# DigITs-AIML/MMNN_STS

Hardware: AMD Instinct MI355X
Metric: training volumes/sec/GPU (128^3 T1+T2+preop, batch 2) at 1/2/4/8 MI355X (higher is better)
Workload: dtype f32; 1 GPU; configs[2] --images --preop --survival --blend: MultiModalModel(DenseNet121-3D(in=2), MLP(32), blend) fwd + GradientBlender Cox loss + bwd + grad all-reduce + SGD-Nesterov/OneCycle step, dropout 0.2; micro_batch=2, global_batch=2, tabular=32, parallelism=dp1, allreduce=none

## Files before the change

### mmnn_sts_amd/csrc/conv3_bf16x3.hip

```cpp
#include <stdlib.h>

#include "fprop.hpp"

namespace mmnn {

typedef float f32x16_t __attribute__((ext_vector_type(16)));
typedef __bf16 bf16x8_t __attribute__((ext_vector_type(8)));

namespace c3b {
constexpr int KC = 16, NT = 7, MAXC = 256;
template <int TD, int TH, int TW>
struct Geo {
  static constexpr int HD = TD + 2, HH = TH + 2, HW = TW + 2, HV = HD * HH * HW, ROWS = TD * TH * TW / 32;
  static constexpr int ITEMS = (2 * HV + 255) / 256;
  static constexpr size_t OPER_BYTES = (size_t)2 * 6 * HV * 16;
  static constexpr size_t SMEM = OPER_BYTES + sizeof(float) * (2 * MAXC + 2 * 4 * 32 + 32);
  static_assert(TD * TH * TW % 32 == 0 && (TW == 32 || TW == 16), "rows of 32 voxels");
  static_assert(ITEMS <= NT, "one staging item per tap slot");
  static_assert(4 * ROWS * 16 * 64 * sizeof(float) <= OPER_BYTES, "the partial tiles are summed in the operand buffers");
  static_assert(SMEM <= 160 * 1024, "LDS");
};

__device__ __forceinline__ void split3(float x, __bf16& h, __bf16& m, __bf16& l) {
  h = (__bf16)x;
  const float r1 = x - (float)h;
  m = (__bf16)r1;
  l = (__bf16)(r1 - (float)m);
}
__device__ __forceinline__ uint32_t pack2(__bf16 lo, __bf16 hi) {
  return (uint32_t)__builtin_bit_cast(unsigned short, lo) | ((uint32_t)__builtin_bit_cast(unsigned short, hi) << 16);
}
__device__ __forceinline__ bf16x8_t as_bf16x8(uint4 v) { return __builtin_bit_cast(bf16x8_t, v); }
}

template <int TD, int TH, int TW>
__global__ void __launch_bounds__(256) conv3_fwd_bf16x3_kernel(const FpropArgs a) {
  using namespace c3b;
  using G = Geo<TD, TH, TW>;
  constexpr int HH = G::HH, HW = G::HW, HV = G::HV, ROWS = G::ROWS, ITEMS = G::ITEMS;
  constexpr size_t OPER_BYTES = G::OPER_BYTES;
  extern __shared__ uint4 xs128[];
  float* const coef = reinterpret_cast<float*>(reinterpret_cast<char*>(xs128) + OPER_BYTES);
  float* const sred = coef + 2 * MAXC;
  float* const dsc = sred + 2 * 4 * 32;
  const int tid = threadIdx.x, lane = tid & 63, wv = tid >> 6, g = tid & 1;
  const int D = a.D, H = a.H, W = a.W, V = D * H * W, Cin = a.Cin, nchunk = Cin / KC;
  const int twn = (W + TW - 1) / TW, thn = (H + TH - 1) / TH, tdn = (D + TD - 1) / TD;
  int b = blockIdx.x;
  const int w0 = (b % twn) * TW; b /= twn;
  const int h0 = (b % thn) * TH; b /= thn;
  const int d0 = (b % tdn) * TD;
  const int n = b / tdn;
  const float* __restrict__ xin = a.in0 + (long)n * a.in0_ns + (long)a.in0_coff * V;
  const float* __restrict__ wgt = a.w;
  for (int c = tid; c < Cin; c += 256) {
    float ca_, cb_, mu, rs;
    bn_fwd_coef(a.bn_in, c, ca_, cb_, mu, rs);
    coef[c] = ca_; coef[MAXC + c] = cb_;
  }
  if (tid < 32) dsc[tid] = drop_scale(a.drop_out, n, tid);
  f32x16_t acc[ROWS];
#pragma unroll
  for (int t = 0; t < ROWS; ++t)
#pragma unroll
    for (int q = 0; q < 16; ++q) acc[t][q] = 0.f;
  float xr[ITEMS][8], ca[8], cb[8];
  auto item_pos = [&](int it, int& hv, int& o) -> bool {
    const int item = tid + it * 256;
    hv = item >> 1;
    const int hd = hv / (HH * HW), hh = (hv / HW) % HH, hw = hv % HW;
    const int d = d0 + hd - 1, h = h0 + hh - 1, w = w0 + hw - 1;
    o = (d * H + h) * W + w;
    return item < 2 * HV && (unsigned)d < (unsigned)D && (unsigned)h < (unsigned)H && (unsigned)w < (unsigned)W;
  };
  auto issue = [&](int ch) {
    const int c0 = ch * KC + 8 * g;
#pragma unroll
    for (int e = 0; e < 8; ++e) { ca[e] = coef[c0 + e]; cb[e] = coef[MAXC + c0 + e]; }
#pragma unroll
    for (int it = 0; it < ITEMS; ++it) {
      int hv, o;
      const bool ok = item_pos(it, hv, o);
#pragma unroll
      for (int e = 0; e < 8; ++e) xr[it][e] = ok ? xin[(long)(c0 + e) * V + o] : 0.f;
    }
  };
  auto commit_item = [&](int it, int buf) {
    int hv, o;
    const bool ok = item_pos(it, hv, o);
    if (tid + it * 256 >= 2 * HV) return;
    __bf16 ph[8], pm[8], pl[8];
#pragma unroll
    for (int e = 0; e < 8; ++e) split3(ok ? fmaxf(fmaf(ca[e], xr[it][e], cb[e]), 0.f) : 0.f, ph[e], pm[e], pl[e]);
    uint4* dst = xs128 + buf * (6 * HV);
    dst[(0 * 2 + g) * HV + hv] = make_uint4(pack2(ph[0], ph[1]), pack2(ph[2], ph[3]), pack2(ph[4], ph[5]), pack2(ph[6], ph[7]));
    dst[(1 * 2 + g) * HV + hv] = make_uint4(pack2(pm[0], pm[1]), pack2(pm[2], pm[3]), pack2(pm[4], pm[5]), pack2(pm[6], pm[7]));
    dst[(2 * 2 + g) * HV + hv] = make_uint4(pack2(pl[0], pl[1]), pack2(pl[2], pl[3]), pack2(pl[4], pl[5]), pack2(pl[6], pl[7]));
  };
  float wr[NT][8];
  auto load_w = [&](int ti, int ch) {
    const int tap = wv + 4 * ti;
    if (tap < 27 && ch < nchunk) {
      const int c0 = ch * KC + 8 * (lane >> 5);
#pragma unroll
      for (int e = 0; e < 8; ++e) wr[ti][e] = wgt[((long)(c0 + e) * 27 + tap) * a.w_ld + (lane & 31)];
    }
  };
#pragma unroll
  for (int ti = 0; ti < NT; ++ti) load_w(ti, 0);
  __syncthreads();
  issue(0);
#pragma unroll
  for (int it = 0; it < ITEMS; ++it) commit_item(it, 0);
  __syncthreads();
  for (int ch = 0; ch < nchunk; ++ch) {
    const int cur = ch & 1;
    const bool more = ch + 1 < nchunk;
    if (more) issue(ch + 1);
#pragma unroll
    for (int ti = 0; ti < NT; ++ti) {
      const int tap = wv + 4 * ti;
      if (tap < 27) {
        const int td = tap / 9, th = (tap / 3) % 3, tw = tap % 3;
        __bf16 ph[8], pm[8], pl[8];
#pragma unroll
        for (int e = 0; e < 8; ++e) split3(wr[ti][e], ph[e], pm[e], pl[e]);
        bf16x8_t aw[3];
#pragma unroll
        for (int e = 0; e < 8; ++e) { aw[0][e] = ph[e]; aw[1][e] = pm[e]; aw[2][e] = pl[e]; }
        load_w(ti, ch + 1);
#pragma unroll
        for (int t = 0; t < ROWS; ++t) {
          const int v = t * 32 + (lane & 31);
          const int hv = ((v / (TW * TH) + td) * HH + ((v / TW) % TH + th)) * HW + (v % TW + tw);
          bf16x8_t bb[3];
#pragma unroll
          for (int p = 0; p < 3; ++p) bb[p] = as_bf16x8(xs128[cur * (6 * HV) + (p * 2 + (lane >> 5)) * HV + hv]);
          acc[t] = __builtin_amdgcn_mfma_f32_32x32x16_bf16(aw[1], bb[1], acc[t], 0, 0, 0);
          acc[t] = __builtin_amdgcn_mfma_f32_32x32x16_bf16(aw[0], bb[2], acc[t], 0, 0, 0);
          acc[t] = __builtin_amdgcn_mfma_f32_32x32x16_bf16(aw[2], bb[0], acc[t], 0, 0, 0);
          acc[t] = __builtin_amdgcn_mfma_f32_32x32x16_bf16(aw[0], bb[1], acc[t], 0, 0, 0);
          acc[t] = __builtin_amdgcn_mfma_f32_32x32x16_bf16(aw[1], bb[0], acc[t], 0, 0, 0);
          acc[t] = __builtin_amdgcn_mfma_f32_32x32x16_bf16(aw[0], bb[0], acc[t], 0, 0, 0);
        }
      }
      if (more && ti < ITEMS) commit_item(ti, cur ^ 1);
    }
    __syncthreads();
  }
  float* red = reinterpret_cast<float*>(xs128);
#pragma unroll
  for (int t = 0; t < ROWS; ++t)
#pragma unroll
    for (int q = 0; q < 16; ++q) red[((wv * ROWS + t) * 16 + q) * 64 + lane] = acc[t][q];
  __syncthreads();
  float* __restrict__ outn = a.out + (long)n * a.out_ns + (long)a.out_coff * V;
  const bool want_sums = a.st_out.sum != nullptr;
  float s0[16], s1[16];
#pragma unroll
  for (int q = 0; q < 16; ++q) { s0[q] = 0.f; s1[q] = 0.f; }
#pragma unroll
  for (int tt = 0; tt < (ROWS + 3) / 4; ++tt) {
    const int t = wv + 4 * tt;
    if (t >= ROWS) break;
    const int v = t * 32 + (lane & 31);
    const int d = d0 + v / (TW * TH), h = h0 + (v / TW) % TH, w = w0 + v % TW;
    const bool ok = d < D && h < H && w < W;
    const int o = (d * H + h) * W + w;
#pragma unroll
    for (int q = 0; q < 16; ++q) {
      float val = 0.f;
#pragma unroll
      for (int w2 = 0; w2 < 4; ++w2) val += red[((w2 * ROWS + t) * 16 + q) * 64 + lane];
      const int m = 8 * (q / 4) + 4 * (lane >> 5) + q % 4;
      val *= dsc[m];
      if (ok) {
        outn[(long)m * V + o] = val;
        s0[q] += val;
        s1[q] += val * val;
      }
    }
  }
  if (want_sums) {
#pragma unroll
    for (int q = 0; q < 16; ++q) {
      float t0 = s0[q], t1 = s1[q];
      t0 += swz_xor<16>(t0); t1 += swz_xor<16>(t1);
      t0 += swz_xor<8>(t0);  t1 += swz_xor<8>(t1);
      t0 += swz_xor<4>(t0);  t1 += swz_xor<4>(t1);
      t0 += swz_xor<2>(t0);  t1 += swz_xor<2>(t1);
      t0 += swz_xor<1>(t0);  t1 += swz_xor<1>(t1);
      if ((lane & 31) == 0) {
        const int m = 8 * (q / 4) + 4 * (lane >> 5) + q % 4;
        sred[wv * 32 + m] = t0;
        sred[4 * 32 + wv * 32 + m] = t1;
      }
    }
    __syncthreads();
    if (tid < 32) {
      const int rep = blockIdx.x & ((a.nrep > 0 ? a.nrep : NREP) - 1);
      double v0 = 0.0, v1 = 0.0;
#pragma unroll
      for (int w2 = 0; w2 < 4; ++w2) { v0 += (double)sred[w2 * 32 + tid]; v1 += (double)sred[4 * 32 + w2 * 32 + tid]; }
      atomicAdd(a.st_out.sum + (long)rep * a.st_out.stride + a.st_out.off + tid, v0);
      atomicAdd(a.st_out.sq + (long)rep * a.st_out.stride + a.st_out.off + tid, v1);
    }
  }
}

__global__ void __launch_bounds__(256) conv3_dgrad_bf16x3_kernel(const FpropArgs a) {
  using namespace c3b;
  using G = Geo<2, 4, 32>;
  constexpr int TH = 4, TW = 32, HH = G::HH, HW = G::HW, HV = G::HV, ROWS = G::ROWS, ITEMS = G::ITEMS, PF = 3;
  extern __shared__ uint4 xs128[];
  float* const coef = reinterpret_cast<float*>(reinterpret_cast<char*>(xs128) + G::OPER_BYTES);
  float* const ecoef = coef + 96;
  const int tid = threadIdx.x, lane = tid & 63, wv = tid >> 6, g = tid & 1;
  const int D = a.D, H = a.H, W = a.W, V = D * H * W;
  const int twn = (W + TW - 1) / TW, thn = (H + TH - 1) / TH, tdn = (D + 1) / 2;
  int b = blockIdx.x;
  const int w0 = (b % twn) * TW; b /= twn;
  const int h0 = (b % thn) * TH; b /= thn;
  const int d0 = (b % tdn) * 2;
  const int n = b / tdn;
  const float* __restrict__ in0n = a.in0 + (long)n * a.in0_ns + (long)a.in0_coff * V;
  const float* __restrict__ in1n = a.in1 + (long)n * a.in1_ns + (long)a.in1_coff * V;
  const float* __restrict__ wgt = a.w;
  if (tid < 32) {
    float p_, q_, r_;
    bn_bwd_coef(a.gr_in, tid, p_, q_, r_);
    const float sc = drop_scale(a.drop_in, n, tid);
    coef[tid] = p_ * sc; coef[32 + tid] = q_ * sc; coef[64 + tid] = r_ * sc;
  }
  if (tid >= 128) {
    const int m = tid - 128;
    float ea, eb, mu, rs;
    bn_fwd_coef(a.ebn, m, ea, eb, mu, rs);
    ecoef[m] = ea; ecoef[128 + m] = eb; ecoef[256 + m] = mu; ecoef[384 + m] = rs;
  }
  float x0[2][ITEMS][8], x1[2][ITEMS][8];
  auto item_pos = [&](int it, int& hv, int& o) -> bool {
    const int item = tid + it * 256;
    hv = item >> 1;
    const int hd = hv / (HH * HW), hh = (hv / HW) % HH, hw = hv % HW;
    const int d = d0 + hd - 1, h = h0 + hh - 1, w = w0 + hw - 1;
    o = (d * H + h) * W + w;
    return item < 2 * HV && (unsigned)d < (unsigned)D && (unsigned)h < (unsigned)H && (unsigned)w < (unsigned)W;
  };
  auto issue = [&](int ch) {
    const int c0 = ch * KC + 8 * g;
#pragma unroll
    for (int it = 0; it < ITEMS; ++it) {
      int hv, o;
      const bool ok = item_pos(it, hv, o);
#pragma unroll
      for (int e = 0; e < 8; ++e) {
        x0[ch][it][e] = ok ? in0n[(long)(c0 + e) * V + o] : 0.f;
        x1[ch][it][e] = ok ? in1n[(long)(c0 + e) * V + o] : 0.f;
      }
    }
  };
  auto commit_item = [&](int it, int buf) {
    int hv, o;
    const bool ok = item_pos(it, hv, o);
    if (tid + it * 256 >= 2 * HV) return;
    const int c0 = buf * KC + 8 * g;
    __bf16 ph[8], pm[8], pl[8];
#pragma unroll
    for (int e = 0; e < 8; ++e)
      split3(ok ? fmaf(coef[c0 + e], x0[buf][it][e], fmaf(coef[32 + c0 + e], x1[buf][it][e], coef[64 + c0 + e])) : 0.f, ph[e], pm[e], pl[e]);
    uint4* dst = xs128 + buf * (6 * HV);
    dst[(0 * 2 + g) * HV + hv] = make_uint4(pack2(ph[0], ph[1]), pack2(ph[2], ph[3]), pack2(ph[4], ph[5]), pack2(ph[6], ph[7]));
    dst[(1 * 2 + g) * HV + hv] = make_uint4(pack2(pm[0], pm[1]), pack2(pm[2], pm[3]), pack2(pm[4], pm[5]), pack2(pm[6], pm[7]));
    dst[(2 * 2 + g) * HV + hv] = make_uint4(pack2(pl[0], pl[1]), pack2(pl[2], pl[3]), pack2(pl[4], pl[5]), pack2(pl[6], pl[7]));
  };
  float wr[PF][8];
  auto load_w = [&](int slot, int tap, int ch) {
    if (ch < 2) {
      const int c0 = ch * KC + 8 * (lane >> 5);
#pragma unroll
      for (int e = 0; e < 8; ++e) wr[slot][e] = wgt[((long)(c0 + e) * 27 + tap) * a.w_ld + wv * 32 + (lane & 31)];
    }
  };
#pragma unroll
  for (int t = 0; t < PF; ++t) load_w(t, t, 0);
  issue(0);
  issue(1);
  __syncthreads();
#pragma unroll
  for (int it = 0; it < ITEMS; ++it) commit_item(it, 0);
#pragma unroll
  for (int it = 0; it < ITEMS; ++it) commit_item(it, 1);
  __syncthreads();
  f32x16_t acc[ROWS];
#pragma unroll
  for (int t = 0; t < ROWS; ++t)
#pragma unroll
    for (int q = 0; q < 16; ++q) acc[t][q] = 0.f;
  for (int ch = 0; ch < 2; ++ch) {
#pragma unroll 1
    for (int tq = 0; tq < 9; ++tq) {
    const int td = tq / 3, th = tq % 3;
#pragma unroll
    for (int tw = 0; tw < 3; ++tw) {
      const int tap = tq * 3 + tw;
      __bf16 ph[8], pm[8], pl[8];
#pragma unroll
      for (int e = 0; e < 8; ++e) split3(wr[tw][e], ph[e], pm[e], pl[e]);
      bf16x8_t aw[3];
#pragma unroll
      for (int e = 0; e < 8; ++e) { aw[0][e] = ph[e]; aw[1][e] = pm[e]; aw[2][e] = pl[e]; }
      if (tq < 8) load_w(tw, tap + PF, ch); else load_w(tw, tw, ch + 1);
#pragma unroll
      for (int t = 0; t < ROWS; ++t) {
        const int hv = ((t / TH + td) * HH + (t % TH + th)) * HW + ((lane & 31) + tw);
        bf16x8_t bb[3];
#pragma unroll
        for (int p = 0; p < 3; ++p) bb[p] = as_bf16x8(xs128[ch * (6 * HV) + (p * 2 + (lane >> 5)) * HV + hv]);
        acc[t] = __builtin_amdgcn_mfma_f32_32x32x16_bf16(aw[1], bb[1], acc[t], 0, 0, 0);
        acc[t] = __builtin_amdgcn_mfma_f32_32x32x16_bf16(aw[0], bb[2], acc[t], 0, 0, 0);
        acc[t] = __builtin_amdgcn_mfma_f32_32x32x16_bf16(aw[2], bb[0], acc[t], 0, 0, 0);
        acc[t] = __builtin_amdgcn_mfma_f32_32x32x16_bf16(aw[0], bb[1], acc[t], 0, 0, 0);
        acc[t] = __builtin_amdgcn_mfma_f32_32x32x16_bf16(aw[1], bb[0], acc[t], 0, 0, 0);
        acc[t] = __builtin_amdgcn_mfma_f32_32x32x16_bf16(aw[0], bb[0], acc[t], 0, 0, 0);
      }
    }
    }
  }
  const float* __restrict__ exn = a.ex + (long)n * a.ex_ns + (long)a.ex_coff * V;
  float* __restrict__ outn = a.out + (long)n * a.out_ns + (long)a.out_coff * V;
  float s0[16], s1[16];
#pragma unroll
  for (int q = 0; q < 16; ++q) { s0[q] = 0.f; s1[q] = 0.f; }
  auto row_pos = [&](int t, int& o) -> bool {
    const int d = d0 + t / TH, h = h0 + t % TH, w = w0 + (lane & 31);
    o = (d * H + h) * W + w;
    return d < D && h < H && w < W;
  };
  float xn[16];
  {
    int o;
    const bool ok = row_pos(0, o);
#pragma unroll
    for (int q = 0; q < 16; ++q) xn[q] = ok ? exn[(long)(wv * 32 + 8 * (q / 4) + 4 * (lane >> 5) + q % 4) * V + o] : 0.f;
  }
#pragma unroll
  for (int t = 0; t < ROWS; ++t) {
    int o;
    const bool ok = row_pos(t, o);
    float xe[16];
#pragma unroll
    for (int q = 0; q < 16; ++q) xe[q] = xn[q];
    if (t + 1 < ROWS) {
      int o2;
      const bool ok2 = row_pos(t + 1, o2);
#pragma unroll
      for (int q = 0; q < 16; ++q) xn[q] = ok2 ? exn[(long)(wv * 32 + 8 * (q / 4) + 4 * (lane >> 5) + q % 4) * V + o2] : 0.f;
    }
#pragma unroll
    for (int q = 0; q < 16; ++q) {
      const int m = wv * 32 + 8 * (q / 4) + 4 * (lane >> 5) + q % 4;
      if (ok) {
        const float pre = fmaf(ecoef[m], xe[q], ecoef[128 + m]);
        const float z = pre > 0.f ? acc[t][q] : 0.f;
        const float xh = (xe[q] - ecoef[256 + m]) * ecoef[384 + m];
        outn[(long)m * V + o] = z;
        s0[q] += z;
        s1[q] += z * xh;
      }
    }
  }
  const int rep = blockIdx.x & ((a.nrep > 0 ? a.nrep : NREP) - 1);
#pragma unroll
  for (int q = 0; q < 16; ++q) {
    float t0 = s0[q], t1 = s1[q];
    t0 += swz_xor<16>(t0); t1 += swz_xor<16>(t1);
    t0 += swz_xor<8>(t0);  t1 += swz_xor<8>(t1);
    t0 += swz_xor<4>(t0);  t1 += swz_xor<4>(t1);
    t0 += swz_xor<2>(t0);  t1 += swz_xor<2>(t1);
    t0 += swz_xor<1>(t0);  t1 += swz_xor<1>(t1);
    if ((lane & 31) == 0) {
      const int m = wv * 32 + 8 * (q / 4) + 4 * (lane >> 5) + q % 4;
      atomicAdd(a.dbeta + (long)rep * a.M + m, (double)t0);
      atomicAdd(a.dgamma + (long)rep * a.M + m, (double)t1);
    }
  }
}

bool conv3_dgrad_bf16x3_eligible(const FpropArgs& a) {
  static const int mode = [] { const char* e = getenv("MMNN_BF16X3_DGRAD"); return e ? atoi(e) : 1; }();
  static const int fmode = [] { const char* e = getenv("MMNN_BF16X3"); return e ? atoi(e) : 32; }();
  return mode != 0 && fmode != 0 && a.M == 128 && a.Cin == 32 && a.W > 16;
}

int launch_conv3_dgrad_bf16x3(const FpropArgs& a, hipStream_t stream) {
  using G = c3b::Geo<2, 4, 32>;
  constexpr size_t SMEM = G::OPER_BYTES + sizeof(float) * (96 + 512);
  static_assert(SMEM <= 160 * 1024, "LDS");
  MMNN_REQUIRE(conv3_dgrad_bf16x3_eligible(a), "conv3 dgrad bf16x3: shape not handled (M=%d, Cin=%d, W=%d)", a.M, a.Cin, a.W);
  MMNN_REQUIRE(a.in1 && a.ex && a.dgamma && a.dbeta, "conv3 dgrad bf16x3: operands missing");
  MMNN_REQUIRE((long)(a.M + 1) * a.D * a.H * a.W < (1l << 31), "conv3 dgrad bf16x3: volume too large for 32-bit element offsets");
  const long tiles = (long)a.N * cdiv(a.D, 2) * cdiv(a.H, 4) * cdiv(a.W, 32);
  MMNN_REQUIRE(tiles > 0 && tiles < (1l << 31), "conv3 dgrad bf16x3: grid out of range");
  static bool configured[MAX_DEVICES] = {false};
  bool& conf = configured[current_device_slot()];
  if (!conf) {
    MMNN_HIP(hipFuncSetAttribute(reinterpret_cast<const void*>(conv3_dgrad_bf16x3_kernel), hipFuncAttributeMaxDynamicSharedMemorySize, (int)SMEM));
    conf = true;
  }
  MMNN_LAUNCH(conv3_dgrad_bf16x3_kernel, dim3((unsigned)tiles), dim3(256), SMEM, stream, a);
  MMNN_HIP(hipGetLastError());
  return 0;
}

bool conv3_fwd_bf16x3_eligible(const FpropArgs& a) {
  static const int mode = [] { const char* e = getenv("MMNN_BF16X3"); return e ? atoi(e) : 32; }();
  return mode != 0 && a.M == 32 && a.Cin % c3b::KC == 0 && a.Cin >= c3b::KC && a.Cin <= c3b::MAXC && a.W > 16;
}

int launch_conv3_fwd_bf16x3(const FpropArgs& a, hipStream_t stream) {
  using G = c3b::Geo<2, 4, 32>;
  MMNN_REQUIRE(conv3_fwd_bf16x3_eligible(a), "conv3 bf16x3: shape not handled (M=%d, Cin=%d, W=%d)", a.M, a.Cin, a.W);
  MMNN_REQUIRE(a.drop_in.p <= 0.f, "conv3 bf16x3: no input dropout on this path");
  MMNN_REQUIRE((long)(a.Cin + 1) * a.D * a.H * a.W < (1l << 31), "conv3 bf16x3: volume too large for 32-bit element offsets");
  const long tiles = (long)a.N * cdiv(a.D, 2) * cdiv(a.H, 4) * cdiv(a.W, 32);
  MMNN_REQUIRE(tiles > 0 && tiles < (1l << 31), "conv3 bf16x3: grid out of range");
  static bool configured[MAX_DEVICES] = {false};
  bool& conf = configured[current_device_slot()];
  if (!conf) {
    MMNN_HIP(hipFuncSetAttribute(reinterpret_cast<const void*>(conv3_fwd_bf16x3_kernel<2, 4, 32>), hipFuncAttributeMaxDynamicSharedMemorySize, (int)G::SMEM));
    conf = true;
  }
  MMNN_LAUNCH((conv3_fwd_bf16x3_kernel<2, 4, 32>), dim3((unsigned)tiles), dim3(256), G::SMEM, stream, a);
  MMNN_HIP(hipGetLastError());
  return 0;
}

}
```

### mmnn_sts_amd/csrc/densenet.hip

```cpp
#include "densenet.hpp"

#include <stdlib.h>
#include <string.h>

#include <algorithm>

#include "fprop.hpp"
#include "stem.hpp"
#include "wgrad.hpp"

namespace mmnn {

static size_t align_up(size_t v, size_t a = 256) { return (v + a - 1) / a * a; }
constexpr size_t KZ_PART_BYTES = (size_t)512 * 4 * 1024 * sizeof(float);
constexpr unsigned KZ_CNT_ENTRIES = 4096;

namespace {
struct Carver {
  size_t cur = 0;
  size_t take(size_t bytes) {
    size_t o = cur;
    cur = align_up(cur + bytes);
    return o;
  }
};
}

int plan_build(Plan& p, const NetCfg& cfg, int N, int D, int H, int W) {
  MMNN_REQUIRE(cfg.nblocks >= 1 && cfg.nblocks <= MAX_BLOCKS, "plan: 1..%d dense blocks supported, got %d", MAX_BLOCKS, cfg.nblocks);
  MMNN_REQUIRE(cfg.in_channels >= 1 && cfg.in_channels <= 4, "plan: in_channels must be 1..4, got %d", cfg.in_channels);
  MMNN_REQUIRE(cfg.init_features >= 1 && cfg.init_features <= 64, "plan: init_features must be <= 64, got %d", cfg.init_features);
  MMNN_REQUIRE(cfg.growth >= 1 && cfg.growth <= 32, "plan: growth_rate must be <= 32, got %d", cfg.growth);
  MMNN_REQUIRE(cfg.bn_size >= 1 && cfg.dropout_p >= 0.f && cfg.dropout_p < 1.f, "plan: bad bn_size / dropout");
  MMNN_REQUIRE(N >= 1 && D >= 1 && H >= 1 && W >= 1, "plan: bad input extent");
  p.cfg = cfg; p.N = N; p.D = D; p.H = H; p.W = W;
  p.mid = cfg.bn_size * cfg.growth;
  p.D0 = (D - 1) / 2 + 1; p.H0 = (H - 1) / 2 + 1; p.W0 = (W - 1) / 2 + 1;
  int d = (p.D0 - 1) / 2 + 1, h = (p.H0 - 1) / 2 + 1, w = (p.W0 - 1) / 2 + 1;
  int c = cfg.init_features;
  for (int b = 0; b < cfg.nblocks; ++b) {
    MMNN_REQUIRE(cfg.block_layers[b] >= 1, "plan: empty dense block %d", b);
    MMNN_REQUIRE(d >= 1 && h >= 1 && w >= 1, "plan: input too small, block %d has no voxels", b + 1);
    p.Db[b] = d; p.Hb[b] = h; p.Wb[b] = w; p.Vb[b] = d * h * w;
    p.cin_b[b] = c;
    p.nrep_b[b] = (b == 0 || (long)N * d * h * w >= 32768) ? NREP : ((long)N * d * h * w >= 4096 ? 2 : 1);
    p.ctot_b[b] = c + cfg.block_layers[b] * cfg.growth;
    c = p.ctot_b[b];
    if (b != cfg.nblocks - 1) {
      MMNN_REQUIRE(c % 2 == 0, "plan: transition halves an odd channel count");
      c /= 2; d /= 2; h /= 2; w /= 2;
    }
  }
  long po = 0, ro = 0;
  int nbn = 0;
  auto bn = [&](int ch, long& w_, long& b_, long& m_, long& v_) { w_ = po; po += ch; b_ = po; po += ch; m_ = ro; ro += ch; v_ = ro; ro += ch; ++nbn; };
  p.p_conv0 = po; po += (long)cfg.init_features * cfg.in_channels * 343;
  bn(cfg.init_features, p.p_n0w, p.p_n0b, p.r_n0m, p.r_n0v);
  p.layers.assign(cfg.nblocks, {});
  p.trans.clear();
  for (int b = 0; b < cfg.nblocks; ++b) {
    int ci = p.cin_b[b];
    for (int l = 0; l < cfg.block_layers[b]; ++l) {
      LayerOff lo;
      lo.cin = ci;
      bn(ci, lo.n1w, lo.n1b, lo.r1m, lo.r1v);
      lo.c1 = po; po += (long)p.mid * ci;
      bn(p.mid, lo.n2w, lo.n2b, lo.r2m, lo.r2v);
      lo.c2 = po; po += (long)cfg.growth * p.mid * 27;
      p.layers[b].push_back(lo);
      ci += cfg.growth;
    }
    if (b != cfg.nblocks - 1) {
      TransOff t;
      t.cin = ci; t.cout = ci / 2;
      bn(ci, t.nw, t.nb, t.rm, t.rv);
      t.cw = po; po += (long)t.cout * ci;
      p.trans.push_back(t);
    } else {
      bn(ci, p.p_n5w, p.p_n5b, p.r_n5m, p.r_n5v);
    }
  }
  p.n_params = po; p.n_runstats = ro; p.n_bn = nbn;

  Carver cv;
  const int nb = cfg.nblocks;
  const size_t F = sizeof(float);
  const long V0 = (long)p.D0 * p.H0 * p.W0;
  p.o_conv0 = cv.take((size_t)N * cfg.init_features * V0 * F);
  p.o_idx = cv.take((size_t)N * cfg.init_features * p.Vb[0]);
  p.o_t1.assign(nb, {});
  size_t dap = 0;
  for (int b = 0; b < nb; ++b) {
    p.o_x[b] = cv.take((size_t)N * p.ctot_b[b] * p.Vb[b] * F);
    p.o_g[b] = cv.take((size_t)N * p.ctot_b[b] * p.Vb[b] * F);
    for (int l = 0; l < cfg.block_layers[b]; ++l) p.o_t1[b].push_back(cv.take((size_t)N * p.mid * p.Vb[b] * F));
    if (b != nb - 1) {
      p.o_ap[b] = cv.take((size_t)N * p.ctot_b[b] * p.Vb[b + 1] * F);
      dap = std::max(dap, (size_t)N * p.ctot_b[b] * p.Vb[b + 1] * F);
    } else {
      p.o_ap[b] = 0;
    }
  }
  p.o_dap = cv.take(dap ? dap : 256);
  p.o_dz0 = cv.take((size_t)N * cfg.init_features * V0 * F);
  const size_t PAIR = 2 * NREP * sizeof(double);
  p.o_fstat = cv.cur;
  p.o_st_conv0 = cv.take(PAIR * cfg.init_features);
  p.o_st_t1.assign(nb, {});
  for (int b = 0; b < nb; ++b) {
    p.o_st_x[b] = cv.take(PAIR * p.ctot_b[b]);
    for (int l = 0; l < cfg.block_layers[b]; ++l) p.o_st_t1[b].push_back(cv.take(PAIR * p.mid));
  }
  p.fstat_bytes = cv.cur - p.o_fstat;
  p.o_bstat = cv.cur;
  p.o_dg_n0 = cv.take(PAIR * cfg.init_features);
  p.o_dg_n1.assign(nb, {}); p.o_dg_n2.assign(nb, {}); p.o_dg_tr.clear();
  for (int b = 0; b < nb; ++b) {
    p.o_s_x[b] = cv.take(PAIR * p.ctot_b[b]);
    for (int l = 0; l < cfg.block_layers[b]; ++l) {
      p.o_dg_n1[b].push_back(cv.take(PAIR * p.layers[b][l].cin));
      p.o_dg_n2[b].push_back(cv.take(PAIR * p.mid));
    }
    if (b != nb - 1) p.o_dg_tr.push_back(cv.take(PAIR * p.ctot_b[b]));
  }
  p.o_dg_n5 = cv.take(PAIR * p.ctot_b[nb - 1]);
  p.bstat_bytes = cv.cur - p.o_bstat;
  p.o_pk_conv0 = cv.take((size_t)7 * stem_krows(cfg.in_channels) * 64 * F);
  p.o_pk_c1.assign(nb, {}); p.o_pk_c2f.assign(nb, {}); p.o_pk_c2b.assign(nb, {}); p.o_pk_tr.clear();
  for (int b = 0; b < nb; ++b) {
    for (int l = 0; l < cfg.block_layers[b]; ++l) {
      p.o_pk_c1[b].push_back(cv.take((size_t)p.mid * p.layers[b][l].cin * F));
      p.o_pk_c2f[b].push_back(cv.take((size_t)cfg.growth * p.mid * 27 * F));
      p.o_pk_c2b[b].push_back(cv.take((size_t)cfg.growth * p.mid * 27 * F));
    }
    if (b != nb - 1) p.o_pk_tr.push_back(cv.take((size_t)p.trans[b].cin * p.trans[b].cout * F));
  }
  p.ns_conv0 = stem_wgrad_pick_splits(N, p.D0, p.H0, p.W0, cfg.in_channels);
  p.o_sl_conv0 = cv.take((size_t)p.ns_conv0 * cfg.in_channels * cfg.init_features * 352 * F);
  p.o_sl_c1.assign(nb, {}); p.o_sl_c2.assign(nb, {}); p.ns_c1.assign(nb, {}); p.ns_c2.assign(nb, {});
  p.o_sl_tr.clear(); p.ns_tr.clear();
  for (int b = 0; b < nb; ++b) {
    for (int l = 0; l < cfg.block_layers[b]; ++l) {
      const int ci = p.layers[b][l].cin;
      int pairs = 0;
      {
        const int cw = wgrad1_channel_width(ci, p.Vb[b]);
        for (int k = 0; k < cfg.block_layers[b]; ++k)
          if (wgrad1_channel_width(p.layers[b][k].cin, p.Vb[b]) == cw) pairs += cdiv(p.layers[b][k].cin, cw);
      }
      const int s1 = wgrad_pick_splits(1, N, p.Db[b], p.Hb[b], p.Wb[b], p.mid, ci, pairs);
      const int s2 = wgrad_pick_splits(27, N, p.Db[b], p.Hb[b], p.Wb[b], cfg.growth, p.mid, cfg.block_layers[b]);
      p.ns_c1[b].push_back(s1); p.ns_c2[b].push_back(s2);
      p.o_sl_c1[b].push_back(cv.take((size_t)s1 * p.mid * ci * F));
      p.o_sl_c2[b].push_back(cv.take((size_t)s2 * 27 * cfg.growth * p.mid * F));
    }
    if (b != nb - 1) {
      const int s = wgrad_pick_splits(1, N, p.Db[b + 1], p.Hb[b + 1], p.Wb[b + 1], p.trans[b].cout, p.trans[b].cin);
      p.ns_tr.push_back(s);
      p.o_sl_tr.push_back(cv.take((size_t)s * p.trans[b].cout * p.trans[b].cin * F));
    }
  }
  for (int b = 0; b < nb; ++b) p.o_dz2[b] = cv.take((size_t)cfg.block_layers[b] * N * p.mid * p.Vb[b] * F);
  p.o_kz_part = cv.take(KZ_PART_BYTES);
  p.o_kz_cnt = cv.take(KZ_CNT_ENTRIES * sizeof(unsigned));
  int nlayers = 0;
  for (int b = 0; b < nb; ++b) nlayers += cfg.block_layers[b];
  p.n_run_jobs = nbn;
  p.n_pack_jobs = 1 + 3 * nlayers + (nb - 1);
  p.n_grad_jobs = 3 + 6 * nlayers + 3 * (nb - 1) + 2;
  p.o_jobs_run = cv.take(sizeof(RunStatJob) * p.n_run_jobs);
  p.o_jobs_pack = cv.take(sizeof(PackJob) * p.n_pack_jobs);
  p.o_jobs_grad = cv.take(sizeof(GradJob) * p.n_grad_jobs);
  p.n_layers = nlayers;
  p.o_wg_table = cv.take(sizeof(WgradArgs) * 2 * nlayers);
  p.ws_bytes = cv.cur;
  p.host_jobs_bytes = p.o_wg_table - p.o_jobs_run;
  if (p.host_jobs) { (void)hipHostFree(p.host_jobs); p.host_jobs = nullptr; }
  p.tab_params = nullptr; p.tab_run = nullptr; p.tab_ws = nullptr;
  return 0;
}

void plan_free(Plan& p) {
  if (p.host_jobs) (void)hipHostFree(p.host_jobs);
  p.host_jobs = nullptr;
  if (p.wg_pinned) (void)hipHostFree(p.wg_pinned);
  p.wg_pinned = nullptr;
  for (hipEvent_t e : p.timer_ev) (void)hipEventDestroy(e);
  p.timer_ev.clear();
  for (hipEvent_t e : p.sync_ev) (void)hipEventDestroy(e);
  p.sync_ev.clear();
  if (p.side) (void)hipStreamDestroy(p.side);
  if (p.side2) (void)hipStreamDestroy(p.side2);
  p.side = p.side2 = nullptr;
}

static StatPtr statptr(char* ws, size_t o, int C, int off, int nrep = NREP) {
  StatPtr s;
  s.sum = reinterpret_cast<double*>(ws + o);
  s.sq = s.sum + (long)NREP * C;
  s.stride = C;
  s.off = off;
  s.nrep = nrep;
  s.pad_ = 0;
  return s;
}
static float* fptr(char* ws, size_t o) { return reinterpret_cast<float*>(ws + o); }

static void set_kz(FpropArgs& a, const Plan& p, char* ws) {
  a.kz_part = p.no_kz ? nullptr : fptr(ws, p.o_kz_part); a.kz_cnt = reinterpret_cast<unsigned*>(ws + p.o_kz_cnt);
  a.kz_part_bytes = KZ_PART_BYTES; a.kz_cnt_entries = KZ_CNT_ENTRIES;
  a.trace = (p.trace_base && p.trace_seq < p.trace_slots) ? p.trace_base + (size_t)(p.trace_seq++) * 64 * 16 : nullptr;
}

static BnFwd bnfwd(const Plan& p, StatPtr st, const float* params, float* run, long w, long b, long rm, long rv, double count, int training) {
  BnFwd f;
  f.st = st;
  f.rmean = run + rm; f.rvar = run + rv;
  f.gamma = params + w; f.beta = params + b;
  f.inv_count = 1.0 / count;
  f.eps = p.cfg.eps;
  f.training = training;
  return f;
}

static bool build_tables(Plan& p, const float* params, float* run, char* ws) {
  if (p.tab_params == params && p.tab_run == run && p.tab_ws == ws) return false;
  char* hj = static_cast<char*>(p.host_jobs);
  RunStatJob* rj = reinterpret_cast<RunStatJob*>(hj);
  PackJob* pj = reinterpret_cast<PackJob*>(hj + (p.o_jobs_pack - p.o_jobs_run));
  GradJob* gj = reinterpret_cast<GradJob*>(hj + (p.o_jobs_grad - p.o_jobs_run));
  const NetCfg& c = p.cfg;
  const int nb = c.nblocks;
  int ir = 0, ip = 0, ig = 0;
  p.max_pack = 0; p.max_grad = 0;
  auto run_job = [&](size_t o, int C, int off, int n, long rm, long rv, double count) {
    StatPtr s = statptr(ws, o, C, off);
    RunStatJob j; j.sum = s.sum; j.sq = s.sq; j.stride = C; j.off = off; j.C = n; j.rmean = run ? run + rm : nullptr; j.rvar = run ? run + rv : nullptr; j.count = count;
    rj[ir++] = j;
  };
  auto pack_job = [&](long src, size_t dst, int kind, int M, int C, long count) {
    PackJob j; j.src = params + src; j.dst = fptr(ws, dst); j.kind = kind; j.M = M; j.C = C; j.count = count;
    pj[ip++] = j; p.max_pack = std::max(p.max_pack, count);
  };
  auto grad_slab = [&](int kind, size_t o, long stride, int ns, int M, int C, long dst, long count) {
    GradJob j; j.kind = kind; j.src = ws + o; j.stride = stride; j.nsplit = ns; j.off = 0; j.M = M; j.C = C; j.dst_off = dst; j.count = count;
    gj[ig++] = j; p.max_grad = std::max(p.max_grad, count);
  };
  auto grad_bn = [&](size_t o, int C, long dw, long db) {
    StatPtr s = statptr(ws, o, C, 0);
    GradJob j; j.kind = 3; j.stride = C; j.nsplit = 0; j.off = 0; j.M = 0; j.C = C; j.count = C;
    j.src = s.sq; j.dst_off = dw; gj[ig++] = j;
    j.src = s.sum; j.dst_off = db; gj[ig++] = j;
    p.max_grad = std::max(p.max_grad, (long)C);
  };
  const double cnt0 = (double)p.N * p.D0 * p.H0 * p.W0;
  run_job(p.o_st_conv0, c.init_features, 0, c.init_features, p.r_n0m, p.r_n0v, cnt0);
  pack_job(p.p_conv0, p.o_pk_conv0, (c.in_channels % 2 == 0) ? 3 : 4, c.init_features, c.in_channels, (long)7 * stem_krows(c.in_channels) * 64);
  grad_slab(2, p.o_sl_conv0, (long)c.in_channels * c.init_features * 352, p.ns_conv0, c.init_features, c.in_channels, p.p_conv0,
            (long)c.init_features * c.in_channels * 343);
  grad_bn(p.o_dg_n0, c.init_features, p.p_n0w, p.p_n0b);
  for (int b = 0; b < nb; ++b) {
    const double cnt = (double)p.N * p.Vb[b];
    p.gj_begin[b] = ig;
    const long max_before = p.max_grad;
    p.max_grad = 0;
    for (int l = 0; l < c.block_layers[b]; ++l) {
      const LayerOff& lo = p.layers[b][l];
      run_job(p.o_st_x[b], p.ctot_b[b], 0, lo.cin, lo.r1m, lo.r1v, cnt);
      run_job(p.o_st_t1[b][l], p.mid, 0, p.mid, lo.r2m, lo.r2v, cnt);
      pack_job(lo.c1, p.o_pk_c1[b][l], 0, p.mid, lo.cin, (long)p.mid * lo.cin);
      pack_job(lo.c2, p.o_pk_c2f[b][l], 1, c.growth, p.mid, (long)c.growth * p.mid * 27);
      pack_job(lo.c2, p.o_pk_c2b[b][l], 2, c.growth, p.mid, (long)c.growth * p.mid * 27);
      grad_bn(p.o_dg_n1[b][l], lo.cin, lo.n1w, lo.n1b);
      grad_slab(0, p.o_sl_c1[b][l], (long)p.mid * lo.cin, p.ns_c1[b][l], p.mid, lo.cin, lo.c1, (long)p.mid * lo.cin);
      grad_bn(p.o_dg_n2[b][l], p.mid, lo.n2w, lo.n2b);
      grad_slab(1, p.o_sl_c2[b][l], (long)27 * c.growth * p.mid, p.ns_c2[b][l], c.growth, p.mid, lo.c2, (long)c.growth * p.mid * 27);
    }
    if (b != nb - 1) {
      const TransOff& t = p.trans[b];
      run_job(p.o_st_x[b], p.ctot_b[b], 0, t.cin, t.rm, t.rv, cnt);
      pack_job(t.cw, p.o_pk_tr[b], 0, t.cout, t.cin, (long)t.cout * t.cin);
      grad_bn(p.o_dg_tr[b], t.cin, t.nw, t.nb);
      grad_slab(0, p.o_sl_tr[b], (long)t.cout * t.cin, p.ns_tr[b], t.cout, t.cin, t.cw, (long)t.cout * t.cin);
    } else {
      run_job(p.o_st_x[b], p.ctot_b[b], 0, p.ctot_b[b], p.r_n5m, p.r_n5v, cnt);
      grad_bn(p.o_dg_n5, p.ctot_b[b], p.p_n5w, p.p_n5b);
    }
    p.gj_max[b] = p.max_grad;
    p.max_grad = std::max(p.max_grad, max_before);
  }
  p.gj_begin[nb] = ig;
  p.n_run_jobs = ir; p.n_pack_jobs = ip; p.n_grad_jobs = ig;
  p.tab_params = params; p.tab_run = run; p.tab_ws = ws;
  return true;
}

namespace {
struct ScopedTimer {
  Plan& p; hipStream_t s; bool on;
  ScopedTimer(Plan& p_, int kind, int block, hipStream_t s_) : p(p_), s(s_), on(false) {
    if (!((p.timer_mask >> kind) & 1u) || (p.timer_block >= 0 && p.timer_block != block)) return;
    if (p.timer_used + 2 > p.timer_ev.size()) {
      if (p.timer_ev.size() >= 16384) return;
      hipEvent_t a, b;
      if (hipEventCreate(&a) != hipSuccess || hipEventCreate(&b) != hipSuccess) return;
      p.timer_ev.push_back(a); p.timer_ev.push_back(b);
      p.timer_tag.push_back(0);
    }
    p.timer_tag[p.timer_used / 2] = kind * MAX_BLOCKS + (block >= 0 && block < MAX_BLOCKS ? block : 0);
    on = hipEventRecord(p.timer_ev[p.timer_used], s) == hipSuccess;
  }
  ~ScopedTimer() {
    if (!on) return;
    (void)hipEventRecord(p.timer_ev[p.timer_used + 1], s);
    p.timer_used += 2;
  }
};
}

int plan_set_timer(Plan& p, int kind, int block) {
  MMNN_REQUIRE(kind >= -1 && kind < T_COUNT, "set_timer: unknown kernel class %d", kind);
  p.timer_mask = kind < 0 ? ~1u : (kind == T_NONE ? 0u : 1u << kind);
  p.timer_block = block; p.timer_used = 0;
  for (int k = 0; k < T_COUNT * MAX_BLOCKS; ++k) { p.timer_ms[k] = 0.0; p.timer_count[k] = 0; }
  return 0;
}

int plan_read_timer(Plan& p, int kind, int block, double* total_ms, long* count) {
  MMNN_REQUIRE(kind >= T_NONE && kind < T_COUNT && block < MAX_BLOCKS, "read_timer: unknown kernel class %d / block %d", kind, block);
  for (size_t i = 0; i + 1 < p.timer_used; i += 2) {
    MMNN_HIP(hipEventSynchronize(p.timer_ev[i + 1]));
    float ms = 0.f;
    MMNN_HIP(hipEventElapsedTime(&ms, p.timer_ev[i], p.timer_ev[i + 1]));
    const int k = p.timer_tag[i / 2];
    p.timer_ms[k] += ms; p.timer_count[k] += 1;
  }
  p.timer_used = 0;
  double ms = 0.0; long n = 0;
  for (int k = 1; k < T_COUNT; ++k)
    for (int b = 0; b < MAX_BLOCKS; ++b)
      if ((kind == T_NONE || kind == k) && (block < 0 || block == b)) { ms += p.timer_ms[k * MAX_BLOCKS + b]; n += p.timer_count[k * MAX_BLOCKS + b]; }
  if (total_ms) *total_ms = ms;
  if (count) *count = n;
  return 0;
}

int plan_set_option(Plan& p, const char* name, long value) {
  const std::string s(name ? name : "");
  if (s == "single_stream") { p.single_stream = value != 0; return 0; }
  if (s == "side_streams") { p.side_streams = value < 0 ? 0 : (value > 2 ? 2 : (int)value); p.side_tried = false; return 0; }
  if (s == "trace_buffer") { p.trace_base = reinterpret_cast<unsigned long long*>(value); p.trace_seq = 0; return 0; }
  if (s == "trace_slots") { p.trace_slots = (int)value; return 0; }
  if (s == "params_version") { p.params_version = value; return 0; }
  if (s == "no_kz") { p.no_kz = value != 0; return 0; }
  set_error("set_option: unknown option '%s'", s.c_str());
  return 1;
}

static DropCfg dropcfg(const Plan& p, uint64_t seed, int layer, int training) {
  DropCfg d;
  d.seed = seed; d.layer = layer;
  d.p = training ? p.cfg.dropout_p : 0.f;
  return d;
}

int plan_forward(Plan& p, const float* params, float* run, const float* x, char* ws, float* out, int training, uint64_t seed,
                 hipStream_t stream) {
  MMNN_REQUIRE(params && run && x && ws && out, "forward: null buffer");
  MMNN_REQUIRE(((uintptr_t)ws & 255) == 0 && ((uintptr_t)params & 15) == 0 && ((uintptr_t)x & 15) == 0, "forward: buffers must be 256/16-byte aligned");
  const NetCfg& c = p.cfg;
  const int nb = c.nblocks, N = p.N;
  if (!p.host_jobs) {
    MMNN_HIP(hipHostMalloc(&p.host_jobs, p.host_jobs_bytes, hipHostMallocDefault));
    memset(p.host_jobs, 0, p.host_jobs_bytes);
  }
  if (p.tab_params != params || p.tab_run != run || p.tab_ws != ws) {
    if (p.tab_ws != nullptr) MMNN_HIP(hipStreamSynchronize(stream));
    build_tables(p, params, run, ws);
    MMNN_HIP(hipMemcpyAsync(ws + p.o_jobs_run, p.host_jobs, p.host_jobs_bytes, hipMemcpyHostToDevice, stream));
  }
  p.trace_seq = 0;
  if (training) MMNN_HIP(hipMemsetAsync(ws + p.o_fstat, 0, p.fstat_bytes, stream));
  MMNN_HIP(hipMemsetAsync(ws + p.o_kz_cnt, 0, KZ_CNT_ENTRIES * sizeof(unsigned), stream));
  int rc = 0;
  if (p.params_version == 0 || p.params_version != p.packed_version || p.packed_params != params || p.packed_ws != ws) {
    rc = launch_pack(reinterpret_cast<const PackJob*>(ws + p.o_jobs_pack), p.n_pack_jobs, p.max_pack, stream);
    if (rc) return rc;
    p.packed_version = p.params_version; p.packed_params = params; p.packed_ws = ws;
    ++p.pack_launches;
  }

  const double cnt0 = (double)N * p.D0 * p.H0 * p.W0;
  {
    StemConvArgs a;
    a.N = N; a.Cin = c.in_channels; a.D = p.D; a.H = p.H; a.W = p.W; a.Do = p.D0; a.Ho = p.H0; a.Wo = p.W0; a.M = c.init_features;
    a.x = x; a.wp = fptr(ws, p.o_pk_conv0); a.out = fptr(ws, p.o_conv0);
    a.st_out = statptr(ws, p.o_st_conv0, c.init_features, 0);
    if (!training) a.st_out.sum = nullptr;
    { ScopedTimer t(p, T_STEM_CONV, -1, stream); rc = launch_stem_conv(a, stream); }
    if (rc) return rc;
    StemPoolArgs q;
    q.N = N; q.C = c.init_features; q.Di = p.D0; q.Hi = p.H0; q.Wi = p.W0; q.Do = p.Db[0]; q.Ho = p.Hb[0]; q.Wo = p.Wb[0];
    q.x = fptr(ws, p.o_conv0);
    q.bn = bnfwd(p, statptr(ws, p.o_st_conv0, c.init_features, 0), params, run, p.p_n0w, p.p_n0b, p.r_n0m, p.r_n0v, cnt0, training);
    q.out = fptr(ws, p.o_x[0]); q.out_ns = (long)p.ctot_b[0] * p.Vb[0];
    q.idx = reinterpret_cast<unsigned char*>(ws + p.o_idx);
    q.st_out = statptr(ws, p.o_st_x[0], p.ctot_b[0], 0, p.nrep_b[0]);
    if (!training) q.st_out.sum = nullptr;
    if ((rc = launch_stem_pool(q, stream))) return rc;
  }
  int layer_id = 0;
  for (int b = 0; b < nb; ++b) {
    const double cnt = (double)N * p.Vb[b];
    const long xns = (long)p.ctot_b[b] * p.Vb[b];
    for (int l = 0; l < c.block_layers[b]; ++l, ++layer_id) {
      const LayerOff& lo = p.layers[b][l];
      FpropArgs a;
      memset(&a, 0, sizeof(a));
      set_kz(a, p, ws);
      a.N = N; a.D = p.Db[b]; a.H = p.Hb[b]; a.W = p.Wb[b];
      a.Cin = lo.cin; a.M = p.mid; a.nrep = p.nrep_b[b];
      a.in0 = fptr(ws, p.o_x[b]); a.in0_ns = xns; a.in0_coff = 0;
      a.bn_in = bnfwd(p, statptr(ws, p.o_st_x[b], p.ctot_b[b], 0, p.nrep_b[b]), params, run, lo.n1w, lo.n1b, lo.r1m, lo.r1v, cnt, training);
      a.w = fptr(ws, p.o_pk_c1[b][l]); a.w_ld = p.mid;
      a.out = fptr(ws, p.o_t1[b][l]); a.out_ns = (long)p.mid * p.Vb[b]; a.out_coff = 0;
      a.st_out = statptr(ws, p.o_st_t1[b][l], p.mid, 0, p.nrep_b[b]);
      if (!training) a.st_out.sum = nullptr;
      a.pf_ptr = fptr(ws, p.o_pk_c2f[b][l]); a.pf_bytes = (unsigned)(sizeof(float) * c.growth * p.mid * 27);
      { ScopedTimer t(p, T_CONV1_FWD, b, stream); rc = launch_fprop(a, 1, PRO_BNRELU, EPI_STORE_STATS, stream); }
      if (rc) return rc;
      FpropArgs e;
      memset(&e, 0, sizeof(e));
      set_kz(e, p, ws);
      e.N = N; e.D = p.Db[b]; e.H = p.Hb[b]; e.W = p.Wb[b];
      e.Cin = p.mid; e.M = c.growth; e.nrep = p.nrep_b[b];
      e.in0 = fptr(ws, p.o_t1[b][l]); e.in0_ns = (long)p.mid * p.Vb[b]; e.in0_coff = 0;
      e.bn_in = bnfwd(p, statptr(ws, p.o_st_t1[b][l], p.mid, 0, p.nrep_b[b]), params, run, lo.n2w, lo.n2b, lo.r2m, lo.r2v, cnt, training);
      e.w = fptr(ws, p.o_pk_c2f[b][l]); e.w_ld = c.growth;
      e.out = fptr(ws, p.o_x[b]); e.out_ns = xns; e.out_coff = lo.cin;
      e.drop_out = dropcfg(p, seed, layer_id, training);
      e.st_out = statptr(ws, p.o_st_x[b], p.ctot_b[b], lo.cin, p.nrep_b[b]);
      if (!training) e.st_out.sum = nullptr;
      if (l + 1 < c.block_layers[b]) {
        e.pf_ptr = fptr(ws, p.o_pk_c1[b][l + 1]); e.pf_bytes = (unsigned)(sizeof(float) * p.mid * p.layers[b][l + 1].cin);
      } else if (b != nb - 1) {
        e.pf_ptr = fptr(ws, p.o_pk_tr[b]); e.pf_bytes = (unsigned)(sizeof(float) * p.trans[b].cin * p.trans[b].cout);
      }
      { ScopedTimer t(p, T_CONV2_FWD, b, stream); rc = launch_fprop(e, 27, PRO_BNRELU, EPI_STORE_STATS, stream); }
      if (rc) return rc;
    }
    if (b != nb - 1) {
      const TransOff& t = p.trans[b];
      PoolFwdArgs q;
      q.N = N; q.C = t.cin; q.D = p.Db[b]; q.H = p.Hb[b]; q.W = p.Wb[b];
      q.x = fptr(ws, p.o_x[b]); q.x_ns = xns;
      q.bn = bnfwd(p, statptr(ws, p.o_st_x[b], p.ctot_b[b], 0, p.nrep_b[b]), params, run, t.nw, t.nb, t.rm, t.rv, cnt, training);
      q.out = fptr(ws, p.o_ap[b]);
      if ((rc = launch_bnrelu_avgpool(q, stream))) return rc;
      FpropArgs a;
      memset(&a, 0, sizeof(a));
      set_kz(a, p, ws);
      a.N = N; a.D = p.Db[b + 1]; a.H = p.Hb[b + 1]; a.W = p.Wb[b + 1];
      a.Cin = t.cin; a.M = t.cout; a.nrep = p.nrep_b[b + 1];
      a.in0 = fptr(ws, p.o_ap[b]); a.in0_ns = (long)t.cin * p.Vb[b + 1]; a.in0_coff = 0;
      a.w = fptr(ws, p.o_pk_tr[b]); a.w_ld = t.cout;
      a.out = fptr(ws, p.o_x[b + 1]); a.out_ns = (long)p.ctot_b[b + 1] * p.Vb[b + 1]; a.out_coff = 0;
      a.st_out = statptr(ws, p.o_st_x[b + 1], p.ctot_b[b + 1], 0, p.nrep_b[b + 1]);
      if (!training) a.st_out.sum = nullptr;
      a.pf_ptr = fptr(ws, p.o_pk_c1[b + 1][0]); a.pf_bytes = (unsigned)(sizeof(float) * p.mid * p.layers[b + 1][0].cin);
      if ((rc = launch_fprop(a, 1, PRO_NONE, EPI_STORE_STATS, stream))) return rc;
    } else {
      BnApplyArgs q;
      q.N = N; q.C = p.ctot_b[b]; q.V = p.Vb[b];
      q.x = fptr(ws, p.o_x[b]); q.x_ns = xns;
      q.bn = bnfwd(p, statptr(ws, p.o_st_x[b], p.ctot_b[b], 0, p.nrep_b[b]), params, run, p.p_n5w, p.p_n5b, p.r_n5m, p.r_n5v, cnt, training);
      q.out = out;
      if ((rc = launch_bn_apply(q, stream))) return rc;
    }
  }
  if (training) {
    if ((rc = launch_running_stats(reinterpret_cast<const RunStatJob*>(ws + p.o_jobs_run), p.n_run_jobs, c.momentum,
                                   p.nbt_count == p.n_run_jobs ? p.nbt : nullptr, stream))) return rc;
  }
  return 0;
}

static void layer_wgrad_args(const Plan& p, const float* params, float* run, char* ws, int b, int l, int layer_id, uint64_t seed,
                             WgradArgs& w2, WgradArgs& w1) {
  const NetCfg& c = p.cfg;
  const int N = p.N;
  const double cnt = (double)N * p.Vb[b];
  const long xns = (long)p.ctot_b[b] * p.Vb[b], tns = (long)p.mid * p.Vb[b];
  const LayerOff& lo = p.layers[b][l];
  const BnFwd bn1 = bnfwd(p, statptr(ws, p.o_st_x[b], p.ctot_b[b], 0, p.nrep_b[b]), params, run, lo.n1w, lo.n1b, lo.r1m, lo.r1v, cnt, 1);
  const BnFwd bn2 = bnfwd(p, statptr(ws, p.o_st_t1[b][l], p.mid, 0, p.nrep_b[b]), params, run, lo.n2w, lo.n2b, lo.r2m, lo.r2v, cnt, 1);
  const StatPtr dg2 = statptr(ws, p.o_dg_n2[b][l], p.mid, 0, p.nrep_b[b]);
  float* dz2 = fptr(ws, p.o_dz2[b]) + (long)l * N * tns;
  memset(&w2, 0, sizeof(w2));
  w2.N = N; w2.D = p.Db[b]; w2.H = p.Hb[b]; w2.W = p.Wb[b];
  w2.M = c.growth; w2.Cin = p.mid;
  w2.g0 = fptr(ws, p.o_g[b]); w2.g0_ns = xns; w2.g0_coff = lo.cin;
  w2.g1 = fptr(ws, p.o_x[b]); w2.g1_ns = xns; w2.g1_coff = lo.cin;
  w2.gr.st = statptr(ws, p.o_st_x[b], p.ctot_b[b], lo.cin, p.nrep_b[b]);
  w2.gr.s = statptr(ws, p.o_s_x[b], p.ctot_b[b], lo.cin, p.nrep_b[b]);
  w2.gr.gamma = nullptr; w2.gr.inv_count = 1.0 / cnt; w2.gr.eps = c.eps;
  w2.drop.seed = seed; w2.drop.layer = layer_id; w2.drop.p = c.dropout_p;
  w2.x = fptr(ws, p.o_t1[b][l]); w2.x_ns = tns; w2.x_coff = 0;
  w2.bn = bn2;
  w2.slab = fptr(ws, p.o_sl_c2[b][l]); w2.slab_stride = (long)27 * c.growth * p.mid; w2.nsplit = p.ns_c2[b][l];
  memset(&w1, 0, sizeof(w1));
  w1.N = N; w1.D = p.Db[b]; w1.H = p.Hb[b]; w1.W = p.Wb[b];
  w1.M = p.mid; w1.Cin = lo.cin;
  w1.g0 = dz2; w1.g0_ns = tns; w1.g0_coff = 0;
  w1.g1 = fptr(ws, p.o_t1[b][l]); w1.g1_ns = tns; w1.g1_coff = 0;
  w1.gr.st = statptr(ws, p.o_st_t1[b][l], p.mid, 0, p.nrep_b[b]);
  w1.gr.s = dg2;
  w1.gr.gamma = params + lo.n2w; w1.gr.inv_count = 1.0 / cnt; w1.gr.eps = c.eps;
  w1.x = fptr(ws, p.o_x[b]); w1.x_ns = xns; w1.x_coff = 0;
  w1.bn = bn1;
  w1.slab = fptr(ws, p.o_sl_c1[b][l]); w1.slab_stride = (long)p.mid * lo.cin; w1.nsplit = p.ns_c1[b][l];
}

int plan_backward(Plan& p, const float* params, const float* x, char* ws, const float* grad_out, float* grad_params, int accumulate,
                  uint64_t seed, hipStream_t stream) {
  return plan_backward_range(p, params, x, ws, grad_out, grad_params, accumulate, seed, p.cfg.nblocks - 1, 0, stream);
}

int plan_block_param_range(const Plan& p, int block, long* begin, long* end) {
  const int nb = p.cfg.nblocks;
  MMNN_REQUIRE(block >= -1 && block < nb && begin && end, "block_param_range: block %d out of range [-1, %d)", block, nb);
  if (block < 0) { *begin = 0; *end = p.layers[0][0].n1w; return 0; }
  *begin = p.layers[block][0].n1w;
  *end = (block + 1 < nb) ? p.layers[block + 1][0].n1w : p.n_params;
  return 0;
}

int plan_backward_range(Plan& p, const float* params, const float* x, char* ws, const float* grad_out, float* grad_params, int accumulate,
                        uint64_t seed, int hi, int lo, hipStream_t stream) {
  MMNN_REQUIRE(params && x && ws && grad_out && grad_params, "backward: null buffer");
  MMNN_REQUIRE(p.tab_ws == ws && p.tab_params == params, "backward: must follow a training forward on the same buffers");
  const NetCfg& c = p.cfg;
  const int nb = c.nblocks, N = p.N;
  MMNN_REQUIRE(hi >= lo && lo >= 0 && hi < nb, "backward: bad block range [%d, %d] of %d blocks", lo, hi, nb);
  MMNN_REQUIRE(hi == nb - 1 || p.bwd_next == hi, "backward: block range [%d, %d] out of order (expected to continue at block %d)", lo, hi, p.bwd_next);
  float* run = p.tab_run;
  int rc;
  const bool first_call = hi == nb - 1;
  if (first_call) {
    MMNN_HIP(hipMemsetAsync(ws + p.o_bstat, 0, p.bstat_bytes, stream));
    MMNN_HIP(hipMemsetAsync(ws + p.o_kz_cnt, 0, KZ_CNT_ENTRIES * sizeof(unsigned), stream));
  }
  p.bwd_next = lo - 1;
  const int want_side = p.single_stream ? 0 : p.side_streams;
  const bool single = want_side <= 0;
  if (!single && (!p.side || (want_side >= 2 && !p.side2)) && !p.side_tried) {
    p.side_tried = true;
    if (!p.side && hipStreamCreateWithFlags(&p.side, hipStreamNonBlocking) != hipSuccess) p.side = nullptr;
    if (want_side >= 2 && p.side && !p.side2 && hipStreamCreateWithFlags(&p.side2, hipStreamNonBlocking) != hipSuccess) p.side2 = nullptr;
  }
  hipStream_t side = (p.side && !single) ? p.side : stream;
  hipStream_t side2 = (p.side2 && !single && want_side >= 2) ? p.side2 : side;
  const bool two = side != stream;
  p.sync_used = 0;
  auto next_event = [&]() -> hipEvent_t {
    if (p.sync_used == p.sync_ev.size()) {
      hipEvent_t e = nullptr;
      if (hipEventCreateWithFlags(&e, hipEventDisableTiming) != hipSuccess) return nullptr;
      p.sync_ev.push_back(e);
    }
    return p.sync_ev[p.sync_used++];
  };
  auto order = [&](hipStream_t from, hipStream_t to) -> int {
    if (!two) return 0;
    hipEvent_t e = next_event();
    MMNN_REQUIRE(e != nullptr, "backward: cannot create a synchronisation event");
    MMNN_HIP(hipEventRecord(e, from));
    MMNN_HIP(hipStreamWaitEvent(to, e, 0));
    return 0;
  };
  if (first_call || !p.wg_uploaded) {
    const size_t bytes = sizeof(WgradArgs) * 2 * p.n_layers;
    if (!p.wg_pinned) {
      MMNN_HIP(hipHostMalloc(&p.wg_pinned, bytes, hipHostMallocDefault));
      p.wg_shadow.assign(bytes, 0);
      p.wg_uploaded = false;
    }
    std::vector<WgradArgs> tab(2 * p.n_layers);
    int id = 0;
    for (int b = 0; b < nb; ++b)
      for (int l = 0; l < c.block_layers[b]; ++l, ++id) layer_wgrad_args(p, params, run, ws, b, l, id, 0, tab[id], tab[p.n_layers + id]);
    if (!p.wg_uploaded || memcmp(tab.data(), p.wg_shadow.data(), bytes) != 0) {
      if (p.wg_uploaded) MMNN_HIP(hipStreamSynchronize(stream));
      memcpy(p.wg_pinned, tab.data(), bytes);
      memcpy(p.wg_shadow.data(), tab.data(), bytes);
      MMNN_HIP(hipMemcpyAsync(ws + p.o_wg_table, p.wg_pinned, bytes, hipMemcpyHostToDevice, stream));
      p.wg_uploaded = true;
    }
  }
  const WgradArgs* dev_w2 = reinterpret_cast<const WgradArgs*>(ws + p.o_wg_table);
  const WgradArgs* dev_w1 = dev_w2 + p.n_layers;
  struct PendingW { WgradArgs w2, w1; int b, id; };
  std::vector<PendingW> pend;
  static const bool no_batch = [] { const char* e = getenv("MMNN_NO_WGRAD_BATCH"); return e && e[0] == '1'; }();
  auto flush = [&]() -> int {
    if (pend.empty()) return 0;
    int rc2;
    if (two) {
      hipEvent_t e = next_event();
      MMNN_REQUIRE(e != nullptr, "backward: cannot create a synchronisation event");
      MMNN_HIP(hipEventRecord(e, stream));
      MMNN_HIP(hipStreamWaitEvent(side, e, 0));
      if (side2 != side) MMNN_HIP(hipStreamWaitEvent(side2, e, 0));
    }
    const int np = (int)pend.size();
    std::vector<WgradArgs> host(np);
    if (np > 1 && !no_batch) {
      for (int i = 0; i < np; ++i) host[np - 1 - i] = pend[i].w2;
      { ScopedTimer t(p, T_CONV2_WGRAD, pend[0].b, side); rc2 = launch_wgrad_batched(host.data(), dev_w2 + pend[np - 1].id, np, seed, 27, PRO_BNRELU, side); }
      if (rc2) return rc2;
      for (int i = 0; i < np;) {
        int j = i + 1;
        const long vb = (long)pend[i].w1.D * pend[i].w1.H * pend[i].w1.W;
        while (j < np && wgrad1_channel_width(pend[j].w1.Cin, vb) == wgrad1_channel_width(pend[i].w1.Cin, vb)) ++j;
        if (j - i > 1) {
          for (int k = i; k < j; ++k) host[j - 1 - k] = pend[k].w1;
          ScopedTimer t(p, T_CONV1_WGRAD, pend[i].b, side2);
          rc2 = launch_wgrad_batched(host.data(), dev_w1 + pend[j - 1].id, j - i, seed, 1, PRO_BNRELU, side2);
        } else {
          ScopedTimer t(p, T_CONV1_WGRAD, pend[i].b, side2);
          rc2 = launch_wgrad(pend[i].w1, 1, PRO_BNRELU, side2);
        }
        if (rc2) return rc2;
        i = j;
      }
    } else {
      for (const PendingW& q : pend) {
        { ScopedTimer t(p, T_CONV2_WGRAD, q.b, side); rc2 = launch_wgrad(q.w2, 27, PRO_BNRELU, side); }
        if (rc2) return rc2;
      }
      for (const PendingW& q : pend) {
        { ScopedTimer t(p, T_CONV1_WGRAD, q.b, side2); rc2 = launch_wgrad(q.w1, 1, PRO_BNRELU, side2); }
        if (rc2) return rc2;
      }
    }
    pend.clear();
    return 0;
  };
  auto sptr = [&](int b, int off) { return statptr(ws, p.o_s_x[b], p.ctot_b[b], off, p.nrep_b[b]); };
  auto concat_grad = [&](int b, int off) {
    BnBwd g;
    g.st = statptr(ws, p.o_st_x[b], p.ctot_b[b], off, p.nrep_b[b]);
    g.s = sptr(b, off);
    g.gamma = nullptr;
    g.inv_count = 1.0 / ((double)N * p.Vb[b]);
    g.eps = c.eps;
    return g;
  };
  if (first_call) {
    const int b = nb - 1;
    ConsumerBwdArgs a;
    a.N = N; a.C = p.ctot_b[b]; a.D = p.Db[b]; a.H = p.Hb[b]; a.W = p.Wb[b]; a.mode = 0; a.nrep = p.nrep_b[b];
    a.dy = grad_out;
    a.x = fptr(ws, p.o_x[b]); a.x_ns = (long)p.ctot_b[b] * p.Vb[b];
    a.bn = bnfwd(p, statptr(ws, p.o_st_x[b], p.ctot_b[b], 0, p.nrep_b[b]), params, run, p.p_n5w, p.p_n5b, p.r_n5m, p.r_n5v, (double)N * p.Vb[b], 1);
    a.g = fptr(ws, p.o_g[b]); a.g_ns = a.x_ns;
    StatPtr dg = statptr(ws, p.o_dg_n5, p.ctot_b[b], 0, p.nrep_b[b]);
    a.dbeta = dg.sum; a.dgamma = dg.sq;
    a.s_acc = sptr(b, 0);
    if ((rc = launch_consumer_bwd(a, stream))) return rc;
  }
  int layer_id = 0;
  for (int b = 0; b <= hi; ++b) layer_id += c.block_layers[b];
  for (int b = hi; b >= lo; --b) {
    const double cnt = (double)N * p.Vb[b];
    const long xns = (long)p.ctot_b[b] * p.Vb[b];
    const long tns = (long)p.mid * p.Vb[b];
    for (int l = c.block_layers[b] - 1; l >= 0; --l) {
      --layer_id;
      const LayerOff& lo = p.layers[b][l];
      const BnFwd bn1 = bnfwd(p, statptr(ws, p.o_st_x[b], p.ctot_b[b], 0, p.nrep_b[b]), params, run, lo.n1w, lo.n1b, lo.r1m, lo.r1v, cnt, 1);
      const BnFwd bn2 = bnfwd(p, statptr(ws, p.o_st_t1[b][l], p.mid, 0, p.nrep_b[b]), params, run, lo.n2w, lo.n2b, lo.r2m, lo.r2v, cnt, 1);
      const StatPtr dg2 = statptr(ws, p.o_dg_n2[b][l], p.mid, 0, p.nrep_b[b]);
      const StatPtr dg1 = statptr(ws, p.o_dg_n1[b][l], lo.cin, 0, p.nrep_b[b]);
      const DropCfg drop = dropcfg(p, seed, layer_id, 1);
      FpropArgs a;
      memset(&a, 0, sizeof(a));
      set_kz(a, p, ws);
      a.N = N; a.D = p.Db[b]; a.H = p.Hb[b]; a.W = p.Wb[b];
      a.Cin = c.growth; a.M = p.mid; a.nrep = p.nrep_b[b];
      a.in0 = fptr(ws, p.o_g[b]); a.in0_ns = xns; a.in0_coff = lo.cin;
      a.in1 = fptr(ws, p.o_x[b]); a.in1_ns = xns; a.in1_coff = lo.cin;
      a.gr_in = concat_grad(b, lo.cin);
      a.drop_in = drop;
      a.w = fptr(ws, p.o_pk_c2b[b][l]); a.w_ld = p.mid;
      float* dz2 = fptr(ws, p.o_dz2[b]) + (long)l * N * tns;
      a.out = dz2; a.out_ns = tns; a.out_coff = 0;
      a.ex = fptr(ws, p.o_t1[b][l]); a.ex_ns = tns; a.ex_coff = 0;
      a.ebn = bn2;
      a.dbeta = dg2.sum; a.dgamma = dg2.sq;
      a.pf_ptr = params + lo.c1; a.pf_bytes = (unsigned)(sizeof(float) * p.mid * lo.cin);
      { ScopedTimer t(p, T_CONV2_DGRAD, b, stream); rc = launch_fprop(a, 27, PRO_GRAD, EPI_MASK_STORE, stream); }
      if (rc) return rc;
      WgradArgs w2, w1;
      layer_wgrad_args(p, params, run, ws, b, l, layer_id, seed, w2, w1);
      w2.trace = (p.trace_base && p.trace_seq < p.trace_slots) ? p.trace_base + (size_t)(p.trace_seq++) * 64 * 16 : nullptr;
      w1.trace = (p.trace_base && p.trace_seq < p.trace_slots) ? p.trace_base + (size_t)(p.trace_seq++) * 64 * 16 : nullptr;
      BnBwd g1;
      g1.st = statptr(ws, p.o_st_t1[b][l], p.mid, 0, p.nrep_b[b]);
      g1.s = dg2;
      g1.gamma = params + lo.n2w;
      g1.inv_count = 1.0 / cnt;
      g1.eps = c.eps;
      FpropArgs d;
      memset(&d, 0, sizeof(d));
      set_kz(d, p, ws);
      d.N = N; d.D = p.Db[b]; d.H = p.Hb[b]; d.W = p.Wb[b];
      d.Cin = p.mid; d.M = lo.cin; d.nrep = p.nrep_b[b];
      d.in0 = dz2; d.in0_ns = tns; d.in0_coff = 0;
      d.in1 = fptr(ws, p.o_t1[b][l]); d.in1_ns = tns; d.in1_coff = 0;
      d.gr_in = g1;
      d.w = params + lo.c1; d.w_ld = lo.cin;
      d.out = fptr(ws, p.o_g[b]); d.out_ns = xns; d.out_coff = 0;
      d.ex = fptr(ws, p.o_x[b]); d.ex_ns = xns; d.ex_coff = 0;
      d.ebn = bn1;
      d.dbeta = dg1.sum; d.dgamma = dg1.sq;
      d.s_acc = sptr(b, 0);
      if (l > 0) { d.pf_ptr = fptr(ws, p.o_pk_c2b[b][l - 1]); d.pf_bytes = (unsigned)(sizeof(float) * c.growth * p.mid * 27); }
      { ScopedTimer t(p, T_CONV1_DGRAD, b, stream); rc = launch_fprop(d, 1, PRO_GRAD, EPI_MASK_ACCUM, stream); }
      if (rc) return rc;
      PendingW pw;
      pw.w2 = w2; pw.w1 = w1; pw.b = b; pw.id = layer_id;
      pend.push_back(pw);
      if (l == 0 && (rc = flush())) return rc;
    }
    if (two) {
      if ((rc = order(stream, side))) return rc;
      if (side2 != side && (rc = order(side2, side))) return rc;
      if ((rc = launch_finalize(reinterpret_cast<const GradJob*>(ws + p.o_jobs_grad) + p.gj_begin[b], p.gj_begin[b + 1] - p.gj_begin[b],
                                p.gj_max[b], grad_params, accumulate, side))) return rc;
    }
    if (b > 0) {
      const int pb = b - 1;
      const TransOff& t = p.trans[pb];
      const long pxns = (long)p.ctot_b[pb] * p.Vb[pb];
      WgradArgs w;
      memset(&w, 0, sizeof(w));
      w.N = N; w.D = p.Db[b]; w.H = p.Hb[b]; w.W = p.Wb[b];
      w.M = t.cout; w.Cin = t.cin;
      w.g0 = fptr(ws, p.o_g[b]); w.g0_ns = xns; w.g0_coff = 0;
      w.g1 = fptr(ws, p.o_x[b]); w.g1_ns = xns; w.g1_coff = 0;
      w.gr = concat_grad(b, 0);
      w.x = fptr(ws, p.o_ap[pb]); w.x_ns = (long)t.cin * p.Vb[b]; w.x_coff = 0;
      w.slab = fptr(ws, p.o_sl_tr[pb]); w.slab_stride = (long)t.cout * t.cin; w.nsplit = p.ns_tr[pb];
      if ((rc = launch_wgrad(w, 1, PRO_NONE, stream))) return rc;
      FpropArgs d;
      memset(&d, 0, sizeof(d));
      set_kz(d, p, ws);
      d.N = N; d.D = p.Db[b]; d.H = p.Hb[b]; d.W = p.Wb[b];
      d.Cin = t.cout; d.M = t.cin;
      d.in0 = w.g0; d.in0_ns = xns; d.in0_coff = 0;
      d.in1 = w.g1; d.in1_ns = xns; d.in1_coff = 0;
      d.gr_in = w.gr;
      d.w = params + t.cw; d.w_ld = t.cin;
      d.out = fptr(ws, p.o_dap); d.out_ns = (long)t.cin * p.Vb[b]; d.out_coff = 0;
      if ((rc = launch_fprop(d, 1, PRO_GRAD, EPI_STORE, stream))) return rc;
      ConsumerBwdArgs q;
      q.N = N; q.C = t.cin; q.D = p.Db[pb]; q.H = p.Hb[pb]; q.W = p.Wb[pb]; q.mode = 1; q.nrep = p.nrep_b[pb];
      q.dy = fptr(ws, p.o_dap);
      q.x = fptr(ws, p.o_x[pb]); q.x_ns = pxns;
      q.bn = bnfwd(p, statptr(ws, p.o_st_x[pb], p.ctot_b[pb], 0, p.nrep_b[pb]), params, run, t.nw, t.nb, t.rm, t.rv, (double)N * p.Vb[pb], 1);
      q.g = fptr(ws, p.o_g[pb]); q.g_ns = pxns;
      StatPtr dg = statptr(ws, p.o_dg_tr[pb], t.cin, 0, p.nrep_b[pb]);
      q.dbeta = dg.sum; q.dgamma = dg.sq;
      q.s_acc = sptr(pb, 0);
      if ((rc = launch_consumer_bwd(q, stream))) return rc;
    } else {
      const double cnt0 = (double)N * p.D0 * p.H0 * p.W0;
      StemPoolBwdArgs q;
      q.N = N; q.C = c.init_features; q.Di = p.D0; q.Hi = p.H0; q.Wi = p.W0; q.Do = p.Db[0]; q.Ho = p.Hb[0]; q.Wo = p.Wb[0];
      q.x = fptr(ws, p.o_conv0);
      q.bn = bnfwd(p, statptr(ws, p.o_st_conv0, c.init_features, 0), params, run, p.p_n0w, p.p_n0b, p.r_n0m, p.r_n0v, cnt0, 1);
      q.g = fptr(ws, p.o_g[0]); q.g_ns = xns;
      q.xp = fptr(ws, p.o_x[0]); q.xp_ns = xns;
      q.gr = concat_grad(0, 0);
      q.idx = reinterpret_cast<const unsigned char*>(ws + p.o_idx);
      q.dz = fptr(ws, p.o_dz0);
      StatPtr dg = statptr(ws, p.o_dg_n0, c.init_features, 0);
      q.dbeta = dg.sum; q.dgamma = dg.sq;
      if ((rc = launch_stem_pool_bwd(q, stream))) return rc;
      StemWgradArgs w;
      w.N = N; w.Cin = c.in_channels; w.D = p.D; w.H = p.H; w.W = p.W; w.Do = p.D0; w.Ho = p.H0; w.Wo = p.W0; w.M = c.init_features;
      w.x = x; w.dz = fptr(ws, p.o_dz0); w.y = fptr(ws, p.o_conv0);
      w.gr.st = statptr(ws, p.o_st_conv0, c.init_features, 0);
      w.gr.s = dg;
      w.gr.gamma = params + p.p_n0w;
      w.gr.inv_count = 1.0 / cnt0;
      w.gr.eps = c.eps;
      w.slab = fptr(ws, p.o_sl_conv0); w.slab_stride = (long)c.in_channels * c.init_features * 352; w.nsplit = p.ns_conv0;
      { ScopedTimer t(p, T_STEM_WGRAD, -1, stream); rc = launch_stem_wgrad(w, stream); }
      if (rc) return rc;
    }
  }
  if ((rc = order(side, stream))) return rc;
  if (side2 != side && (rc = order(side2, stream))) return rc;
  const long stem_count = (long)c.init_features * c.in_channels * 343;
  const GradJob* jobs = reinterpret_cast<const GradJob*>(ws + p.o_jobs_grad);
  if (two) {
    if (lo > 0) return 0;
    return launch_finalize(jobs, 3, stem_count, grad_params, accumulate, stream);
  }
  const int j0 = lo == 0 ? 0 : p.gj_begin[lo], j1 = p.gj_begin[hi + 1];
  long jmax = lo == 0 ? stem_count : 0;
  for (int b = lo; b <= hi; ++b) jmax = std::max(jmax, p.gj_max[b]);
  return launch_finalize(jobs + j0, j1 - j0, jmax, grad_params, accumulate, stream);
}

int plan_relu_mask(Plan& p, const float* params, char* ws, int kind, int b, int l, unsigned char* out, hipStream_t stream) {
  MMNN_REQUIRE(p.tab_ws == ws && p.tab_params == params, "relu_mask: must follow a training forward on the same buffers");
  const NetCfg& c = p.cfg;
  float* run = p.tab_run;
  MaskArgs a;
  a.out = out; a.N = p.N;
  if (kind == 0) {
    a.C = c.init_features; a.V = p.D0 * p.H0 * p.W0;
    a.x = fptr(ws, p.o_conv0); a.x_ns = (long)a.C * a.V;
    a.bn = bnfwd(p, statptr(ws, p.o_st_conv0, c.init_features, 0), params, run, p.p_n0w, p.p_n0b, p.r_n0m, p.r_n0v, (double)p.N * a.V, 1);
    return launch_relu_mask(a, stream);
  }
  MMNN_REQUIRE(b >= 0 && b < c.nblocks, "relu_mask: bad block %d", b);
  const double cnt = (double)p.N * p.Vb[b];
  a.V = p.Vb[b];
  if (kind == 3) {
    MMNN_REQUIRE(b < c.nblocks - 1, "relu_mask: block %d has no transition", b);
    const TransOff& t = p.trans[b];
    a.C = t.cin; a.x = fptr(ws, p.o_x[b]); a.x_ns = (long)p.ctot_b[b] * p.Vb[b];
    a.bn = bnfwd(p, statptr(ws, p.o_st_x[b], p.ctot_b[b], 0, p.nrep_b[b]), params, run, t.nw, t.nb, t.rm, t.rv, cnt, 1);
    return launch_relu_mask(a, stream);
  }
  MMNN_REQUIRE(l >= 0 && l < c.block_layers[b] && (kind == 1 || kind == 2), "relu_mask: bad site (%d,%d,%d)", kind, b, l);
  const LayerOff& lo = p.layers[b][l];
  if (kind == 1) {
    a.C = lo.cin; a.x = fptr(ws, p.o_x[b]); a.x_ns = (long)p.ctot_b[b] * p.Vb[b];
    a.bn = bnfwd(p, statptr(ws, p.o_st_x[b], p.ctot_b[b], 0, p.nrep_b[b]), params, run, lo.n1w, lo.n1b, lo.r1m, lo.r1v, cnt, 1);
  } else {
    a.C = p.mid; a.x = fptr(ws, p.o_t1[b][l]); a.x_ns = (long)p.mid * p.Vb[b];
    a.bn = bnfwd(p, statptr(ws, p.o_st_t1[b][l], p.mid, 0, p.nrep_b[b]), params, run, lo.n2w, lo.n2b, lo.r2m, lo.r2v, cnt, 1);
  }
  return launch_relu_mask(a, stream);
}

long plan_ws_offset(const Plan& p, const char* name, int i, int j) {
  const std::string s(name);
  const int nb = p.cfg.nblocks;
  auto okb = [&](int b) { return b >= 0 && b < nb; };
  auto okl = [&](int b, int l) { return okb(b) && l >= 0 && l < p.cfg.block_layers[b]; };
  if (s == "conv0") return (long)p.o_conv0;
  if (s == "idx") return (long)p.o_idx;
  if (s == "dz0") return (long)p.o_dz0;
  if (s == "dz2" && okl(i, j)) return (long)(p.o_dz2[i] + (size_t)j * p.N * p.mid * p.Vb[i] * sizeof(float));
  if (s == "dap") return (long)p.o_dap;
  if (s == "x" && okb(i)) return (long)p.o_x[i];
  if (s == "g" && okb(i)) return (long)p.o_g[i];
  if (s == "ap" && okb(i) && i < nb - 1) return (long)p.o_ap[i];
  if (s == "t1" && okl(i, j)) return (long)p.o_t1[i][j];
  if (s == "st_conv0") return (long)p.o_st_conv0;
  if (s == "st_x" && okb(i)) return (long)p.o_st_x[i];
  if (s == "st_t1" && okl(i, j)) return (long)p.o_st_t1[i][j];
  if (s == "s_x" && okb(i)) return (long)p.o_s_x[i];
  if (s == "pk_c1" && okl(i, j)) return (long)p.o_pk_c1[i][j];
  if (s == "pk_c2f" && okl(i, j)) return (long)p.o_pk_c2f[i][j];
  if (s == "pk_c2b" && okl(i, j)) return (long)p.o_pk_c2b[i][j];
  if (s == "pk_conv0") return (long)p.o_pk_conv0;
  if (s == "#pack_launches") return p.pack_launches;
  return -1;
}

}
```

### mmnn_sts_amd/csrc/densenet.hpp

```cpp
#pragma once
#include <string>
#include <vector>

#include "common.hpp"
#include "elementwise.hpp"

namespace mmnn {

constexpr int MAX_BLOCKS = 8;

struct NetCfg {
  int in_channels, init_features, growth, bn_size, nblocks;
  int block_layers[MAX_BLOCKS];
  float eps, momentum, dropout_p;
};

struct LayerOff {
  long n1w, n1b, c1, n2w, n2b, c2;
  long r1m, r1v, r2m, r2v;
  int cin;
};
struct TransOff { long nw, nb, cw; long rm, rv; int cin, cout; };

struct Plan {
  NetCfg cfg;
  int N, D, H, W;
  int D0, H0, W0;
  int Db[MAX_BLOCKS], Hb[MAX_BLOCKS], Wb[MAX_BLOCKS], Vb[MAX_BLOCKS];
  int cin_b[MAX_BLOCKS], ctot_b[MAX_BLOCKS];
  int nrep_b[MAX_BLOCKS];
  int mid;
  long p_conv0, p_n0w, p_n0b, r_n0m, r_n0v, p_n5w, p_n5b, r_n5m, r_n5v;
  std::vector<std::vector<LayerOff>> layers;
  std::vector<TransOff> trans;
  long n_params, n_runstats;
  int n_bn;
  size_t ws_bytes;
  size_t o_conv0, o_idx, o_x[MAX_BLOCKS], o_g[MAX_BLOCKS], o_ap[MAX_BLOCKS], o_dz2[MAX_BLOCKS], o_dap, o_dz0;
  std::vector<std::vector<size_t>> o_t1;
  size_t o_fstat, fstat_bytes, o_bstat, bstat_bytes;
  size_t o_st_conv0, o_st_x[MAX_BLOCKS];
  std::vector<std::vector<size_t>> o_st_t1;
  size_t o_s_x[MAX_BLOCKS];
  size_t o_dg_n0, o_dg_n5;
  std::vector<std::vector<size_t>> o_dg_n1, o_dg_n2;
  std::vector<size_t> o_dg_tr;
  size_t o_pk_conv0;
  std::vector<std::vector<size_t>> o_pk_c1, o_pk_c2f, o_pk_c2b;
  std::vector<size_t> o_pk_tr;
  size_t o_sl_conv0; int ns_conv0;
  std::vector<std::vector<size_t>> o_sl_c1, o_sl_c2;
  std::vector<std::vector<int>> ns_c1, ns_c2;
  std::vector<size_t> o_sl_tr; std::vector<int> ns_tr;
  size_t o_kz_part, o_kz_cnt;
  size_t o_jobs_run, o_jobs_pack, o_jobs_grad;
  int n_layers = 0;
  size_t o_wg_table = 0;
  void* wg_pinned = nullptr; std::vector<char> wg_shadow; bool wg_uploaded = false;
  void* host_jobs = nullptr; size_t host_jobs_bytes = 0;
  const float* tab_params = nullptr; float* tab_run = nullptr; char* tab_ws = nullptr;
  int n_run_jobs = 0, n_pack_jobs = 0, n_grad_jobs = 0; long max_pack = 0, max_grad = 0;
  int gj_begin[MAX_BLOCKS + 1] = {0};
  long gj_max[MAX_BLOCKS] = {0};
  hipStream_t side = nullptr, side2 = nullptr; bool side_tried = false;
  std::vector<hipEvent_t> sync_ev; size_t sync_used = 0;
  unsigned timer_mask = 0; int timer_block = -1;
  std::vector<hipEvent_t> timer_ev;
  std::vector<int> timer_tag;
  size_t timer_used = 0;
  double timer_ms[16 * MAX_BLOCKS] = {0}; long timer_count[16 * MAX_BLOCKS] = {0};
  bool single_stream = false;
  int side_streams = 0;
  long params_version = 0, packed_version = 0; const float* packed_params = nullptr; const char* packed_ws = nullptr;
  long pack_launches = 0;
  long long* nbt = nullptr; int nbt_count = 0;
  bool no_kz = false;
  int bwd_next = -1;
  unsigned long long* trace_base = nullptr; mutable int trace_seq = 0; int trace_slots = 0;
};

enum TimerKind { T_NONE = 0, T_CONV2_FWD = 1, T_CONV2_DGRAD = 2, T_CONV2_WGRAD = 3, T_CONV1_FWD = 4, T_CONV1_DGRAD = 5,
                 T_CONV1_WGRAD = 6, T_STEM_CONV = 7, T_STEM_WGRAD = 8, T_BLOCK_FWD = 9, T_COUNT = 10 };
int plan_set_timer(Plan& p, int kind, int block);
int plan_read_timer(Plan& p, int kind, int block, double* total_ms, long* count);
int plan_set_option(Plan& p, const char* name, long value);

int plan_build(Plan& p, const NetCfg& cfg, int N, int D, int H, int W);
void plan_free(Plan& p);
int plan_forward(Plan& p, const float* params, float* runstats, const float* x, char* ws, float* out, int training,
                 uint64_t seed, hipStream_t stream);
int plan_backward(Plan& p, const float* params, const float* x, char* ws, const float* grad_out, float* grad_params,
                  int accumulate, uint64_t seed, hipStream_t stream);
int plan_backward_range(Plan& p, const float* params, const float* x, char* ws, const float* grad_out, float* grad_params,
                        int accumulate, uint64_t seed, int hi, int lo, hipStream_t stream);
int plan_block_param_range(const Plan& p, int block, long* begin, long* end);
long plan_ws_offset(const Plan& p, const char* name, int i, int j);
int plan_relu_mask(Plan& p, const float* params, char* ws, int kind, int b, int l, unsigned char* out, hipStream_t stream);

}
```

### mmnn_sts_amd/csrc/elementwise.hip

```cpp
#include "elementwise.hpp"

#include <algorithm>

namespace mmnn {

__device__ __forceinline__ void block_sum2(float& s0, float& s1, float (*red)[4]) {
  s0 = wave_sum(s0);
  s1 = wave_sum(s1);
  const int wave = threadIdx.x >> 6;
  if ((threadIdx.x & 63) == 0) { red[0][wave] = s0; red[1][wave] = s1; }
  __syncthreads();
  s0 = red[0][0] + red[0][1] + red[0][2] + red[0][3];
  s1 = red[1][0] + red[1][1] + red[1][2] + red[1][3];
}

__global__ void __launch_bounds__(256) bnrelu_avgpool_kernel(const PoolFwdArgs a) {
  const int c = blockIdx.y, n = blockIdx.z;
  const int Do = a.D / 2, Ho = a.H / 2, Wo = a.W / 2;
  const int Vo = Do * Ho * Wo, V = a.D * a.H * a.W;
  float ca, cb, mu, rs;
  bn_fwd_coef(a.bn, c, ca, cb, mu, rs);
  const float* xc = a.x + (long)n * a.x_ns + (long)c * V;
  for (int p = blockIdx.x * 256 + threadIdx.x; p < Vo; p += gridDim.x * 256) {
    const int wo = p % Wo, ho = (p / Wo) % Ho, d_o = p / (Wo * Ho);
    float s = 0.f;
#pragma unroll
    for (int kd = 0; kd < 2; ++kd)
#pragma unroll
      for (int kh = 0; kh < 2; ++kh) {
        const float* row = xc + ((long)(2 * d_o + kd) * a.H + 2 * ho + kh) * a.W + 2 * wo;
        s += fmaxf(fmaf(ca, row[0], cb), 0.f) + fmaxf(fmaf(ca, row[1], cb), 0.f);
      }
    a.out[((long)n * a.C + c) * Vo + p] = s * 0.125f;
  }
}

int launch_bnrelu_avgpool(const PoolFwdArgs& a, hipStream_t stream) {
  MMNN_REQUIRE(a.N > 0 && a.C > 0 && a.D >= 2 && a.H >= 2 && a.W >= 2, "avgpool: extent too small (%d,%d,%d)", a.D, a.H, a.W);
  MMNN_REQUIRE(a.N <= 65535 && a.C <= 65535, "avgpool: grid out of range");
  const int Vo = (a.D / 2) * (a.H / 2) * (a.W / 2);
  MMNN_LAUNCH(bnrelu_avgpool_kernel, dim3(cdiv(Vo, 256), a.C, a.N), dim3(256), 0, stream, a);
  MMNN_HIP(hipGetLastError());
  return 0;
}

__global__ void __launch_bounds__(256) bn_apply_kernel(const BnApplyArgs a) {
  const int c = blockIdx.y, n = blockIdx.z;
  float ca, cb, mu, rs;
  bn_fwd_coef(a.bn, c, ca, cb, mu, rs);
  const float* xc = a.x + (long)n * a.x_ns + (long)c * a.V;
  float* oc = a.out + ((long)n * a.C + c) * a.V;
  for (int v = blockIdx.x * 256 + threadIdx.x; v < a.V; v += gridDim.x * 256) oc[v] = fmaf(ca, xc[v], cb);
}

int launch_bn_apply(const BnApplyArgs& a, hipStream_t stream) {
  MMNN_REQUIRE(a.N > 0 && a.C > 0 && a.V > 0 && a.N <= 65535 && a.C <= 65535, "bn_apply: bad extent");
  int gx = cdiv(a.V, 256);
  if (gx > 64) gx = 64;
  MMNN_LAUNCH(bn_apply_kernel, dim3(gx, a.C, a.N), dim3(256), 0, stream, a);
  MMNN_HIP(hipGetLastError());
  return 0;
}

__global__ void __launch_bounds__(256) relu_mask_kernel(const MaskArgs a) {
  const int c = blockIdx.y, n = blockIdx.z;
  float ca, cb, mu, rs;
  bn_fwd_coef(a.bn, c, ca, cb, mu, rs);
  const float* xc = a.x + (long)n * a.x_ns + (long)c * a.V;
  unsigned char* oc = a.out + ((long)n * a.C + c) * a.V;
  for (int v = blockIdx.x * 256 + threadIdx.x; v < a.V; v += gridDim.x * 256) oc[v] = fmaf(ca, xc[v], cb) > 0.f ? 1 : 0;
}

int launch_relu_mask(const MaskArgs& a, hipStream_t stream) {
  MMNN_REQUIRE(a.N > 0 && a.C > 0 && a.V > 0 && a.N <= 65535 && a.C <= 65535 && a.out, "relu_mask: bad arguments");
  int gx = cdiv(a.V, 256);
  if (gx > 64) gx = 64;
  MMNN_LAUNCH(relu_mask_kernel, dim3(gx, a.C, a.N), dim3(256), 0, stream, a);
  MMNN_HIP(hipGetLastError());
  return 0;
}

__global__ void __launch_bounds__(256) consumer_bwd_kernel(const ConsumerBwdArgs a) {
  __shared__ float red[2][4];
  const int c = blockIdx.y, n = blockIdx.z;
  const int V = a.D * a.H * a.W;
  const int Do = a.D / 2, Ho = a.H / 2, Wo = a.W / 2;
  float ca, cb, mu, rs;
  bn_fwd_coef(a.bn, c, ca, cb, mu, rs);
  const float gam = a.bn.gamma[c];
  const float* xc = a.x + (long)n * a.x_ns + (long)c * V;
  float* gc = a.g + (long)n * a.g_ns + (long)c * V;
  const float* dyc = a.dy + ((long)n * a.C + c) * (a.mode == 0 ? V : Do * Ho * Wo);
  float s0 = 0.f, s1 = 0.f;
  if (a.mode == 1 && (a.W & 3) == 0 && ((((uintptr_t)xc | (uintptr_t)gc) & 15) == 0) && (Wo & 1) == 0 &&
      (long)V * (a.W >> 2) < (4l << 32) && (long)a.D * a.H * a.H < (1l << 32)) {
    const int wq_n = a.W >> 2, rows = a.D * a.H, items = rows * wq_n;
    const unsigned mg_q = wq_n > 1 ? (unsigned)((0x100000000ull + wq_n - 1) / wq_n) : 0u;
    const unsigned mg_h = a.H > 1 ? (unsigned)((0x100000000ull + a.H - 1) / a.H) : 0u;
    for (int it = blockIdx.x * 256 + threadIdx.x; it < items; it += gridDim.x * 256) {
      const int row = mg_q ? (int)__umulhi((unsigned)it, mg_q) : it;
      const int w = (it - row * wq_n) << 2;
      const int d = mg_h ? (int)__umulhi((unsigned)row, mg_h) : row;
      const int h = row - d * a.H;
      const int v = row * a.W + w;
      const f32x4 x = *reinterpret_cast<const f32x4*>(xc + v);
      const int pw = w >> 1, ph = h >> 1, pd = d >> 1;
      float dy0 = 0.f, dy1 = 0.f;
      if (pw < Wo && ph < Ho && pd < Do) {
        const float* q = dyc + ((long)pd * Ho + ph) * Wo + pw;
        dy0 = 0.125f * q[0]; dy1 = 0.125f * q[1];
      }
      f32x4 g;
#pragma unroll
      for (int e = 0; e < 4; ++e) {
        const float z = fmaf(ca, x[e], cb) > 0.f ? (e < 2 ? dy0 : dy1) : 0.f;
        g[e] = gam * z;
        s0 += z;
        s1 += z * (x[e] - mu) * rs;
      }
      *reinterpret_cast<f32x4*>(gc + v) = g;
    }
  } else
  for (int v = blockIdx.x * 256 + threadIdx.x; v < V; v += gridDim.x * 256) {
    const float x = xc[v];
    float z;
    if (a.mode == 0) {
      z = dyc[v];
    } else {
      const int w = v % a.W, h = (v / a.W) % a.H, d = v / (a.W * a.H);
      const int pw = w >> 1, ph = h >> 1, pd = d >> 1;
      z = 0.f;
      if (pw < Wo && ph < Ho && pd < Do && fmaf(ca, x, cb) > 0.f) z = 0.125f * dyc[((long)pd * Ho + ph) * Wo + pw];
    }
    gc[v] = gam * z;
    s0 += z;
    s1 += z * (x - mu) * rs;
  }
  block_sum2(s0, s1, red);
  if (threadIdx.x == 0) {
    const int rep = blockIdx.x & ((a.nrep > 0 ? a.nrep : NREP) - 1);
    atomicAdd(a.dbeta + (long)rep * a.C + c, (double)s0);
    atomicAdd(a.dgamma + (long)rep * a.C + c, (double)s1);
    atomicAdd(a.s_acc.sum + (long)rep * a.s_acc.stride + a.s_acc.off + c, (double)gam * s0);
    atomicAdd(a.s_acc.sq + (long)rep * a.s_acc.stride + a.s_acc.off + c, (double)gam * s1);
  }
}

int launch_consumer_bwd(const ConsumerBwdArgs& a, hipStream_t stream) {
  MMNN_REQUIRE(a.N > 0 && a.C > 0 && a.N <= 65535 && a.C <= 65535, "consumer_bwd: bad extent");
  MMNN_REQUIRE(a.mode == 0 || a.mode == 1, "consumer_bwd: bad mode");
  const int V = a.D * a.H * a.W;
  int gx = cdiv(V, 8192);
  if (gx > 64) gx = 64;
  MMNN_LAUNCH(consumer_bwd_kernel, dim3(gx, a.C, a.N), dim3(256), 0, stream, a);
  MMNN_HIP(hipGetLastError());
  return 0;
}

__global__ void __launch_bounds__(256) running_stats_kernel(const RunStatJob* jobs, float momentum, long long* nbt) {
  const RunStatJob j = jobs[blockIdx.x];
  if (nbt && threadIdx.x == 0) nbt[blockIdx.x] += 1;
  for (int c = threadIdx.x; c < j.C; c += 256) {
    const double mean = stat_total(j.sum, j.stride, j.off + c) / j.count;
    double var = stat_total(j.sq, j.stride, j.off + c) / j.count - mean * mean;
    if (var < 0.0) var = 0.0;
    const double unb = j.count > 1.0 ? var * j.count / (j.count - 1.0) : var;
    j.rmean[c] = (float)((1.0 - momentum) * (double)j.rmean[c] + momentum * mean);
    j.rvar[c] = (float)((1.0 - momentum) * (double)j.rvar[c] + momentum * unb);
  }
}

int launch_running_stats(const RunStatJob* jobs_dev, int njobs, float momentum, long long* nbt, hipStream_t stream) {
  if (njobs <= 0) return 0;
  MMNN_LAUNCH(running_stats_kernel, dim3(njobs), dim3(256), 0, stream, jobs_dev, momentum, nbt);
  MMNN_HIP(hipGetLastError());
  return 0;
}

__global__ void __launch_bounds__(256) pack_kernel(const PackJob* jobs) {
  const PackJob j = jobs[blockIdx.y];
  if (j.kind <= 2) {
    __shared__ float tile[32][33];
    const int B = j.kind == 2 ? j.M : 1, I = j.kind == 2 ? j.C : j.M, J = j.kind == 0 ? j.C : (j.kind == 1 ? j.C * 27 : 27);
    const bool flip = j.kind == 2;
    const int ti_n = (I + 31) / 32, tj_n = (J + 31) / 32;
    const long ntiles = (long)B * ti_n * tj_n;
    const int tx = threadIdx.x & 31, ty = threadIdx.x >> 5;
    for (long t = blockIdx.x; t < ntiles; t += gridDim.x) {
      const int tj = (int)(t % tj_n), ti = (int)((t / tj_n) % ti_n), b = (int)(t / ((long)tj_n * ti_n));
      const float* src = j.src + (long)b * I * J;
      float* dst = j.dst + (long)b * I * J;
      __syncthreads();
#pragma unroll
      for (int r = 0; r < 4; ++r) {
        const int i = ti * 32 + ty + 8 * r, jj = tj * 32 + tx;
        tile[ty + 8 * r][tx] = (i < I && jj < J) ? src[(long)i * J + jj] : 0.f;
      }
      __syncthreads();
#pragma unroll
      for (int r = 0; r < 4; ++r) {
        const int jj = tj * 32 + ty + 8 * r, i = ti * 32 + tx;
        if (i < I && jj < J) dst[(long)(flip ? J - 1 - jj : jj) * I + i] = tile[tx][ty + 8 * r];
      }
    }
    return;
  }
  for (long i = (long)blockIdx.x * 256 + threadIdx.x; i < j.count; i += (long)gridDim.x * 256) {
    float v = 0.f;
    if (j.kind == 0) {
      const int m = (int)(i % j.M), c = (int)(i / j.M);
      v = j.src[(long)m * j.C + c];
    } else if (j.kind == 1) {
      const int m = (int)(i % j.M);
      const long k = i / j.M;
      v = j.src[(long)m * j.C * 27 + k];
    } else if (j.kind == 2) {
      const int c = (int)(i % j.C);
      const long k = i / j.C;
      const int t = (int)(k % 27), m = (int)(k / 27);
      v = j.src[((long)m * j.C + c) * 27 + 26 - t];
    } else if (j.kind == 3) {
      const int m = (int)(i % 64);
      long k = i / 64;
      const int r = (int)(k % (j.C * 49)), kd = (int)(k / (j.C * 49));
      const int c = r / 49, hw = r % 49;
      if (m < j.M) v = j.src[(((long)m * j.C + c) * 7 + kd) * 49 + hw];
    } else {
      const int m = (int)(i % 64);
      long k = i / 64;
      const int r = (int)(k % (j.C * 56)), kd = (int)(k / (j.C * 56));
      const int c = r / 56, kh = (r % 56) / 8, kw = r % 8;
      if (m < j.M && kw < 7) v = j.src[((((long)m * j.C + c) * 7 + kd) * 7 + kh) * 7 + kw];
    }
    j.dst[i] = v;
  }
}

int launch_pack(const PackJob* jobs_dev, int njobs, long max_count, hipStream_t stream) {
  if (njobs <= 0) return 0;
  MMNN_REQUIRE(njobs <= 65535, "pack: too many jobs");
  int gx = cdiv(max_count, 256 * 4);
  if (gx < 1) gx = 1;
  if (gx > 256) gx = 256;
  MMNN_LAUNCH(pack_kernel, dim3(gx, njobs), dim3(256), 0, stream, jobs_dev);
  MMNN_HIP(hipGetLastError());
  return 0;
}

__global__ void __launch_bounds__(256) finalize_kernel(const GradJob* jobs, float* grad, int accumulate) {
  const GradJob j = jobs[blockIdx.y];
  float* dst = grad + j.dst_off;
  for (long i = (long)blockIdx.x * 256 + threadIdx.x; i < j.count; i += (long)gridDim.x * 256) {
    float v;
    long di = i;
    if (j.kind == 3) {
      const double* s = static_cast<const double*>(j.src);
      double t = 0.0;
      for (int r = 0; r < NREP; ++r) t += s[(long)r * j.stride + j.off + i];
      v = (float)t;
    } else {
      const float* s = static_cast<const float*>(j.src);
      long si;
      if (j.kind == 0) {
        si = i;
      } else if (j.kind == 1) {
        const long mc_n = (long)j.M * j.C;
        const int tap = (int)(i / mc_n);
        const long mc = i - (long)tap * mc_n;
        si = i;
        di = mc * 27 + tap;
      } else {
        const int tap = (int)(i % 343);
        const long mc = i / 343;
        const int c = (int)(mc % j.C), m = (int)(mc / j.C);
        si = ((long)c * j.M + m) * 352 + tap;
      }
      float t = 0.f;
      int sp = 0;
      for (; sp + 8 <= j.nsplit; sp += 8) {
        float u[8];
#pragma unroll
        for (int k = 0; k < 8; ++k) u[k] = s[(long)(sp + k) * j.stride + si];
#pragma unroll
        for (int k = 0; k < 8; ++k) t += u[k];
      }
      for (; sp < j.nsplit; ++sp) t += s[(long)sp * j.stride + si];
      v = t;
    }
    dst[di] = accumulate ? dst[di] + v : v;
  }
}

int launch_finalize(const GradJob* jobs_dev, int njobs, long max_count, float* grad, int accumulate, hipStream_t stream) {
  if (njobs <= 0) return 0;
  MMNN_REQUIRE(njobs <= 65535 && grad, "finalize: bad arguments");
  int gx = cdiv(max_count, 256 * 2);
  if (gx < 1) gx = 1;
  if (gx > 128) gx = 128;
  MMNN_LAUNCH(finalize_kernel, dim3(gx, njobs), dim3(256), 0, stream, jobs_dev, grad, accumulate);
  MMNN_HIP(hipGetLastError());
  return 0;
}

__global__ void __launch_bounds__(256) sgd_kernel(float* p, const float* g, float* buf, long n, float lr, float mom, float wd, int nesterov, int first) {
  for (long i = ((long)blockIdx.x * 256 + threadIdx.x) * 4; i < n; i += (long)gridDim.x * 1024) {
    if (i + 3 < n && ((((uintptr_t)p | (uintptr_t)g | (uintptr_t)buf) & 15) == 0)) {
      f32x4 pv = *reinterpret_cast<f32x4*>(p + i), gv = *reinterpret_cast<const f32x4*>(g + i);
      f32x4 bv = first ? f32x4{0.f, 0.f, 0.f, 0.f} : *reinterpret_cast<f32x4*>(buf + i);
#pragma unroll
      for (int e = 0; e < 4; ++e) {
        float d = fmaf(wd, pv[e], gv[e]);
        const float b = first ? d : fmaf(mom, bv[e], d);
        bv[e] = b;
        d = nesterov ? fmaf(mom, b, d) : b;
        pv[e] = fmaf(-lr, d, pv[e]);
      }
      *reinterpret_cast<f32x4*>(p + i) = pv;
      *reinterpret_cast<f32x4*>(buf + i) = bv;
    } else {
      for (long j = i; j < n && j < i + 4; ++j) {
        float d = fmaf(wd, p[j], g[j]);
        const float b = first ? d : fmaf(mom, buf[j], d);
        buf[j] = b;
        d = nesterov ? fmaf(mom, b, d) : b;
        p[j] = fmaf(-lr, d, p[j]);
      }
    }
  }
}

int launch_sgd(float* p, const float* g, float* buf, long n, float lr, float momentum, float weight_decay, int nesterov, int first_step,
               hipStream_t stream) {
  MMNN_REQUIRE(p && g && buf && n > 0, "sgd: bad arguments");
  int gx = cdiv(n, 1024);
  if (gx > 2048) gx = 2048;
  MMNN_LAUNCH(sgd_kernel, dim3(gx), dim3(256), 0, stream, p, g, buf, n, lr, momentum, weight_decay, nesterov, first_step);
  MMNN_HIP(hipGetLastError());
  return 0;
}

struct MultiTable {
  int n;
  float* p[MMNN_MULTI_MAX]; const float* g[MMNN_MULTI_MAX]; long count[MMNN_MULTI_MAX]; long off[MMNN_MULTI_MAX]; int first[MMNN_MULTI_MAX];
};

__global__ void __launch_bounds__(256) sgd_multi_kernel(const MultiTable t, float* buf, float lr, float mom, float wd, int nesterov) {
  const int k = blockIdx.y;
  float* p = t.p[k]; const float* g = t.g[k]; float* b = buf + t.off[k];
  const bool first = t.first[k] != 0;
  for (long i = (long)blockIdx.x * 256 + threadIdx.x; i < t.count[k]; i += (long)gridDim.x * 256) {
    float d = fmaf(wd, p[i], g[i]);
    const float m = first ? d : fmaf(mom, b[i], d);
    b[i] = m;
    d = nesterov ? fmaf(mom, m, d) : m;
    p[i] = fmaf(-lr, d, p[i]);
  }
}

int launch_sgd_multi(const mmnn_tensor_ref* refs, int n, float* buf, float lr, float momentum, float weight_decay, int nesterov, hipStream_t stream) {
  MMNN_REQUIRE(refs && buf && n >= 1 && n <= MMNN_MULTI_MAX, "sgd_multi: 1..%d tensors per call, got %d", MMNN_MULTI_MAX, n);
  MultiTable t;
  t.n = n;
  long most = 0;
  for (int i = 0; i < n; ++i) {
    MMNN_REQUIRE(refs[i].param && refs[i].grad && refs[i].count > 0 && refs[i].flat_offset >= 0, "sgd_multi: bad tensor %d", i);
    t.p[i] = refs[i].param; t.g[i] = refs[i].grad; t.count[i] = refs[i].count; t.off[i] = refs[i].flat_offset; t.first[i] = refs[i].first_step;
    most = std::max(most, (long)refs[i].count);
  }
  int gx = cdiv(most, 256);
  if (gx > 64) gx = 64;
  MMNN_LAUNCH(sgd_multi_kernel, dim3(gx, n), dim3(256), 0, stream, t, buf, lr, momentum, weight_decay, nesterov);
  MMNN_HIP(hipGetLastError());
  return 0;
}

__global__ void __launch_bounds__(256) multi_copy_kernel(const MultiTable t, float* flat, int scatter) {
  const int k = blockIdx.y;
  float* g = const_cast<float*>(t.g[k]); float* f = flat + t.off[k];
  for (long i = (long)blockIdx.x * 256 + threadIdx.x; i < t.count[k]; i += (long)gridDim.x * 256) {
    if (scatter) g[i] = f[i]; else f[i] = g[i];
  }
}

int launch_multi_copy(const mmnn_tensor_ref* refs, int n, float* flat, int scatter, hipStream_t stream) {
  MMNN_REQUIRE(refs && flat && n >= 1 && n <= MMNN_MULTI_MAX, "multi_copy: 1..%d tensors per call, got %d", MMNN_MULTI_MAX, n);
  MultiTable t;
  t.n = n;
  long most = 0;
  for (int i = 0; i < n; ++i) {
    MMNN_REQUIRE(refs[i].grad && refs[i].count > 0 && refs[i].flat_offset >= 0, "multi_copy: bad tensor %d", i);
    t.p[i] = nullptr; t.g[i] = refs[i].grad; t.count[i] = refs[i].count; t.off[i] = refs[i].flat_offset; t.first[i] = 0;
    most = std::max(most, (long)refs[i].count);
  }
  int gx = cdiv(most, 256);
  if (gx > 64) gx = 64;
  MMNN_LAUNCH(multi_copy_kernel, dim3(gx, n), dim3(256), 0, stream, t, flat, scatter);
  MMNN_HIP(hipGetLastError());
  return 0;
}

__global__ void __launch_bounds__(256) poison_lds_kernel(int words) {
  extern __shared__ unsigned poison[];
  volatile unsigned* q = poison;
  for (int i = threadIdx.x; i < words; i += 256) q[i] = 0xFFFFFFFFu;
}

void debug_poison_lds(hipStream_t stream) {
  static const int on = [] { const char* e = getenv("MMNN_POISON_LDS"); return (e && e[0] == '1') ? 1 : 0; }();
  if (!on) return;
  constexpr int BYTES = 160 * 1024;
  static const bool ready =
      hipFuncSetAttribute(reinterpret_cast<const void*>(poison_lds_kernel), hipFuncAttributeMaxDynamicSharedMemorySize, BYTES) == hipSuccess;
  if (!ready) return;
  hipLaunchKernelGGL(poison_lds_kernel, dim3(1024), dim3(256), BYTES, stream, BYTES / 4);
}

}
```

### mmnn_sts_amd/csrc/fprop.hpp

```cpp
#pragma once
#include "common.hpp"

namespace mmnn {

#if !defined(MMNN_KZ_FENCED)
#if defined(__gfx950__) || !defined(__HIP_DEVICE_COMPILE__)
#define MMNN_KZ_FENCED 0
#else
#define MMNN_KZ_FENCED 1
#endif
#endif

enum Pro { PRO_NONE = 0, PRO_BNRELU = 1, PRO_GRAD = 2 };
enum Epi { EPI_STORE = 0, EPI_STORE_STATS = 1, EPI_MASK_STORE = 2, EPI_MASK_ACCUM = 3 };

struct FpropArgs {
  int N, D, H, W;
  int Cin, M;
  const float* in0; long in0_ns; int in0_coff;
  const float* in1; long in1_ns; int in1_coff;
  BnFwd bn_in;
  BnBwd gr_in;
  DropCfg drop_in;
  const float* w; int w_ld;
  float* out; long out_ns; int out_coff;
  DropCfg drop_out;
  StatPtr st_out;
  const float* ex; long ex_ns; int ex_coff;
  BnFwd ebn;
  double* dgamma; double* dbeta;
  StatPtr s_acc;
  int nrep;
  float* kz_part; unsigned* kz_cnt;
  size_t kz_part_bytes; unsigned kz_cnt_entries;
  const float* pf_ptr; unsigned pf_bytes;
  unsigned mg_w, mg_h, mg_d;
  unsigned long long* trace;
};

int launch_fprop(const FpropArgs& a, int taps, int pro, int epi, hipStream_t stream);
int current_device_slot();
constexpr int MAX_DEVICES = 32;

#if defined(__HIPCC__)

template <int TAPS, int PRO, int EPI, int WM, int WN, int KS, int MT, int NT, int KC, int TD, int TH, int TW, bool SPEC = false>
struct FpropCfg {
  static constexpr int NWAVES = WM * WN * KS;
  static constexpr int NCOMPUTE = NWAVES * 64;
  static constexpr int NTHREADS = NCOMPUTE * (SPEC ? 2 : 1);
  static constexpr int M_B = WM * MT * 32;
  static constexpr int V_B = WN * NT * 32;
  static constexpr int RS = (TAPS == 27) ? TW + 8 : TW;
  static constexpr int HS = (TAPS == 27) ? TH + 2 : 1;
  static constexpr int DS = (TAPS == 27) ? TD + 2 : 1;
  static constexpr int XS = DS * HS * RS;
  static constexpr int NCOEF = (PRO == PRO_BNRELU) ? 2 : (PRO == PRO_GRAD ? 3 : 0);
  static constexpr int ECOEF = 6 + 2 * WN;
  static_assert(TD * TH * TW == V_B, "tile volume must equal the block's voxel count");
  static_assert(KC % 2 == 0 && (KC / 2) % KS == 0, "channel-pair count of a chunk must be a multiple of the K-split");
  static constexpr int STAGE = KC * XS + KC * TAPS * M_B;
  static constexpr bool DIST = (MT * NT == 1) && KS > 1 && !SPEC;
  static constexpr int REDN = (DIST ? KS : KS - 1) * WM * WN * MT * NT * 1024;
  static constexpr int BUF0 = ((SPEC ? 2 : 1) * STAGE) > REDN ? ((SPEC ? 2 : 1) * STAGE) : REDN;
  static constexpr bool WIDE = (EPI == EPI_MASK_STORE || EPI == EPI_MASK_ACCUM || (EPI == EPI_STORE_STATS && !(TAPS == 27 && WM * WN > 1))) && !SPEC;
  static constexpr int TSTRIDE = 36;
  static constexpr int TRANS = WIDE ? WM * WN * 32 * TSTRIDE : 0;
  static constexpr int BUF = BUF0 > TRANS ? BUF0 : TRANS;
  static size_t smem_bytes(int Cin) {
    int cpad = ((Cin + KC - 1) / KC) * KC;
    size_t ncoef = ((size_t)NCOEF * cpad + 3) & ~(size_t)3;
    return sizeof(float) * (ncoef + (size_t)BUF + (size_t)ECOEF * M_B + 4);
  }
};

template <int PRO>
__device__ __forceinline__ float pro_apply(const float* coef, int cpad, int c, float x0, float x1) {
  if (PRO == PRO_BNRELU) return fmaxf(fmaf(coef[c], x0, coef[cpad + c]), 0.f);
  if (PRO == PRO_GRAD) return fmaf(coef[c], x0, fmaf(coef[cpad + c], x1, coef[2 * cpad + c]));
  return x0;
}

template <int R>
__device__ __forceinline__ float half_reduce_n(const float (&v)[R], int lane) {
  static_assert(R == 2 || R == 4 || R == 8, "half_reduce_n: 2, 4 or 8 registers");
  float w[R];
#pragma unroll
  for (int r = 0; r < R; ++r) w[r] = v[r];
  if (R >= 8) {
    const bool b = lane & 16;
#pragma unroll
    for (int r = 0; r < 4; ++r) { const float send = b ? w[r] : w[r + 4], keep = b ? w[r + 4] : w[r]; w[r] = keep + swz_xor<16>(send); }
  }
  if (R >= 4) {
    constexpr int X = (R == 8) ? 8 : 16;
    const bool b = lane & X;
#pragma unroll
    for (int r = 0; r < 2; ++r) { const float send = b ? w[r] : w[r + 2], keep = b ? w[r + 2] : w[r]; w[r] = keep + swz_xor<X>(send); }
  }
  {
    constexpr int X = (R == 8) ? 4 : (R == 4 ? 8 : 16);
    const bool b = lane & X;
    const float send = b ? w[0] : w[1], keep = b ? w[1] : w[0];
    w[0] = keep + swz_xor<X>(send);
  }
  float t = w[0];
  if (R <= 2) t += swz_xor<8>(t);
  if (R <= 4) t += swz_xor<4>(t);
  t += swz_xor<2>(t);
  t += swz_xor<1>(t);
  return t;
}

template <int TAPS, int PRO, int EPI, int WM, int WN, int KS, int MT, int NT, int KC, int TD, int TH, int TW, bool SPEC = false>
__global__ void __launch_bounds__(WM* WN* KS * 64 * (SPEC ? 2 : 1)) fprop_kernel(const FpropArgs a) {
  using C = FpropCfg<TAPS, PRO, EPI, WM, WN, KS, MT, NT, KC, TD, TH, TW, SPEC>;
  constexpr int NL = C::NCOMPUTE;
  constexpr int NTHREADS = C::NTHREADS, M_B = C::M_B, V_B = C::V_B, RS = C::RS, HS = C::HS, DS = C::DS, XS = C::XS;
  extern __shared__ __attribute__((aligned(16))) float smem[];
  const int tid = threadIdx.x, lane = tid & 63;
#if defined(MMNN_PHASE_TRACE)
  const bool tracing = a.trace != nullptr && tid == 0 && blockIdx.x < 64 && blockIdx.y == 0;
#else
  constexpr bool tracing = false;
#endif
  auto stamp = [&](int k) {
    if (tracing) a.trace[(blockIdx.x * (gridDim.z > 1 ? 2 : 1) + (blockIdx.z ? 1 : 0)) % 64 * 16 + k] = __builtin_amdgcn_s_memtime();
  };
  stamp(0);
  kernarg_warm<sizeof(FpropArgs)>();
  stamp(13);
  float pf_sink = 0.f, pf_sink2 = 0.f;
  const bool loader = SPEC && tid >= NL;
  const int ltid = loader ? tid - NL : tid;
  const int wave = ltid >> 6;
  const int half = lane >> 5, l31 = lane & 31;
  const int kg = wave / (WM * WN);
  const int wm = (wave % (WM * WN)) / WN, wn = wave % WN;
  const int V = a.D * a.H * a.W;
  const int cpad = ((a.Cin + KC - 1) / KC) * KC;

  float* coef = smem;
  float* Xs = coef + ((C::NCOEF * cpad + 3) & ~3);
  float* Ws = Xs + KC * XS;
  float* ecoef = Xs + C::BUF;

  int n, d0 = 0, h0 = 0, w0 = 0, v0_ = 0;
  {
    int b = blockIdx.x;
    if (TAPS == 27 && (gridDim.x & 7) == 0) b = (b & 7) * (int)(gridDim.x >> 3) + (b >> 3);
    auto divmod = [](int& x, int d, unsigned magic) {
      const int q = magic ? (int)__umulhi((unsigned)x, magic) : x;
      const int r = x - q * d;
      x = q;
      return r;
    };
    if (TAPS == 27) {
      const int nw = (a.W + TW - 1) / TW, nh = (a.H + TH - 1) / TH, nd = (a.D + TD - 1) / TD;
      w0 = divmod(b, nw, a.mg_w) * TW;
      h0 = divmod(b, nh, a.mg_h) * TH;
      d0 = divmod(b, nd, a.mg_d) * TD;
      n = b;
    } else {
      const int nt = (V + V_B - 1) / V_B;
      v0_ = divmod(b, nt, a.mg_w) * V_B;
      n = b;
    }
  }
  const int m0 = blockIdx.y * M_B;
  const int rep = blockIdx.x & ((a.nrep > 0 ? a.nrep : NREP) - 1);
  const int kz = gridDim.z, nch_all = (a.Cin + KC - 1) / KC;
  const int kz_sh = __builtin_ctz((unsigned)kz);
  const int c_begin = ((nch_all * (int)blockIdx.z) >> kz_sh) * KC;
  const int c_end = min(a.Cin, ((nch_all * ((int)blockIdx.z + 1)) >> kz_sh) * KC);

  constexpr bool EARLY_K = (MT * NT == 1) || (TAPS == 27 && TW <= 16);
  constexpr bool MASK_E = (EPI == EPI_MASK_STORE || EPI == EPI_MASK_ACCUM);
  static_assert(!EARLY_K || M_B <= NTHREADS, "one epilogue row per thread");
  const int c_hi = min(cpad, c_begin + ((c_end - c_begin + KC - 1) / KC) * KC);
  bool fastp = EARLY_K && (c_hi - c_begin) <= NTHREADS;
  if (PRO == PRO_BNRELU) fastp = fastp && a.bn_in.training && a.bn_in.st.nrep <= 2;
  if (PRO == PRO_GRAD) fastp = fastp && a.gr_in.st.nrep <= 2 && a.gr_in.s.nrep <= 2;
  if (MASK_E) fastp = fastp && a.ebn.training && a.ebn.st.nrep <= 2;
  BnFwdRaw raw_in, raw_e;
  BnBwdRaw raw_gr;
  if (EARLY_K && fastp) {
    const int pc = max(0, min(c_begin + tid, a.Cin - 1)), pm = max(0, min(m0 + tid, a.M - 1));
    if (PRO != PRO_NONE && c_begin + (tid & ~63) < c_hi) {
      if (PRO == PRO_BNRELU) bn_fwd_issue(a.bn_in, pc, raw_in);
      if (PRO == PRO_GRAD) bn_bwd_issue(a.gr_in, pc, raw_gr);
    }
    if (MASK_E && (tid & ~63) < M_B) bn_fwd_issue(a.ebn, pm, raw_e);
  }
  stamp(14);
  auto prologue_fast = [&]() {
    const int c = c_begin + tid;
    if (c < c_hi) {
      if (PRO == PRO_BNRELU) {
        float ca = 0.f, cb = 0.f, mu, rs;
        bn_fwd_finish(a.bn_in, raw_in, ca, cb, mu, rs);
        const bool ok = c < a.Cin;
        coef[c] = ok ? ca : 0.f; coef[cpad + c] = ok ? cb : 0.f;
      } else if (PRO == PRO_GRAD) {
        float p = 0.f, q = 0.f, r = 0.f;
        bn_bwd_finish(a.gr_in, raw_gr, p, q, r);
        const bool ok = c < a.Cin;
        const float sc = drop_scale(a.drop_in, n, c);
        coef[c] = ok ? p * sc : 0.f; coef[cpad + c] = ok ? q * sc : 0.f; coef[2 * cpad + c] = ok ? r * sc : 0.f;
      }
    }
    if (tid < M_B) {
      const int m = tid;
      float ea = 0.f, eb = 0.f, mu = 0.f, rs = 0.f, g = 0.f, ds = 1.f;
      if (m0 + m < a.M) {
        if (MASK_E) {
          bn_fwd_finish(a.ebn, raw_e, ea, eb, mu, rs);
          g = raw_e.g;
        }
        if (EPI == EPI_STORE_STATS) ds = drop_scale(a.drop_out, n, m0 + m);
      }
      ecoef[m] = ea; ecoef[M_B + m] = eb; ecoef[2 * M_B + m] = mu; ecoef[3 * M_B + m] = rs;
      ecoef[4 * M_B + m] = g; ecoef[5 * M_B + m] = ds;
    }
    __syncthreads();
  };

  auto prologue = [&]() {
    if (PRO == PRO_BNRELU) {
      for (int c = c_begin + tid; c < min(cpad, c_begin + ((c_end - c_begin + KC - 1) / KC) * KC); c += NTHREADS) {
        float ca = 0.f, cb = 0.f, mu, rs;
        if (c < a.Cin) bn_fwd_coef(a.bn_in, c, ca, cb, mu, rs);
        coef[c] = ca; coef[cpad + c] = cb;
      }
    } else if (PRO == PRO_GRAD) {
      for (int c = c_begin + tid; c < min(cpad, c_begin + ((c_end - c_begin + KC - 1) / KC) * KC); c += NTHREADS) {
        float p = 0.f, q = 0.f, r = 0.f;
        if (c < a.Cin) {
          bn_bwd_coef(a.gr_in, c, p, q, r);
          const float s = drop_scale(a.drop_in, n, c);
          p *= s; q *= s; r *= s;
        }
        coef[c] = p; coef[cpad + c] = q; coef[2 * cpad + c] = r;
      }
    }
    for (int m = tid; m < M_B; m += NTHREADS) {
      float ea = 0.f, eb = 0.f, mu = 0.f, rs = 0.f, g = 0.f, ds = 1.f;
      if (m0 + m < a.M) {
        if (EPI == EPI_MASK_STORE || EPI == EPI_MASK_ACCUM) {
          bn_fwd_coef(a.ebn, m0 + m, ea, eb, mu, rs);
          g = a.ebn.gamma[m0 + m];
        }
        if (EPI == EPI_STORE_STATS) ds = drop_scale(a.drop_out, n, m0 + m);
      }
      ecoef[m] = ea; ecoef[M_B + m] = eb; ecoef[2 * M_B + m] = mu; ecoef[3 * M_B + m] = rs;
      ecoef[4 * M_B + m] = g; ecoef[5 * M_B + m] = ds;
    }
    __syncthreads();
  };

  f32x16 acc[MT][NT];
#pragma unroll
  for (int i = 0; i < MT; ++i)
#pragma unroll
    for (int j = 0; j < NT; ++j)
#pragma unroll
      for (int r = 0; r < 16; ++r) acc[i][j][r] = 0.f;

  int pos[NT];
#pragma unroll
  for (int j = 0; j < NT; ++j) {
    const int t = (wn * NT + j) * 32 + l31;
    if (TAPS == 27) {
      const int wx = t % TW, hy = (t / TW) % TH, dz = t / (TW * TH);
      pos[j] = (dz * HS + hy) * RS + wx + 3;
    } else {
      pos[j] = t;
    }
  }

  const float* in0n = a.in0 + (long)n * a.in0_ns + (long)a.in0_coff * V;
  const float* in1n = (PRO == PRO_GRAD) ? a.in1 + (long)n * a.in1_ns + (long)a.in1_coff * V : nullptr;
  const bool al_x = (((uintptr_t)in0n | (uintptr_t)in1n) & 15) == 0;
  const bool vecx = al_x && ((TAPS == 27) ? ((a.W & 3) == 0) : ((V & 3) == 0));
  const bool vecw = ((a.w_ld & 3) == 0) && ((a.M & 3) == 0) && (((uintptr_t)a.w & 15) == 0);

  auto mfma_chunk = [&](int boff = 0) {
    const float* xb = Xs + boff + (2 * kg + half) * XS;
    const float* wb = Ws + boff + (2 * kg + half) * TAPS * M_B + wm * MT * 32 + l31;
    constexpr int PAIR = 2 * KS;
    constexpr int NSTEP = (KC / 2 / KS) * TAPS;
    auto rd = [&](int st, float (&av)[MT], float (&bv)[NT]) {
      const int jj = st / TAPS, tap = st % TAPS;
      const int toff = (TAPS == 27) ? (((tap / 9) * HS + (tap / 3) % 3) * RS + tap % 3) : 0;
#pragma unroll
      for (int i = 0; i < MT; ++i) av[i] = wb[(jj * PAIR * TAPS + tap) * M_B + i * 32];
#pragma unroll
      for (int j = 0; j < NT; ++j) bv[j] = xb[jj * PAIR * XS + pos[j] + toff];
    };
    auto mm = [&](const float (&av)[MT], const float (&bv)[NT]) {
#pragma unroll
      for (int i = 0; i < MT; ++i)
#pragma unroll
        for (int j = 0; j < NT; ++j) acc[i][j] = __builtin_amdgcn_mfma_f32_32x32x2f32(av[i], bv[j], acc[i][j], 0, 0, 0);
    };
    float a0[MT], b0[NT], a1[MT], b1[NT];
    rd(0, a0, b0);
#pragma unroll
    for (int st = 0; st < NSTEP; st += 2) {
      if (st + 1 < NSTEP) rd(st + 1, a1, b1);
      __builtin_amdgcn_sched_group_barrier(0x100, MT + NT, 0);
      mm(a0, b0);
      __builtin_amdgcn_sched_group_barrier(0x008, MT * NT, 0);
      if (st + 2 < NSTEP) rd(st + 2, a0, b0);
      __builtin_amdgcn_sched_group_barrier(0x100, MT + NT, 0);
      if (st + 1 < NSTEP) mm(a1, b1);
      __builtin_amdgcn_sched_group_barrier(0x008, MT * NT, 0);
    }
  };

  float* outn = a.out + (long)n * a.out_ns + (long)a.out_coff * V;
  const float* exn = (EPI == EPI_MASK_STORE || EPI == EPI_MASK_ACCUM) ? a.ex + (long)n * a.ex_ns + (long)a.ex_coff * V : nullptr;
  constexpr bool ALL_ROWS = (EPI == EPI_MASK_STORE);
  float xall[ALL_ROWS ? MT : 1][ALL_ROWS ? 16 : 1][NT];
  bool xall_loaded = false;
  auto load_xall = [&]() {
    if (ALL_ROWS) {
      int vox[NT];
      bool vok[NT];
#pragma unroll
      for (int j = 0; j < NT; ++j) {
        const int t = (wn * NT + j) * 32 + l31;
        if (TAPS == 27) {
          const int wx = t % TW, hy = (t / TW) % TH, dz = t / (TW * TH);
          const int d = d0 + dz, h = h0 + hy, w = w0 + wx;
          vok[j] = d < a.D && h < a.H && w < a.W;
          vox[j] = (d * a.H + h) * a.W + w;
        } else {
          vox[j] = v0_ + t;
          vok[j] = vox[j] < V;
        }
      }
#pragma unroll
      for (int i = 0; i < MT; ++i)
#pragma unroll
        for (int q = 0; q < 16; ++q) {
          const int ml = wm * MT * 32 + i * 32 + acc_row(q, half);
          const bool mok = (m0 + ml) < a.M;
#pragma unroll
          for (int j = 0; j < NT; ++j) {
            const unsigned o = (mok && vok[j]) ? (unsigned)(m0 + ml) * (unsigned)V + (unsigned)vox[j] : 0u;
            xall[ALL_ROWS ? i : 0][ALL_ROWS ? q : 0][j] = exn[o];
          }
        }
    }
    xall_loaded = true;
  };
  constexpr bool XPRE = false && ALL_ROWS && TAPS == 27 && TW > 16 && MT * NT > 1 && !SPEC;
  const bool xall_early = XPRE && gridDim.z == 1 && kg == 0 && !loader;

  if (vecx && vecw && (long)KC * V < (1l << 30)) {
    constexpr int ROWS = (TAPS == 27) ? KC * DS * HS : KC;
    constexpr int VPR = (TAPS == 27) ? TW / 4 : V_B / 4;
    constexpr int XV_ITEMS = ROWS * VPR;
    constexpr int XH_ITEMS = (TAPS == 27) ? ROWS * 2 : 0;
    constexpr int W_ITEMS = KC * TAPS * (M_B / 4);
    constexpr int XV_IT = (XV_ITEMS + NL - 1) / NL, XH_IT = (XH_ITEMS + NL - 1) / NL;
    constexpr int W_IT = (W_ITEMS + NL - 1) / NL;
    static_assert(XV_IT <= 32 && XH_IT <= 32 && W_IT <= 32, "validity bits of the staged items are kept in 32-bit masks");
    constexpr bool GR = (PRO == PRO_GRAD);
    constexpr int PF = (MT * NT == 1) ? 2 : 1;
    struct Stage {
      f32x4 xv0[XV_IT], xv1[GR ? XV_IT : 1], wr[W_IT];
      float xh0[XH_IT > 0 ? XH_IT : 1], xh1[(GR && XH_IT > 0) ? XH_IT : 1];
      unsigned okv, okh, okw;
    };
    Stage stA, stB;

    int xv_off[XV_IT], xv_dst[XV_IT], xv_cl[XV_IT];
    int xh_off[XH_IT > 0 ? XH_IT : 1], xh_dst[XH_IT > 0 ? XH_IT : 1], xh_cl[XH_IT > 0 ? XH_IT : 1];
    int w_off[W_IT], w_cl[W_IT];
#pragma unroll
    for (int i = 0; i < W_IT; ++i) {
      const int it = ltid + i * NL;
      const int q = it % (M_B / 4), kr = it / (M_B / 4);
      const bool ok = (it < W_ITEMS) && (m0 + 4 * q < a.M);
      w_off[i] = ok ? kr * a.w_ld + m0 + 4 * q : -1;
      w_cl[i] = kr / TAPS;
    }
    const bool w_nomask = (a.Cin % KC == 0) && (m0 + M_B <= a.M);
    auto load_w = [&](int c0, Stage& st) {
      const int crem = a.Cin - c0;
      const float* bw = a.w + (long)c0 * TAPS * a.w_ld;
      unsigned okw = 0;
#pragma unroll
      for (int i = 0; i < W_IT; ++i) {
        const bool ok = w_off[i] >= 0 && w_cl[i] < crem;
        okw |= (ok ? 1u : 0u) << i;
        st.wr[i] = *reinterpret_cast<const f32x4*>(ok ? bw + w_off[i] : a.w);
      }
      st.okw = okw;
    };
    constexpr bool EARLY = (MT * NT == 1) || (TAPS == 27 && TW <= 16);
    const bool first_chunk_mine = (c_begin < c_end) && (!SPEC || loader);
    if (EARLY && first_chunk_mine) load_w(c_begin, stA);
    stamp(15);
    {
      auto row_info = [&](int r, int& cl, int& lrow, int& gro, bool& rowok) {
        if (TAPS == 27) {
          const int hy = r % HS, dz = (r / HS) % DS;
          cl = r / (HS * DS);
          const int d = d0 + dz - 1, h = h0 + hy - 1;
          rowok = (unsigned)d < (unsigned)a.D && (unsigned)h < (unsigned)a.H;
          gro = cl * V + (d * a.H + h) * a.W;
          lrow = cl * XS + (dz * HS + hy) * RS;
        } else {
          cl = r;
          rowok = true;
          gro = cl * V;
          lrow = cl * XS;
        }
      };
#pragma unroll
      for (int i = 0; i < XV_IT; ++i) {
        const int it = ltid + i * NL;
        int cl, lrow, gro; bool rowok;
        row_info(it / VPR, cl, lrow, gro, rowok);
        const int col = ((TAPS == 27) ? w0 : v0_) + 4 * (it % VPR);
        const bool ok = (it < XV_ITEMS) && rowok && col < ((TAPS == 27) ? a.W : V);
        xv_off[i] = ok ? gro + col : -1;
        xv_dst[i] = lrow + ((TAPS == 27) ? 4 : 0) + 4 * (it % VPR);
        xv_cl[i] = cl;
      }
#pragma unroll
      for (int i = 0; i < XH_IT; ++i) {
        const int it = ltid + i * NL;
        int cl, lrow, gro; bool rowok;
        row_info(it >> 1, cl, lrow, gro, rowok);
        const int w = (it & 1) ? w0 + TW : w0 - 1;
        const bool ok = (it < XH_ITEMS) && rowok && (unsigned)w < (unsigned)a.W;
        xh_off[i] = ok ? gro + w : -1;
        xh_dst[i] = lrow + ((it & 1) ? TW + 4 : 3);
        xh_cl[i] = cl;
      }
    }

    auto load_x = [&](int c0, Stage& st) {
      unsigned okv = 0, okh = 0;
      const float* b0 = in0n + (long)c0 * V;
      const float* b1 = GR ? in1n + (long)c0 * V : nullptr;
      const int crem = a.Cin - c0;
#pragma unroll
      for (int i = 0; i < XV_IT; ++i) {
        const bool ok = xv_off[i] >= 0 && xv_cl[i] < crem;
        const int off = ok ? xv_off[i] : 0;
        okv |= (ok ? 1u : 0u) << i;
        st.xv0[i] = *reinterpret_cast<const f32x4*>(ok ? b0 + off : in0n);
        if (GR) st.xv1[i] = *reinterpret_cast<const f32x4*>(ok ? b1 + off : in1n);
      }
#pragma unroll
      for (int i = 0; i < XH_IT; ++i) {
        const bool ok = xh_off[i] >= 0 && xh_cl[i] < crem;
        const int off = ok ? xh_off[i] : 0;
        okh |= (ok ? 1u : 0u) << i;
        st.xh0[i] = *(ok ? b0 + off : in0n);
        if (GR) st.xh1[i] = *(ok ? b1 + off : in1n);
      }
      st.okv = okv; st.okh = okh;
    };

    auto load_chunk = [&](int c0, Stage& st) { load_x(c0, st); load_w(c0, st); };
    auto load_first = [&](Stage& st) { if (EARLY) load_x(c_begin, st); else load_chunk(c_begin, st); };

    auto store_chunk = [&](int c0, const Stage& st, int boff = 0) {
      const unsigned okv = st.okv, okh = st.okh;
#pragma unroll
      for (int i = 0; i < XV_IT; ++i) {
        if (ltid + i * NL < XV_ITEMS) {
          f32x4 o;
#pragma unroll
          for (int e = 0; e < 4; ++e) o[e] = pro_apply<PRO>(coef, cpad, c0 + xv_cl[i], st.xv0[i][e], GR ? st.xv1[i][e] : 0.f);
          if (!((okv >> i) & 1u)) o = f32x4{0.f, 0.f, 0.f, 0.f};
          *reinterpret_cast<f32x4*>(Xs + boff + xv_dst[i]) = o;
        }
      }
#pragma unroll
      for (int i = 0; i < XH_IT; ++i) {
        if (ltid + i * NL < XH_ITEMS) {
          const float o = pro_apply<PRO>(coef, cpad, c0 + xh_cl[i], st.xh0[i], GR ? st.xh1[i] : 0.f);
          Xs[boff + xh_dst[i]] = ((okh >> i) & 1u) ? o : 0.f;
        }
      }
      if (w_nomask) {
#pragma unroll
        for (int i = 0; i < W_IT; ++i) {
          const int it = ltid + i * NL;
          if (it < W_ITEMS) *reinterpret_cast<f32x4*>(Ws + boff + 4 * it) = st.wr[i];
        }
      } else {
#pragma unroll
        for (int i = 0; i < W_IT; ++i) {
          const int it = ltid + i * NL;
          if (it < W_ITEMS) *reinterpret_cast<f32x4*>(Ws + boff + 4 * it) = ((st.okw >> i) & 1u) ? st.wr[i] : f32x4{0.f, 0.f, 0.f, 0.f};
        }
      }
    };

    if (!EARLY) prologue();
    auto prefetch_next_weights = [&]() {
      const unsigned lines = a.pf_bytes >> 7;
      if (a.pf_ptr == nullptr || lines == 0) return;
      const unsigned lin = blockIdx.x + gridDim.x * (blockIdx.y + gridDim.y * blockIdx.z);
      const unsigned per_xcd = (gridDim.x * gridDim.y * gridDim.z + 7u) >> 3;
      const unsigned ln0 = (lin >> 3) * NTHREADS + tid, ln1 = ln0 + per_xcd * NTHREADS;
      pf_sink = a.pf_ptr[(size_t)min(ln0, lines - 1) * 32];
      pf_sink2 = a.pf_ptr[(size_t)min(ln1, lines - 1) * 32];
    };
    if (SPEC) {
      if (loader && c_begin < c_end) load_first(stA);
      stamp(1);
      if (EARLY) { if (fastp) prologue_fast(); else prologue(); }
      prefetch_next_weights();
      stamp(2);
      if (loader && c_begin < c_end) store_chunk(c_begin, stA, 0);
      __syncthreads();
      stamp(9);
      int k = 0;
      for (int c0 = c_begin; c0 < c_end; c0 += KC, ++k) {
        if (loader) {
          if (c0 + KC < c_end) { load_chunk(c0 + KC, stA); store_chunk(c0 + KC, stA, ((k + 1) & 1) * C::STAGE); }
        } else {
          mfma_chunk((k & 1) * C::STAGE);
        }
        __syncthreads();
      }
    } else if (PF == 1) {
      if (c_begin < c_end) load_first(stA);
      stamp(1);
      if (EARLY) { if (fastp) prologue_fast(); else prologue(); }
      prefetch_next_weights();
      stamp(2);
      for (int c0 = c_begin; c0 < c_end; c0 += KC) {
        store_chunk(c0, stA);
        __syncthreads();
        if (c0 == c_begin) stamp(9);
        if (c0 + KC < c_end) load_chunk(c0 + KC, stA);
        else if (XPRE && xall_early) load_xall();
        mfma_chunk();
        __syncthreads();
      }
    } else {
      if (c_begin < c_end) load_first(stA);
      if (c_begin + KC < c_end) load_chunk(c_begin + KC, stB);
      stamp(1);
      if (EARLY) { if (fastp) prologue_fast(); else prologue(); }
      prefetch_next_weights();
      stamp(2);
      for (int c0 = c_begin; c0 < c_end; c0 += 2 * KC) {
        store_chunk(c0, stA);
        __syncthreads();
        if (c0 == c_begin) stamp(9);
        if (c0 + 2 * KC < c_end) load_chunk(c0 + 2 * KC, stA);
        mfma_chunk();
        __syncthreads();
        if (c0 + KC < c_end) {
          store_chunk(c0 + KC, stB);
          __syncthreads();
          if (c0 + 3 * KC < c_end) load_chunk(c0 + 3 * KC, stB);
          mfma_chunk();
          __syncthreads();
        }
      }
    }
  } else {
  prologue();
  for (int c0 = c_begin; c0 < c_end; c0 += KC) {
    if (TAPS == 27) {
      if (vecx) {
        constexpr int IPR = TW / 4 + 2;
        constexpr int ITEMS = KC * DS * HS * IPR;
        for (int it = tid; it < ITEMS; it += NTHREADS) {
          const int q = it % IPR;
          int row = it / IPR;
          const int hy = row % HS; row /= HS;
          const int dz = row % DS;
          const int cl = row / DS;
          const int c = c0 + cl;
          const int d = d0 + dz - 1, h = h0 + hy - 1;
          const bool rowok = (c < a.Cin) && (unsigned)d < (unsigned)a.D && (unsigned)h < (unsigned)a.H;
          float* dst = Xs + cl * XS + (dz * HS + hy) * RS;
          const long gro = (long)c * V + ((long)d * a.H + h) * a.W;
          if (q < TW / 4) {
            const int w = w0 + 4 * q;
            f32x4 o = {0.f, 0.f, 0.f, 0.f};
            if (rowok && w < a.W) {
              f32x4 x0 = *reinterpret_cast<const f32x4*>(in0n + gro + w);
              f32x4 x1 = x0;
              if (PRO == PRO_GRAD) x1 = *reinterpret_cast<const f32x4*>(in1n + gro + w);
#pragma unroll
              for (int e = 0; e < 4; ++e) o[e] = pro_apply<PRO>(coef, cpad, c, x0[e], x1[e]);
            }
            *reinterpret_cast<f32x4*>(dst + 4 + 4 * q) = o;
          } else {
            const int w = (q == TW / 4) ? w0 - 1 : w0 + TW;
            float o = 0.f;
            if (rowok && (unsigned)w < (unsigned)a.W) {
              const float x0 = in0n[gro + w];
              const float x1 = (PRO == PRO_GRAD) ? in1n[gro + w] : x0;
              o = pro_apply<PRO>(coef, cpad, c, x0, x1);
            }
            dst[(q == TW / 4) ? 3 : TW + 4] = o;
          }
        }
      } else {
        constexpr int IPR = TW + 2;
        constexpr int ITEMS = KC * DS * HS * IPR;
        for (int it = tid; it < ITEMS; it += NTHREADS) {
          const int q = it % IPR;
          int row = it / IPR;
          const int hy = row % HS; row /= HS;
          const int dz = row % DS;
          const int cl = row / DS;
          const int c = c0 + cl;
          const int d = d0 + dz - 1, h = h0 + hy - 1, w = w0 + q - 1;
          float o = 0.f;
          if ((c < a.Cin) && (unsigned)d < (unsigned)a.D && (unsigned)h < (unsigned)a.H && (unsigned)w < (unsigned)a.W) {
            const long g = (long)c * V + ((long)d * a.H + h) * a.W + w;
            const float x0 = in0n[g];
            const float x1 = (PRO == PRO_GRAD) ? in1n[g] : x0;
            o = pro_apply<PRO>(coef, cpad, c, x0, x1);
          }
          Xs[cl * XS + (dz * HS + hy) * RS + 3 + q] = o;
        }
      }
    } else {
      if (vecx) {
        constexpr int ITEMS = KC * V_B / 4;
        for (int it = tid; it < ITEMS; it += NTHREADS) {
          const int q = it % (V_B / 4);
          const int cl = it / (V_B / 4);
          const int c = c0 + cl;
          const int v = v0_ + 4 * q;
          f32x4 o = {0.f, 0.f, 0.f, 0.f};
          if (c < a.Cin && v < V) {
            const long g = (long)c * V + v;
            f32x4 x0 = *reinterpret_cast<const f32x4*>(in0n + g);
            f32x4 x1 = x0;
            if (PRO == PRO_GRAD) x1 = *reinterpret_cast<const f32x4*>(in1n + g);
#pragma unroll
            for (int e = 0; e < 4; ++e) o[e] = pro_apply<PRO>(coef, cpad, c, x0[e], x1[e]);
          }
          *reinterpret_cast<f32x4*>(Xs + cl * XS + 4 * q) = o;
        }
      } else {
        constexpr int ITEMS = KC * V_B;
        for (int it = tid; it < ITEMS; it += NTHREADS) {
          const int q = it % V_B;
          const int cl = it / V_B;
          const int c = c0 + cl;
          const int v = v0_ + q;
          float o = 0.f;
          if (c < a.Cin && v < V) {
            const long g = (long)c * V + v;
            const float x0 = in0n[g];
            const float x1 = (PRO == PRO_GRAD) ? in1n[g] : x0;
            o = pro_apply<PRO>(coef, cpad, c, x0, x1);
          }
          Xs[cl * XS + q] = o;
        }
      }
    }
    {
      const int krows = KC * TAPS;
      const long kbase = (long)c0 * TAPS;
      const long klim = (long)a.Cin * TAPS;
      if (vecw) {
        const int items = krows * (M_B / 4);
        for (int it = tid; it < items; it += NTHREADS) {
          const int q = it % (M_B / 4);
          const int kr = it / (M_B / 4);
          const int m = m0 + 4 * q;
          f32x4 o = {0.f, 0.f, 0.f, 0.f};
          if (kbase + kr < klim && m < a.M) o = *reinterpret_cast<const f32x4*>(a.w + (kbase + kr) * a.w_ld + m);
          *reinterpret_cast<f32x4*>(Ws + kr * M_B + 4 * q) = o;
        }
      } else {
        const int items = krows * M_B;
        for (int it = tid; it < items; it += NTHREADS) {
          const int q = it % M_B;
          const int kr = it / M_B;
          float o = 0.f;
          if (kbase + kr < klim && m0 + q < a.M) o = a.w[(kbase + kr) * a.w_ld + m0 + q];
          Ws[kr * M_B + q] = o;
        }
      }
    }
    __syncthreads();
    if (!loader) mfma_chunk();
    __syncthreads();
  }
  }

  stamp(3);
  float* red0 = ecoef + 6 * M_B;
  float* red1 = red0 + WN * M_B;
  const bool want_sums = (EPI == EPI_STORE_STATS) ? (a.st_out.sum != nullptr) : (EPI != EPI_STORE);
  if constexpr (C::DIST) {
    constexpr int RP = 16 / KS, NSLOT = WM * WN;
    constexpr bool MASK = (EPI == EPI_MASK_STORE || EPI == EPI_MASK_ACCUM);
    float* rbuf = Xs;
    const int slot = wm * WN + wn;
#pragma unroll
    for (int r = 0; r < 16; ++r) rbuf[((kg * NSLOT + slot) * 16 + r) * 64 + lane] = acc[0][0][r];
    __syncthreads();
    float my[RP];
#pragma unroll
    for (int q = 0; q < RP; ++q) {
      float t = rbuf[((0 * NSLOT + slot) * 16 + kg * RP + q) * 64 + lane];
#pragma unroll
      for (int g = 1; g < KS; ++g) t += rbuf[((g * NSLOT + slot) * 16 + kg * RP + q) * 64 + lane];
      my[q] = t;
    }
    stamp(4);
    if (kz > 1) {
      const long tile_id = blockIdx.x + (long)gridDim.x * blockIdx.y;
      float* part = a.kz_part + (tile_id * kz) * NSLOT * 1024;
#pragma unroll
      for (int q = 0; q < RP; ++q) {
        float* dst = part + (((long)blockIdx.z * NSLOT + slot) * 16 + kg * RP + q) * 64 + lane;
#if MMNN_KZ_FENCED
        *dst = my[q];
#else
        __hip_atomic_store(dst, my[q], __ATOMIC_RELAXED, __HIP_MEMORY_SCOPE_AGENT);
#endif
      }
      asm volatile("s_waitcnt vmcnt(0)" ::: "memory");
      __syncthreads();
      unsigned* ticket = reinterpret_cast<unsigned*>(ecoef + C::ECOEF * M_B);
      if (tid == 0) {
#if MMNN_KZ_FENCED
        __builtin_amdgcn_fence(__ATOMIC_RELEASE, "agent");
        asm volatile("s_waitcnt vmcnt(0)" ::: "memory");
#endif
        *ticket = __hip_atomic_fetch_add(a.kz_cnt + tile_id, 1u, __ATOMIC_RELAXED, __HIP_MEMORY_SCOPE_AGENT);
      }
      __syncthreads();
      stamp(5);
      const unsigned arrived = *ticket;
      if (arrived != (unsigned)(kz - 1)) return;
      if (tid == 0) __hip_atomic_store(a.kz_cnt + tile_id, 0u, __ATOMIC_RELAXED, __HIP_MEMORY_SCOPE_AGENT);
#if MMNN_KZ_FENCED
      __builtin_amdgcn_fence(__ATOMIC_ACQUIRE, "agent");
#endif
      constexpr int ZB = (RP <= 4) ? 8 : 4;
#pragma unroll
      for (int q = 0; q < RP; ++q) my[q] = 0.f;
      for (int z0 = 0; z0 < kz; z0 += ZB) {
        float pz[ZB][RP];
#pragma unroll
        for (int z = 0; z < ZB; ++z) {
          const int zc = min(z0 + z, kz - 1);
#pragma unroll
          for (int q = 0; q < RP; ++q) {
            const float* sp = part + (((long)zc * NSLOT + slot) * 16 + kg * RP + q) * 64 + lane;
#if MMNN_KZ_FENCED
            pz[z][q] = *sp;
#else
            pz[z][q] = __hip_atomic_load(sp, __ATOMIC_RELAXED, __HIP_MEMORY_SCOPE_AGENT);
#endif
          }
        }
#pragma unroll
        for (int z = 0; z < ZB; ++z)
#pragma unroll
          for (int q = 0; q < RP; ++q) my[q] += (z0 + z < kz) ? pz[z][q] : 0.f;
      }
    }
    stamp(6);
    int vox; bool vok;
    {
      const int t = wn * 32 + l31;
      if (TAPS == 27) {
        const int wx = t % TW, hy = (t / TW) % TH, dz = t / (TW * TH);
        const int d = d0 + dz, h = h0 + hy, w = w0 + wx;
        vok = d < a.D && h < a.H && w < a.W;
        vox = (d * a.H + h) * a.W + w;
      } else {
        vox = v0_ + t;
        vok = vox < V;
      }
    }
    int ml[RP]; bool ok[RP]; unsigned off[RP];
    float xe[MASK ? RP : 1], go[(EPI == EPI_MASK_ACCUM) ? RP : 1];
#pragma unroll
    for (int q = 0; q < RP; ++q) {
      ml[q] = wm * 32 + acc_row(kg * RP + q, half);
      ok[q] = vok && (m0 + ml[q]) < a.M;
      off[q] = ok[q] ? (unsigned)(m0 + ml[q]) * (unsigned)V + (unsigned)vox : 0u;
      if (MASK) xe[MASK ? q : 0] = exn[off[q]];
      if (EPI == EPI_MASK_ACCUM) go[(EPI == EPI_MASK_ACCUM) ? q : 0] = outn[off[q]];
    }
    float s0[RP], s1[RP];
#pragma unroll
    for (int q = 0; q < RP; ++q) {
      float val = my[q], t0 = 0.f, t1 = 0.f;
      if (EPI == EPI_STORE) {
        if (ok[q]) outn[off[q]] = val;
      } else if (EPI == EPI_STORE_STATS) {
        val *= ecoef[5 * M_B + ml[q]];
        if (ok[q]) { outn[off[q]] = val; t0 = val; t1 = val * val; }
      } else {
        if (ok[q]) {
          const float x = xe[MASK ? q : 0];
          const float pre = fmaf(ecoef[ml[q]], x, ecoef[M_B + ml[q]]);
          const float z = pre > 0.f ? val : 0.f;
          const float xh = (x - ecoef[2 * M_B + ml[q]]) * ecoef[3 * M_B + ml[q]];
          t0 = z; t1 = z * xh;
          if (EPI == EPI_MASK_STORE) outn[off[q]] = z;
          else outn[off[q]] = go[(EPI == EPI_MASK_ACCUM) ? q : 0] + ecoef[4 * M_B + ml[q]] * z;
        }
      }
      s0[q] = t0; s1[q] = t1;
    }
    if (want_sums) {
      const float r0 = half_reduce_n<RP>(s0, lane), r1 = half_reduce_n<RP>(s1, lane);
      constexpr int SH = (RP == 8) ? 2 : (RP == 4 ? 3 : 4);
      if ((l31 & ((1 << SH) - 1)) == 0) {
        const int mrow = wm * 32 + acc_row(kg * RP + (l31 >> SH), half);
        red0[wn * M_B + mrow] = r0;
        red1[wn * M_B + mrow] = r1;
      }
    }
  } else {
  if (KS > 1) {
    float* rbuf = Xs;
    const int slot = (wm * WN + wn) * MT * NT;
    if (kg > 0 && !loader) {
#pragma unroll
      for (int i = 0; i < MT; ++i)
#pragma unroll
        for (int j = 0; j < NT; ++j)
#pragma unroll
          for (int r = 0; r < 16; ++r) rbuf[(((kg - 1) * WM * WN * MT * NT + slot + i * NT + j) * 16 + r) * 64 + lane] = acc[i][j][r];
    }
    __syncthreads();
    if (kg == 0 && !loader) {
#pragma unroll
      for (int g = 1; g < KS; ++g)
#pragma unroll
        for (int i = 0; i < MT; ++i)
#pragma unroll
          for (int j = 0; j < NT; ++j)
#pragma unroll
            for (int r = 0; r < 16; ++r) acc[i][j][r] += rbuf[(((g - 1) * WM * WN * MT * NT + slot + i * NT + j) * 16 + r) * 64 + lane];
    }
  }

  stamp(4);
  if (kz > 1) {
    constexpr int NSLOT = WM * WN * MT * NT;
    const long tile_id = blockIdx.x + (long)gridDim.x * blockIdx.y;
    float* part = a.kz_part + (tile_id * kz) * NSLOT * 1024;
    const int slot = (wm * WN + wn) * MT * NT;
    if (kg == 0 && !loader) {
#pragma unroll
      for (int i = 0; i < MT; ++i)
#pragma unroll
        for (int j = 0; j < NT; ++j)
#pragma unroll
          for (int r = 0; r < 16; ++r) {
            float* dst = part + (((long)blockIdx.z * NSLOT + slot + i * NT + j) * 16 + r) * 64 + lane;
#if MMNN_KZ_FENCED
            *dst = acc[i][j][r];
#else
            __hip_atomic_store(dst, acc[i][j][r], __ATOMIC_RELAXED, __HIP_MEMORY_SCOPE_AGENT);
#endif
          }
    }
    asm volatile("s_waitcnt vmcnt(0)" ::: "memory");
    __syncthreads();
    unsigned* ticket = reinterpret_cast<unsigned*>(ecoef + C::ECOEF * M_B);
    if (tid == 0) {
#if MMNN_KZ_FENCED
      __builtin_amdgcn_fence(__ATOMIC_RELEASE, "agent");
      asm volatile("s_waitcnt vmcnt(0)" ::: "memory");
#endif
      *ticket = __hip_atomic_fetch_add(a.kz_cnt + tile_id, 1u, __ATOMIC_RELAXED, __HIP_MEMORY_SCOPE_AGENT);
    }
    __syncthreads();
    stamp(5);
    const unsigned arrived = *ticket;
    if (arrived != (unsigned)(kz - 1)) return;
    if (tid == 0) __hip_atomic_store(a.kz_cnt + tile_id, 0u, __ATOMIC_RELAXED, __HIP_MEMORY_SCOPE_AGENT);
#if MMNN_KZ_FENCED
    __builtin_amdgcn_fence(__ATOMIC_ACQUIRE, "agent");
#endif
    if constexpr (KS > 1) {
      constexpr int RP = 16 / KS;
      constexpr int ZB = (RP <= 4) ? 8 : 4;
      float* xbuf = Xs;
      if (!loader) {
#pragma unroll
        for (int i = 0; i < MT; ++i)
#pragma unroll
          for (int j = 0; j < NT; ++j) {
            float sacc[RP];
#pragma unroll
            for (int q = 0; q < RP; ++q) sacc[q] = 0.f;
            for (int z0 = 0; z0 < kz; z0 += ZB) {
              float pz[ZB][RP];
#pragma unroll
              for (int z = 0; z < ZB; ++z) {
                const int zc = min(z0 + z, kz - 1);
#pragma unroll
                for (int q = 0; q < RP; ++q) {
                  const float* sp = part + (((long)zc * NSLOT + slot + i * NT + j) * 16 + kg * RP + q) * 64 + lane;
#if MMNN_KZ_FENCED
                  pz[z][q] = *sp;
#else
                  pz[z][q] = __hip_atomic_load(sp, __ATOMIC_RELAXED, __HIP_MEMORY_SCOPE_AGENT);
#endif
                }
              }
#pragma unroll
              for (int z = 0; z < ZB; ++z)
#pragma unroll
                for (int q = 0; q < RP; ++q) sacc[q] += (z0 + z < kz) ? pz[z][q] : 0.f;
            }
#pragma unroll
            for (int q = 0; q < RP; ++q) xbuf[((slot + i * NT + j) * 16 + kg * RP + q) * 64 + lane] = sacc[q];
          }
      }
      __syncthreads();
      if (kg == 0 && !loader) {
#pragma unroll
        for (int i = 0; i < MT; ++i)
#pragma unroll
          for (int j = 0; j < NT; ++j)
#pragma unroll
            for (int r = 0; r < 16; ++r) acc[i][j][r] = xbuf[((slot + i * NT + j) * 16 + r) * 64 + lane];
      }
    } else {
    if (kg == 0 && !loader) {
#pragma unroll
      for (int i = 0; i < MT; ++i)
#pragma unroll
        for (int j = 0; j < NT; ++j) {
#pragma unroll
          for (int r = 0; r < 16; ++r) acc[i][j][r] = 0.f;
          for (int z = 0; z < kz; z += 2) {
            float p0[16], p1[16];
#pragma unroll
            for (int r = 0; r < 16; ++r) {
              const float* s0 = part + (((long)z * NSLOT + slot + i * NT + j) * 16 + r) * 64 + lane;
              const float* s1 = part + (((long)(z + 1) * NSLOT + slot + i * NT + j) * 16 + r) * 64 + lane;
#if MMNN_KZ_FENCED
              p0[r] = *s0; p1[r] = *s1;
#else
              p0[r] = __hip_atomic_load(s0, __ATOMIC_RELAXED, __HIP_MEMORY_SCOPE_AGENT);
              p1[r] = __hip_atomic_load(s1, __ATOMIC_RELAXED, __HIP_MEMORY_SCOPE_AGENT);
#endif
            }
#pragma unroll
            for (int r = 0; r < 16; ++r) acc[i][j][r] = (acc[i][j][r] + p0[r]) + p1[r];
          }
        }
    }
    }
  }

  stamp(6);
  if (C::WIDE && KS > 1) __syncthreads();

  int vox[NT];
  bool vok[NT];
#pragma unroll
  for (int j = 0; j < NT; ++j) {
    const int t = (wn * NT + j) * 32 + l31;
    if (TAPS == 27) {
      const int wx = t % TW, hy = (t / TW) % TH, dz = t / (TW * TH);
      const int d = d0 + dz, h = h0 + hy, w = w0 + wx;
      vok[j] = d < a.D && h < a.H && w < a.W;
      vox[j] = (d * a.H + h) * a.W + w;
    } else {
      vox[j] = v0_ + t;
      vok[j] = vox[j] < V;
    }
  }

  if (kg == 0 && !loader) {
  constexpr bool MASK = (EPI == EPI_MASK_STORE || EPI == EPI_MASK_ACCUM);
  const bool wide_ok = C::WIDE && (V & 3) == 0 && ((TAPS == 27) ? ((a.W & 3) == 0) : true) && ((((uintptr_t)outn | (uintptr_t)exn) & 15) == 0);
  if (C::WIDE && wide_ok) {
    float* tb = Xs + (wm * WN + wn) * (32 * C::TSTRIDE);
    const int q4 = 4 * (lane & 7), rl = lane >> 3;
#pragma unroll
    for (int i = 0; i < MT; ++i) {
      f32x4 vt[NT][4], xq[MASK ? NT : 1][4], gq[(EPI == EPI_MASK_ACCUM) ? NT : 1][4];
      unsigned off[NT][4];
      bool okq[NT][4];
#pragma unroll
      for (int j = 0; j < NT; ++j) {
        const int t = (wn * NT + j) * 32 + q4;
        int vq; bool vk;
        if (TAPS == 27) {
          const int wx = t % TW, hy = (t / TW) % TH, dz = t / (TW * TH);
          const int d = d0 + dz, h = h0 + hy, w = w0 + wx;
          vk = d < a.D && h < a.H && w < a.W;
          vq = (d * a.H + h) * a.W + w;
        } else {
          vq = v0_ + t;
          vk = vq < V;
        }
        __builtin_amdgcn_fence(__ATOMIC_ACQ_REL, "wavefront");
        __builtin_amdgcn_wave_barrier();
#pragma unroll
        for (int r = 0; r < 16; ++r) tb[acc_row(r, half) * C::TSTRIDE + l31] = acc[i][j][r];
        __builtin_amdgcn_fence(__ATOMIC_ACQ_REL, "wavefront");
        __builtin_amdgcn_wave_barrier();
#pragma unroll
        for (int k = 0; k < 4; ++k) {
          const int ml = wm * MT * 32 + i * 32 + rl + 8 * k;
          vt[j][k] = *reinterpret_cast<const f32x4*>(tb + (rl + 8 * k) * C::TSTRIDE + q4);
          okq[j][k] = vk && (m0 + ml) < a.M;
          off[j][k] = okq[j][k] ? (unsigned)(m0 + ml) * (unsigned)V + (unsigned)vq : 0u;
        }
      }
#pragma unroll
      for (int j = 0; j < NT; ++j)
#pragma unroll
        for (int k = 0; k < 4; ++k) {
          if (MASK) xq[MASK ? j : 0][k] = *reinterpret_cast<const f32x4*>(exn + off[j][k]);
          if (EPI == EPI_MASK_ACCUM) gq[(EPI == EPI_MASK_ACCUM) ? j : 0][k] = *reinterpret_cast<const f32x4*>(outn + off[j][k]);
        }
      float s0[4], s1[4];
#pragma unroll
      for (int k = 0; k < 4; ++k) {
        const int ml = wm * MT * 32 + i * 32 + rl + 8 * k;
        const float ea = ecoef[ml], eb = ecoef[M_B + ml], mu = ecoef[2 * M_B + ml], rs = ecoef[3 * M_B + ml], gm = ecoef[4 * M_B + ml];
        const float ds = ecoef[5 * M_B + ml];
        float t0 = 0.f, t1 = 0.f;
#pragma unroll
        for (int j = 0; j < NT; ++j) {
          if (okq[j][k]) {
            f32x4 o;
#pragma unroll
            for (int e = 0; e < 4; ++e) {
              if (MASK) {
                const float x = xq[MASK ? j : 0][k][e];
                const float pre = fmaf(ea, x, eb);
                const float z = pre > 0.f ? vt[j][k][e] : 0.f;
                const float xh = (x - mu) * rs;
                t0 += z;
                t1 += z * xh;
                o[e] = (EPI == EPI_MASK_STORE) ? z : gq[(EPI == EPI_MASK_ACCUM) ? j : 0][k][e] + gm * z;
              } else {
                const float val = vt[j][k][e] * ds;
                t0 += val;
                t1 += val * val;
                o[e] = val;
              }
            }
            *reinterpret_cast<f32x4*>(outn + off[j][k]) = o;
          }
        }
        s0[k] = t0; s1[k] = t1;
      }
      if (want_sums) {
#pragma unroll
        for (int k = 0; k < 4; ++k) {
          float r0 = s0[k], r1 = s1[k];
          r0 += swz_xor<1>(r0); r1 += swz_xor<1>(r1);
          r0 += swz_xor<2>(r0); r1 += swz_xor<2>(r1);
          r0 += swz_xor<4>(r0); r1 += swz_xor<4>(r1);
          if ((lane & 7) == 0) {
            const int ml = wm * MT * 32 + i * 32 + rl + 8 * k;
            red0[wn * M_B + ml] = r0;
            red1[wn * M_B + ml] = r1;
          }
        }
      }
    }
  } else {
  if (ALL_ROWS && !(XPRE && xall_loaded)) load_xall();
#pragma unroll
  for (int i = 0; i < MT; ++i) {
    float s0[16], s1[16];
    float xe[(MASK && !ALL_ROWS) ? 16 : 1][NT], go[(EPI == EPI_MASK_ACCUM) ? 16 : 1][NT];
    if (MASK && !ALL_ROWS) {
#pragma unroll
      for (int q = 0; q < 16; ++q) {
        const int ml = wm * MT * 32 + i * 32 + acc_row(q, half);
        const bool mok = (m0 + ml) < a.M;
#pragma unroll
        for (int j = 0; j < NT; ++j) {
          const unsigned o = (mok && vok[j]) ? (unsigned)(m0 + ml) * (unsigned)V + (unsigned)vox[j] : 0u;
          xe[(MASK && !ALL_ROWS) ? q : 0][j] = exn[o];
          if (EPI == EPI_MASK_ACCUM) go[(EPI == EPI_MASK_ACCUM) ? q : 0][j] = outn[o];
        }
      }
    }
#pragma unroll
    for (int r = 0; r < 16; ++r) {
      const int ml = wm * MT * 32 + i * 32 + acc_row(r, half);
      const bool mok = (m0 + ml) < a.M;
      float t0 = 0.f, t1 = 0.f;
#pragma unroll
      for (int j = 0; j < NT; ++j) {
        const bool ok = mok && vok[j];
        const unsigned o = (unsigned)(m0 + ml) * (unsigned)V + (unsigned)vox[j];
        float val = acc[i][j][r];
        if (EPI == EPI_STORE) {
          if (ok) outn[o] = val;
        } else if (EPI == EPI_STORE_STATS) {
          val *= ecoef[5 * M_B + ml];
          if (ok) {
            outn[o] = val;
            t0 += val;
            t1 += val * val;
          }
        } else {
          if (ok) {
            const float x = ALL_ROWS ? xall[ALL_ROWS ? i : 0][ALL_ROWS ? r : 0][j] : xe[(MASK && !ALL_ROWS) ? r : 0][j];
            const float pre = fmaf(ecoef[ml], x, ecoef[M_B + ml]);
            const float z = pre > 0.f ? val : 0.f;
            const float xh = (x - ecoef[2 * M_B + ml]) * ecoef[3 * M_B + ml];
            t0 += z;
            t1 += z * xh;
            if (EPI == EPI_MASK_STORE) outn[o] = z;
            else outn[o] = go[(EPI == EPI_MASK_ACCUM) ? r : 0][j] + ecoef[4 * M_B + ml] * z;
          }
        }
      }
      s0[r] = t0;
      s1[r] = t1;
    }
    if (want_sums) {
      const float r0 = half_reduce16(s0, lane);
      const float r1 = half_reduce16(s1, lane);
      if ((lane & 1) == 0) {
        const int ml = wm * MT * 32 + i * 32 + acc_row((l31 >> 1) & 15, half);
        red0[wn * M_B + ml] = r0;
        red1[wn * M_B + ml] = r1;
      }
    }
  }
  }
  }
  }
  stamp(7);
  if (want_sums) {
    __syncthreads();
    for (int m = tid; m < M_B; m += NTHREADS) {
      if (m0 + m >= a.M) continue;
      double v0d = 0.0, v1d = 0.0;
#pragma unroll
      for (int j = 0; j < WN; ++j) { v0d += (double)red0[j * M_B + m]; v1d += (double)red1[j * M_B + m]; }
      if (EPI == EPI_STORE_STATS) {
        atomicAdd(a.st_out.sum + (long)rep * a.st_out.stride + a.st_out.off + m0 + m, v0d);
        atomicAdd(a.st_out.sq + (long)rep * a.st_out.stride + a.st_out.off + m0 + m, v1d);
      } else {
        atomicAdd(a.dbeta + (long)rep * a.M + m0 + m, v0d);
        atomicAdd(a.dgamma + (long)rep * a.M + m0 + m, v1d);
        if (EPI == EPI_MASK_ACCUM) {
          const double g = (double)ecoef[4 * M_B + m];
          atomicAdd(a.s_acc.sum + (long)rep * a.s_acc.stride + a.s_acc.off + m0 + m, g * v0d);
          atomicAdd(a.s_acc.sq + (long)rep * a.s_acc.stride + a.s_acc.off + m0 + m, g * v1d);
        }
      }
    }
  }
  if (pf_sink + pf_sink2 == 1.2345678e-33f) a.out[0] = pf_sink;
  stamp(8);
  if (tracing) {
    a.trace[10] = ((unsigned long long)TAPS << 48) | ((unsigned long long)PRO << 40) | ((unsigned long long)EPI << 32) | ((unsigned long long)a.M << 16) | (unsigned long long)a.Cin;
    a.trace[11] = ((unsigned long long)gridDim.x << 32) | ((unsigned long long)gridDim.y << 16) | gridDim.z;
    a.trace[12] = ((unsigned long long)(WM * WN * KS) << 32) | ((unsigned long long)KC << 16) | (unsigned long long)(MT * NT);
  }
}

#endif
}
```

Measured before the change: 256.4 volumes/s (whole job; 1 volume = 1 patient = stacked T1+T2 2x128^3 + 32 tabular).

## Pre-split activations and weights into bf16x3 planes outside the conv3 kernels

Moves the BN-ReLU (or BN-backward) prologue and the three-way bf16 split of activations into a separate pass that writes hi/mid/lo planes to a workspace buffer. The conv3 fwd and dgrad kernels then load those planes directly. Weights are likewise pre-split during the packing step into new panels, so the split arithmetic leaves the MFMA inner loops. The intent is to cut per-tile VALU work and redundant splitting of halo voxels, at the cost of an extra elementwise launch per conv and extra global traffic (three 16-bit planes written and re-read instead of one fp32 read).

```diff
diff --git a/mmnn_sts_amd/csrc/bf16x3.hpp b/mmnn_sts_amd/csrc/bf16x3.hpp
--- /dev/null
+++ b/mmnn_sts_amd/csrc/bf16x3.hpp
@@ -0,0 +1,26 @@
+#pragma once
+#include "common.hpp"
+
+namespace mmnn {
+
+#if defined(__HIPCC__)
+__device__ __forceinline__ void split3(float x, __bf16& h, __bf16& m, __bf16& l) {
+  h = (__bf16)x;
+  const float r1 = x - (float)h;
+  m = (__bf16)r1;
+  l = (__bf16)(r1 - (float)m);
+}
+__device__ __forceinline__ uint32_t pack2(__bf16 lo, __bf16 hi) {
+  return (uint32_t)__builtin_bit_cast(unsigned short, lo) | ((uint32_t)__builtin_bit_cast(unsigned short, hi) << 16);
+}
+__device__ __forceinline__ void split3x8(const float (&v)[8], uint4& hi, uint4& mid, uint4& lo) {
+  __bf16 ph[8], pm[8], pl[8];
+#pragma unroll
+  for (int e = 0; e < 8; ++e) split3(v[e], ph[e], pm[e], pl[e]);
+  hi = make_uint4(pack2(ph[0], ph[1]), pack2(ph[2], ph[3]), pack2(ph[4], ph[5]), pack2(ph[6], ph[7]));
+  mid = make_uint4(pack2(pm[0], pm[1]), pack2(pm[2], pm[3]), pack2(pm[4], pm[5]), pack2(pm[6], pm[7]));
+  lo = make_uint4(pack2(pl[0], pl[1]), pack2(pl[2], pl[3]), pack2(pl[4], pl[5]), pack2(pl[6], pl[7]));
+}
+#endif
+
+}
diff --git a/mmnn_sts_amd/csrc/conv3_bf16x3.hip b/mmnn_sts_amd/csrc/conv3_bf16x3.hip
--- a/mmnn_sts_amd/csrc/conv3_bf16x3.hip
+++ b/mmnn_sts_amd/csrc/conv3_bf16x3.hip
@@ -1,6 +1,7 @@
 #include <stdlib.h>
 
 #include "fprop.hpp"
+#include "bf16x3.hpp"
 
 namespace mmnn {
 
@@ -14,23 +15,77 @@
   static constexpr int HD = TD + 2, HH = TH + 2, HW = TW + 2, HV = HD * HH * HW, ROWS = TD * TH * TW / 32;
   static constexpr int ITEMS = (2 * HV + 255) / 256;
   static constexpr size_t OPER_BYTES = (size_t)2 * 6 * HV * 16;
-  static constexpr size_t SMEM = OPER_BYTES + sizeof(float) * (2 * MAXC + 2 * 4 * 32 + 32);
+  static constexpr size_t SMEM = OPER_BYTES + sizeof(float) * (2 * 4 * 32 + 32);
   static_assert(TD * TH * TW % 32 == 0 && (TW == 32 || TW == 16), "rows of 32 voxels");
   static_assert(ITEMS <= NT, "one staging item per tap slot");
   static_assert(4 * ROWS * 16 * 64 * sizeof(float) <= OPER_BYTES, "the partial tiles are summed in the operand buffers");
   static_assert(SMEM <= 160 * 1024, "LDS");
 };
 
-__device__ __forceinline__ void split3(float x, __bf16& h, __bf16& m, __bf16& l) {
-  h = (__bf16)x;
-  const float r1 = x - (float)h;
-  m = (__bf16)r1;
-  l = (__bf16)(r1 - (float)m);
-}
-__device__ __forceinline__ uint32_t pack2(__bf16 lo, __bf16 hi) {
-  return (uint32_t)__builtin_bit_cast(unsigned short, lo) | ((uint32_t)__builtin_bit_cast(unsigned short, hi) << 16);
-}
 __device__ __forceinline__ bf16x8_t as_bf16x8(uint4 v) { return __builtin_bit_cast(bf16x8_t, v); }
+}
+
+__global__ void __launch_bounds__(256) conv3_split_bnrelu_kernel(const FpropArgs a) {
+  __shared__ float cf[2][8];
+  const int c8 = blockIdx.y, n = blockIdx.z, C8 = a.Cin / 8, V = a.D * a.H * a.W;
+  const int v = blockIdx.x * 256 + threadIdx.x;
+  const float* __restrict__ x = a.in0 + (long)n * a.in0_ns + (long)(a.in0_coff + 8 * c8) * V;
+  float xv[8];
+#pragma unroll
+  for (int e = 0; e < 8; ++e) xv[e] = v < V ? x[(long)e * V + v] : 0.f;
+  if (threadIdx.x < 8) {
+    float ca, cb, mu, rs;
+    bn_fwd_coef(a.bn_in, 8 * c8 + threadIdx.x, ca, cb, mu, rs);
+    cf[0][threadIdx.x] = ca; cf[1][threadIdx.x] = cb;
+  }
+  __syncthreads();
+  if (v >= V) return;
+#pragma unroll
+  for (int e = 0; e < 8; ++e) xv[e] = fmaxf(fmaf(cf[0][e], xv[e], cf[1][e]), 0.f);
+  uint4 hi, mid, lo;
+  split3x8(xv, hi, mid, lo);
+  const long ps = (long)a.N * C8 * V;
+  uint4* __restrict__ dst = reinterpret_cast<uint4*>(a.x3) + ((long)n * C8 + c8) * V + v;
+  dst[0] = hi; dst[ps] = mid; dst[2 * ps] = lo;
+}
+
+__global__ void __launch_bounds__(256) conv3_split_bnbwd_kernel(const FpropArgs a) {
+  __shared__ float cf[3][8];
+  const int c8 = blockIdx.y, n = blockIdx.z, C8 = a.Cin / 8, V = a.D * a.H * a.W;
+  const int v = blockIdx.x * 256 + threadIdx.x;
+  const float* __restrict__ gn = a.in0 + (long)n * a.in0_ns + (long)(a.in0_coff + 8 * c8) * V;
+  const float* __restrict__ xn = a.in1 + (long)n * a.in1_ns + (long)(a.in1_coff + 8 * c8) * V;
+  float gv[8], xv[8];
+#pragma unroll
+  for (int e = 0; e < 8; ++e) {
+    gv[e] = v < V ? gn[(long)e * V + v] : 0.f;
+    xv[e] = v < V ? xn[(long)e * V + v] : 0.f;
+  }
+  if (threadIdx.x < 8) {
+    const int c = 8 * c8 + threadIdx.x;
+    float p_, q_, r_;
+    bn_bwd_coef(a.gr_in, c, p_, q_, r_);
+    const float sc = drop_scale(a.drop_in, n, c);
+    cf[0][threadIdx.x] = p_ * sc; cf[1][threadIdx.x] = q_ * sc; cf[2][threadIdx.x] = r_ * sc;
+  }
+  __syncthreads();
+  if (v >= V) return;
+#pragma unroll
+  for (int e = 0; e < 8; ++e) gv[e] = fmaf(cf[0][e], gv[e], fmaf(cf[1][e], xv[e], cf[2][e]));
+  uint4 hi, mid, lo;
+  split3x8(gv, hi, mid, lo);
+  const long ps = (long)a.N * C8 * V;
+  uint4* __restrict__ dst = reinterpret_cast<uint4*>(a.x3) + ((long)n * C8 + c8) * V + v;
+  dst[0] = hi; dst[ps] = mid; dst[2 * ps] = lo;
+}
+
+static int launch_split(bool bwd, const FpropArgs& a, hipStream_t stream) {
+  const int V = a.D * a.H * a.W;
+  const dim3 grid((unsigned)cdiv(V, 256), (unsigned)(a.Cin / 8), (unsigned)a.N);
+  if (bwd) MMNN_LAUNCH(conv3_split_bnbwd_kernel, grid, dim3(256), 0, stream, a);
+  else MMNN_LAUNCH(conv3_split_bnrelu_kernel, grid, dim3(256), 0, stream, a);
+  MMNN_HIP(hipGetLastError());
+  return 0;
 }
 
 template <int TD, int TH, int TW>
@@ -40,75 +95,64 @@
   constexpr int HH = G::HH, HW = G::HW, HV = G::HV, ROWS = G::ROWS, ITEMS = G::ITEMS;
   constexpr size_t OPER_BYTES = G::OPER_BYTES;
   extern __shared__ uint4 xs128[];
-  float* const coef = reinterpret_cast<float*>(reinterpret_cast<char*>(xs128) + OPER_BYTES);
-  float* const sred = coef + 2 * MAXC;
+  float* const sred = reinterpret_cast<float*>(reinterpret_cast<char*>(xs128) + OPER_BYTES);
   float* const dsc = sred + 2 * 4 * 32;
-  const int tid = threadIdx.x, lane = tid & 63, wv = tid >> 6, g = tid & 1;
-  const int D = a.D, H = a.H, W = a.W, V = D * H * W, Cin = a.Cin, nchunk = Cin / KC;
+  const int tid = threadIdx.x, lane = tid & 63, wv = tid >> 6;
+  const int D = a.D, H = a.H, W = a.W, V = D * H * W, C8 = a.Cin / 8, nchunk = a.Cin / KC;
   const int twn = (W + TW - 1) / TW, thn = (H + TH - 1) / TH, tdn = (D + TD - 1) / TD;
   int b = blockIdx.x;
   const int w0 = (b % twn) * TW; b /= twn;
   const int h0 = (b % thn) * TH; b /= thn;
   const int d0 = (b % tdn) * TD;
   const int n = b / tdn;
-  const float* __restrict__ xin = a.in0 + (long)n * a.in0_ns + (long)a.in0_coff * V;
-  const float* __restrict__ wgt = a.w;
-  for (int c = tid; c < Cin; c += 256) {
-    float ca_, cb_, mu, rs;
-    bn_fwd_coef(a.bn_in, c, ca_, cb_, mu, rs);
-    coef[c] = ca_; coef[MAXC + c] = cb_;
-  }
+  const long ps = (long)a.N * C8 * V;
+  const uint4* __restrict__ xin = reinterpret_cast<const uint4*>(a.x3) + (long)n * C8 * V;
+  const uint4* __restrict__ wp = reinterpret_cast<const uint4*>(a.w3);
   if (tid < 32) dsc[tid] = drop_scale(a.drop_out, n, tid);
   f32x16_t acc[ROWS];
 #pragma unroll
   for (int t = 0; t < ROWS; ++t)
 #pragma unroll
     for (int q = 0; q < 16; ++q) acc[t][q] = 0.f;
-  float xr[ITEMS][8], ca[8], cb[8];
-  auto item_pos = [&](int it, int& hv, int& o) -> bool {
+  uint4 xr[ITEMS][3];
+  auto item_pos = [&](int it, int& g, int& hv, int& o) -> bool {
     const int item = tid + it * 256;
-    hv = item >> 1;
+    g = item >= HV;
+    hv = item - g * HV;
     const int hd = hv / (HH * HW), hh = (hv / HW) % HH, hw = hv % HW;
     const int d = d0 + hd - 1, h = h0 + hh - 1, w = w0 + hw - 1;
     o = (d * H + h) * W + w;
     return item < 2 * HV && (unsigned)d < (unsigned)D && (unsigned)h < (unsigned)H && (unsigned)w < (unsigned)W;
   };
   auto issue = [&](int ch) {
-    const int c0 = ch * KC + 8 * g;
-#pragma unroll
-    for (int e = 0; e < 8; ++e) { ca[e] = coef[c0 + e]; cb[e] = coef[MAXC + c0 + e]; }
 #pragma unroll
     for (int it = 0; it < ITEMS; ++it) {
-      int hv, o;
-      const bool ok = item_pos(it, hv, o);
-#pragma unroll
-      for (int e = 0; e < 8; ++e) xr[it][e] = ok ? xin[(long)(c0 + e) * V + o] : 0.f;
+      int g, hv, o;
+      const bool ok = item_pos(it, g, hv, o);
+      const uint4* src = xin + (long)(2 * ch + g) * V + o;
+#pragma unroll
+      for (int p = 0; p < 3; ++p) xr[it][p] = ok ? src[p * ps] : make_uint4(0u, 0u, 0u, 0u);
     }
   };
   auto commit_item = [&](int it, int buf) {
-    int hv, o;
-    const bool ok = item_pos(it, hv, o);
+    int g, hv, o;
+    item_pos(it, g, hv, o);
     if (tid + it * 256 >= 2 * HV) return;
-    __bf16 ph[8], pm[8], pl[8];
-#pragma unroll
-    for (int e = 0; e < 8; ++e) split3(ok ? fmaxf(fmaf(ca[e], xr[it][e], cb[e]), 0.f) : 0.f, ph[e], pm[e], pl[e]);
     uint4* dst = xs128 + buf * (6 * HV);
-    dst[(0 * 2 + g) * HV + hv] = make_uint4(pack2(ph[0], ph[1]), pack2(ph[2], ph[3]), pack2(ph[4], ph[5]), pack2(ph[6], ph[7]));
-    dst[(1 * 2 + g) * HV + hv] = make_uint4(pack2(pm[0], pm[1]), pack2(pm[2], pm[3]), pack2(pm[4], pm[5]), pack2(pm[6], pm[7]));
-    dst[(2 * 2 + g) * HV + hv] = make_uint4(pack2(pl[0], pl[1]), pack2(pl[2], pl[3]), pack2(pl[4], pl[5]), pack2(pl[6], pl[7]));
-  };
-  float wr[NT][8];
+#pragma unroll
+    for (int p = 0; p < 3; ++p) dst[(p * 2 + g) * HV + hv] = xr[it][p];
+  };
+  bf16x8_t wr[NT][3];
   auto load_w = [&](int ti, int ch) {
     const int tap = wv + 4 * ti;
     if (tap < 27 && ch < nchunk) {
-      const int c0 = ch * KC + 8 * (lane >> 5);
-#pragma unroll
-      for (int e = 0; e < 8; ++e) wr[ti][e] = wgt[((long)(c0 + e) * 27 + tap) * a.w_ld + (lane & 31)];
+      const int c8 = 2 * ch + (lane >> 5);
+#pragma unroll
+      for (int p = 0; p < 3; ++p) wr[ti][p] = as_bf16x8(wp[((long)(p * 27 + tap) * C8 + c8) * 32 + (lane & 31)]);
     }
   };
 #pragma unroll
   for (int ti = 0; ti < NT; ++ti) load_w(ti, 0);
-  __syncthreads();
   issue(0);
 #pragma unroll
   for (int it = 0; it < ITEMS; ++it) commit_item(it, 0);
@@ -122,12 +166,9 @@
       const int tap = wv + 4 * ti;
       if (tap < 27) {
         const int td = tap / 9, th = (tap / 3) % 3, tw = tap % 3;
-        __bf16 ph[8], pm[8], pl[8];
-#pragma unroll
-        for (int e = 0; e < 8; ++e) split3(wr[ti][e], ph[e], pm[e], pl[e]);
         bf16x8_t aw[3];
 #pragma unroll
-        for (int e = 0; e < 8; ++e) { aw[0][e] = ph[e]; aw[1][e] = pm[e]; aw[2][e] = pl[e]; }
+        for (int p = 0; p < 3; ++p) aw[p] = wr[ti][p];
         load_w(ti, ch + 1);
 #pragma unroll
         for (int t = 0; t < ROWS; ++t) {
@@ -211,11 +252,10 @@
 __global__ void __launch_bounds__(256) conv3_dgrad_bf16x3_kernel(const FpropArgs a) {
   using namespace c3b;
   using G = Geo<2, 4, 32>;
-  constexpr int TH = 4, TW = 32, HH = G::HH, HW = G::HW, HV = G::HV, ROWS = G::ROWS, ITEMS = G::ITEMS, PF = 3;
+  constexpr int TH = 4, TW = 32, HH = G::HH, HW = G::HW, HV = G::HV, ROWS = G::ROWS, ITEMS = G::ITEMS, PF = 3, C8 = 4;
   extern __shared__ uint4 xs128[];
-  float* const coef = reinterpret_cast<float*>(reinterpret_cast<char*>(xs128) + G::OPER_BYTES);
-  float* const ecoef = coef + 96;
-  const int tid = threadIdx.x, lane = tid & 63, wv = tid >> 6, g = tid & 1;
+  float* const ecoef = reinterpret_cast<float*>(reinterpret_cast<char*>(xs128) + G::OPER_BYTES);
+  const int tid = threadIdx.x, lane = tid & 63, wv = tid >> 6;
   const int D = a.D, H = a.H, W = a.W, V = D * H * W;
   const int twn = (W + TW - 1) / TW, thn = (H + TH - 1) / TH, tdn = (D + 1) / 2;
   int b = blockIdx.x;
@@ -223,93 +263,74 @@
   const int h0 = (b % thn) * TH; b /= thn;
   const int d0 = (b % tdn) * 2;
   const int n = b / tdn;
-  const float* __restrict__ in0n = a.in0 + (long)n * a.in0_ns + (long)a.in0_coff * V;
-  const float* __restrict__ in1n = a.in1 + (long)n * a.in1_ns + (long)a.in1_coff * V;
-  const float* __restrict__ wgt = a.w;
-  if (tid < 32) {
-    float p_, q_, r_;
-    bn_bwd_coef(a.gr_in, tid, p_, q_, r_);
-    const float sc = drop_scale(a.drop_in, n, tid);
-    coef[tid] = p_ * sc; coef[32 + tid] = q_ * sc; coef[64 + tid] = r_ * sc;
-  }
+  const long ps = (long)a.N * C8 * V;
+  const uint4* __restrict__ xin = reinterpret_cast<const uint4*>(a.x3) + (long)n * C8 * V;
+  const uint4* __restrict__ wp = reinterpret_cast<const uint4*>(a.w3);
+  uint4 xr[ITEMS][3];
+  auto item_pos = [&](int it, int& g, int& hv, int& o) -> bool {
+    const int item = tid + it * 256;
+    g = item >= HV;
+    hv = item - g * HV;
+    const int hd = hv / (HH * HW), hh = (hv / HW) % HH, hw = hv % HW;
+    const int d = d0 + hd - 1, h = h0 + hh - 1, w = w0 + hw - 1;
+    o = (d * H + h) * W + w;
+    return item < 2 * HV && (unsigned)d < (unsigned)D && (unsigned)h < (unsigned)H && (unsigned)w < (unsigned)W;
+  };
+  auto issue = [&](int ch) {
+#pragma unroll
+    for (int it = 0; it < ITEMS; ++it) {
+      int g, hv, o;
+      const bool ok = item_pos(it, g, hv, o);
+      const uint4* src = xin + (long)(2 * ch + g) * V + o;
+#pragma unroll
+      for (int p = 0; p < 3; ++p) xr[it][p] = ok ? src[p * ps] : make_uint4(0u, 0u, 0u, 0u);
+    }
+  };
+  auto commit = [&](int buf) {
+#pragma unroll
+    for (int it = 0; it < ITEMS; ++it) {
+      int g, hv, o;
+      item_pos(it, g, hv, o);
+      if (tid + it * 256 < 2 * HV) {
+        uint4* dst = xs128 + buf * (6 * HV);
+#pragma unroll
+        for (int p = 0; p < 3; ++p) dst[(p * 2 + g) * HV + hv] = xr[it][p];
+      }
+    }
+  };
+  bf16x8_t wr[PF][3];
+  auto load_w = [&](int slot, int tap, int ch) {
+    if (ch < 2) {
+      const int c8 = 2 * ch + (lane >> 5);
+#pragma unroll
+      for (int p = 0; p < 3; ++p) wr[slot][p] = as_bf16x8(wp[((long)(p * 27 + tap) * C8 + c8) * 128 + wv * 32 + (lane & 31)]);
+    }
+  };
+#pragma unroll
+  for (int t = 0; t < PF; ++t) load_w(t, t, 0);
+  issue(0);
   if (tid >= 128) {
     const int m = tid - 128;
     float ea, eb, mu, rs;
     bn_fwd_coef(a.ebn, m, ea, eb, mu, rs);
     ecoef[m] = ea; ecoef[128 + m] = eb; ecoef[256 + m] = mu; ecoef[384 + m] = rs;
   }
-  float x0[2][ITEMS][8], x1[2][ITEMS][8];
-  auto item_pos = [&](int it, int& hv, int& o) -> bool {
-    const int item = tid + it * 256;
-    hv = item >> 1;
-    const int hd = hv / (HH * HW), hh = (hv / HW) % HH, hw = hv % HW;
-    const int d = d0 + hd - 1, h = h0 + hh - 1, w = w0 + hw - 1;
-    o = (d * H + h) * W + w;
-    return item < 2 * HV && (unsigned)d < (unsigned)D && (unsigned)h < (unsigned)H && (unsigned)w < (unsigned)W;
-  };
-  auto issue = [&](int ch) {
-    const int c0 = ch * KC + 8 * g;
-#pragma unroll
-    for (int it = 0; it < ITEMS; ++it) {
-      int hv, o;
-      const bool ok = item_pos(it, hv, o);
-#pragma unroll
-      for (int e = 0; e < 8; ++e) {
-        x0[ch][it][e] = ok ? in0n[(long)(c0 + e) * V + o] : 0.f;
-        x1[ch][it][e] = ok ? in1n[(long)(c0 + e) * V + o] : 0.f;
-      }
-    }
-  };
-  auto commit_item = [&](int it, int buf) {
-    int hv, o;
-    const bool ok = item_pos(it, hv, o);
-    if (tid + it * 256 >= 2 * HV) return;
-    const int c0 = buf * KC + 8 * g;
-    __bf16 ph[8], pm[8], pl[8];
-#pragma unroll
-    for (int e = 0; e < 8; ++e)
-      split3(ok ? fmaf(coef[c0 + e], x0[buf][it][e], fmaf(coef[32 + c0 + e], x1[buf][it][e], coef[64 + c0 + e])) : 0.f, ph[e], pm[e], pl[e]);
-    uint4* dst = xs128 + buf * (6 * HV);
-    dst[(0 * 2 + g) * HV + hv] = make_uint4(pack2(ph[0], ph[1]), pack2(ph[2], ph[3]), pack2(ph[4], ph[5]), pack2(ph[6], ph[7]));
-    dst[(1 * 2 + g) * HV + hv] = make_uint4(pack2(pm[0], pm[1]), pack2(pm[2], pm[3]), pack2(pm[4], pm[5]), pack2(pm[6], pm[7]));
-    dst[(2 * 2 + g) * HV + hv] = make_uint4(pack2(pl[0], pl[1]), pack2(pl[2], pl[3]), pack2(pl[4], pl[5]), pack2(pl[6], pl[7]));
-  };
-  float wr[PF][8];
-  auto load_w = [&](int slot, int tap, int ch) {
-    if (ch < 2) {
-      const int c0 = ch * KC + 8 * (lane >> 5);
-#pragma unroll
-      for (int e = 0; e < 8; ++e) wr[slot][e] = wgt[((long)(c0 + e) * 27 + tap) * a.w_ld + wv * 32 + (lane & 31)];
-    }
-  };
-#pragma unroll
-  for (int t = 0; t < PF; ++t) load_w(t, t, 0);
-  issue(0);
+  commit(0);
   issue(1);
   __syncthreads();
-#pragma unroll
-  for (int it = 0; it < ITEMS; ++it) commit_item(it, 0);
-#pragma unroll
-  for (int it = 0; it < ITEMS; ++it) commit_item(it, 1);
-  __syncthreads();
   f32x16_t acc[ROWS];
 #pragma unroll
   for (int t = 0; t < ROWS; ++t)
 #pragma unroll
     for (int q = 0; q < 16; ++q) acc[t][q] = 0.f;
-  for (int ch = 0; ch < 2; ++ch) {
-#pragma unroll 1
-    for (int tq = 0; tq < 9; ++tq) {
+  auto pair = [&](int ch, int tq) {
     const int td = tq / 3, th = tq % 3;
 #pragma unroll
     for (int tw = 0; tw < 3; ++tw) {
       const int tap = tq * 3 + tw;
-      __bf16 ph[8], pm[8], pl[8];
-#pragma unroll
-      for (int e = 0; e < 8; ++e) split3(wr[tw][e], ph[e], pm[e], pl[e]);
       bf16x8_t aw[3];
 #pragma unroll
-      for (int e = 0; e < 8; ++e) { aw[0][e] = ph[e]; aw[1][e] = pm[e]; aw[2][e] = pl[e]; }
+      for (int p = 0; p < 3; ++p) aw[p] = wr[tw][p];
       if (tq < 8) load_w(tw, tap + PF, ch); else load_w(tw, tw, ch + 1);
 #pragma unroll
       for (int t = 0; t < ROWS; ++t) {
@@ -325,8 +346,14 @@
         acc[t] = __builtin_amdgcn_mfma_f32_32x32x16_bf16(aw[0], bb[0], acc[t], 0, 0, 0);
       }
     }
-    }
-  }
+  };
+  pair(0, 0);
+  commit(1);
+  __syncthreads();
+#pragma unroll 1
+  for (int tq = 1; tq < 9; ++tq) pair(0, tq);
+#pragma unroll 1
+  for (int tq = 0; tq < 9; ++tq) pair(1, tq);
   const float* __restrict__ exn = a.ex + (long)n * a.ex_ns + (long)a.ex_coff * V;
   float* __restrict__ outn = a.out + (long)n * a.out_ns + (long)a.out_coff * V;
   float s0[16], s1[16];
@@ -387,6 +414,8 @@
   }
 }
 
+size_t conv3_bf16x3_plane_bytes(const FpropArgs& a) { return (size_t)3 * a.N * (a.Cin / 8) * a.D * a.H * a.W * 16; }
+
 bool conv3_dgrad_bf16x3_eligible(const FpropArgs& a) {
   static const int mode = [] { const char* e = getenv("MMNN_BF16X3_DGRAD"); return e ? atoi(e) : 1; }();
   static const int fmode = [] { const char* e = getenv("MMNN_BF16X3"); return e ? atoi(e) : 32; }();
@@ -395,10 +424,11 @@
 
 int launch_conv3_dgrad_bf16x3(const FpropArgs& a, hipStream_t stream) {
   using G = c3b::Geo<2, 4, 32>;
-  constexpr size_t SMEM = G::OPER_BYTES + sizeof(float) * (96 + 512);
+  constexpr size_t SMEM = G::OPER_BYTES + sizeof(float) * 512;
   static_assert(SMEM <= 160 * 1024, "LDS");
   MMNN_REQUIRE(conv3_dgrad_bf16x3_eligible(a), "conv3 dgrad bf16x3: shape not handled (M=%d, Cin=%d, W=%d)", a.M, a.Cin, a.W);
   MMNN_REQUIRE(a.in1 && a.ex && a.dgamma && a.dbeta, "conv3 dgrad bf16x3: operands missing");
+  MMNN_REQUIRE(a.w3 && a.x3 && a.x3_bytes >= conv3_bf16x3_plane_bytes(a), "conv3 dgrad bf16x3: pre-split weights or plane scratch missing");
   MMNN_REQUIRE((long)(a.M + 1) * a.D * a.H * a.W < (1l << 31), "conv3 dgrad bf16x3: volume too large for 32-bit element offsets");
   const long tiles = (long)a.N * cdiv(a.D, 2) * cdiv(a.H, 4) * cdiv(a.W, 32);
   MMNN_REQUIRE(tiles > 0 && tiles < (1l << 31), "conv3 dgrad bf16x3: grid out of range");
@@ -408,6 +438,7 @@
     MMNN_HIP(hipFuncSetAttribute(reinterpret_cast<const void*>(conv3_dgrad_bf16x3_kernel), hipFuncAttributeMaxDynamicSharedMemorySize, (int)SMEM));
     conf = true;
   }
+  if (int rc = launch_split(true, a, stream)) return rc;
   MMNN_LAUNCH(conv3_dgrad_bf16x3_kernel, dim3((unsigned)tiles), dim3(256), SMEM, stream, a);
   MMNN_HIP(hipGetLastError());
   return 0;
@@ -422,6 +453,7 @@
   using G = c3b::Geo<2, 4, 32>;
   MMNN_REQUIRE(conv3_fwd_bf16x3_eligible(a), "conv3 bf16x3: shape not handled (M=%d, Cin=%d, W=%d)", a.M, a.Cin, a.W);
   MMNN_REQUIRE(a.drop_in.p <= 0.f, "conv3 bf16x3: no input dropout on this path");
+  MMNN_REQUIRE(a.w3 && a.x3 && a.x3_bytes >= conv3_bf16x3_plane_bytes(a), "conv3 bf16x3: pre-split weights or plane scratch missing");
   MMNN_REQUIRE((long)(a.Cin + 1) * a.D * a.H * a.W < (1l << 31), "conv3 bf16x3: volume too large for 32-bit element offsets");
   const long tiles = (long)a.N * cdiv(a.D, 2) * cdiv(a.H, 4) * cdiv(a.W, 32);
   MMNN_REQUIRE(tiles > 0 && tiles < (1l << 31), "conv3 bf16x3: grid out of range");
@@ -431,6 +463,7 @@
     MMNN_HIP(hipFuncSetAttribute(reinterpret_cast<const void*>(conv3_fwd_bf16x3_kernel<2, 4, 32>), hipFuncAttributeMaxDynamicSharedMemorySize, (int)G::SMEM));
     conf = true;
   }
+  if (int rc = launch_split(false, a, stream)) return rc;
   MMNN_LAUNCH((conv3_fwd_bf16x3_kernel<2, 4, 32>), dim3((unsigned)tiles), dim3(256), G::SMEM, stream, a);
   MMNN_HIP(hipGetLastError());
   return 0;
diff --git a/mmnn_sts_amd/csrc/densenet.hip b/mmnn_sts_amd/csrc/densenet.hip
--- a/mmnn_sts_amd/csrc/densenet.hip
+++ b/mmnn_sts_amd/csrc/densenet.hip
@@ -127,14 +127,29 @@
   p.bstat_bytes = cv.cur - p.o_bstat;
   p.o_pk_conv0 = cv.take((size_t)7 * stem_krows(cfg.in_channels) * 64 * F);
   p.o_pk_c1.assign(nb, {}); p.o_pk_c2f.assign(nb, {}); p.o_pk_c2b.assign(nb, {}); p.o_pk_tr.clear();
+  p.o_pk_c2f3.assign(nb, {}); p.o_pk_c2b3.assign(nb, {});
+  p.x3_bytes = 0;
   for (int b = 0; b < nb; ++b) {
+    FpropArgs f, g;
+    memset(&f, 0, sizeof(f));
+    f.N = N; f.D = p.Db[b]; f.H = p.Hb[b]; f.W = p.Wb[b];
+    g = f;
+    f.Cin = p.mid; f.M = cfg.growth;
+    g.Cin = cfg.growth; g.M = p.mid;
+    const bool f3 = conv3_fwd_bf16x3_eligible(f), b3 = conv3_dgrad_bf16x3_eligible(g);
+    if (f3) p.x3_bytes = std::max(p.x3_bytes, conv3_bf16x3_plane_bytes(f));
+    if (b3) p.x3_bytes = std::max(p.x3_bytes, conv3_bf16x3_plane_bytes(g));
+    const size_t split_panel = (size_t)3 * cfg.growth * p.mid * 27 * sizeof(uint16_t);
     for (int l = 0; l < cfg.block_layers[b]; ++l) {
       p.o_pk_c1[b].push_back(cv.take((size_t)p.mid * p.layers[b][l].cin * F));
       p.o_pk_c2f[b].push_back(cv.take((size_t)cfg.growth * p.mid * 27 * F));
       p.o_pk_c2b[b].push_back(cv.take((size_t)cfg.growth * p.mid * 27 * F));
+      p.o_pk_c2f3[b].push_back(f3 ? cv.take(split_panel) : 0);
+      p.o_pk_c2b3[b].push_back(b3 ? cv.take(split_panel) : 0);
     }
     if (b != nb - 1) p.o_pk_tr.push_back(cv.take((size_t)p.trans[b].cin * p.trans[b].cout * F));
   }
+  p.o_x3 = p.x3_bytes ? cv.take(p.x3_bytes) : 0;
   p.ns_conv0 = stem_wgrad_pick_splits(N, p.D0, p.H0, p.W0, cfg.in_channels);
   p.o_sl_conv0 = cv.take((size_t)p.ns_conv0 * cfg.in_channels * cfg.init_features * 352 * F);
   p.o_sl_c1.assign(nb, {}); p.o_sl_c2.assign(nb, {}); p.ns_c1.assign(nb, {}); p.ns_c2.assign(nb, {});
@@ -166,7 +181,7 @@
   int nlayers = 0;
   for (int b = 0; b < nb; ++b) nlayers += cfg.block_layers[b];
   p.n_run_jobs = nbn;
-  p.n_pack_jobs = 1 + 3 * nlayers + (nb - 1);
+  p.n_pack_jobs = 1 + 5 * nlayers + (nb - 1);
   p.n_grad_jobs = 3 + 6 * nlayers + 3 * (nb - 1) + 2;
   p.o_jobs_run = cv.take(sizeof(RunStatJob) * p.n_run_jobs);
   p.o_jobs_pack = cv.take(sizeof(PackJob) * p.n_pack_jobs);
@@ -271,6 +286,8 @@
       pack_job(lo.c1, p.o_pk_c1[b][l], 0, p.mid, lo.cin, (long)p.mid * lo.cin);
       pack_job(lo.c2, p.o_pk_c2f[b][l], 1, c.growth, p.mid, (long)c.growth * p.mid * 27);
       pack_job(lo.c2, p.o_pk_c2b[b][l], 2, c.growth, p.mid, (long)c.growth * p.mid * 27);
+      if (p.o_pk_c2f3[b][l]) pack_job(lo.c2, p.o_pk_c2f3[b][l], 5, c.growth, p.mid, (long)27 * (p.mid / 8) * c.growth);
+      if (p.o_pk_c2b3[b][l]) pack_job(lo.c2, p.o_pk_c2b3[b][l], 6, c.growth, p.mid, (long)27 * (c.growth / 8) * p.mid);
       grad_bn(p.o_dg_n1[b][l], lo.cin, lo.n1w, lo.n1b);
       grad_slab(0, p.o_sl_c1[b][l], (long)p.mid * lo.cin, p.ns_c1[b][l], p.mid, lo.cin, lo.c1, (long)p.mid * lo.cin);
       grad_bn(p.o_dg_n2[b][l], p.mid, lo.n2w, lo.n2b);
@@ -426,7 +443,8 @@
       a.out = fptr(ws, p.o_t1[b][l]); a.out_ns = (long)p.mid * p.Vb[b]; a.out_coff = 0;
       a.st_out = statptr(ws, p.o_st_t1[b][l], p.mid, 0, p.nrep_b[b]);
       if (!training) a.st_out.sum = nullptr;
-      a.pf_ptr = fptr(ws, p.o_pk_c2f[b][l]); a.pf_bytes = (unsigned)(sizeof(float) * c.growth * p.mid * 27);
+      if (p.o_pk_c2f3[b][l]) { a.pf_ptr = fptr(ws, p.o_pk_c2f3[b][l]); a.pf_bytes = (unsigned)(3 * sizeof(uint16_t) * c.growth * p.mid * 27); }
+      else { a.pf_ptr = fptr(ws, p.o_pk_c2f[b][l]); a.pf_bytes = (unsigned)(sizeof(float) * c.growth * p.mid * 27); }
       { ScopedTimer t(p, T_CONV1_FWD, b, stream); rc = launch_fprop(a, 1, PRO_BNRELU, EPI_STORE_STATS, stream); }
       if (rc) return rc;
       FpropArgs e;
@@ -437,6 +455,7 @@
       e.in0 = fptr(ws, p.o_t1[b][l]); e.in0_ns = (long)p.mid * p.Vb[b]; e.in0_coff = 0;
       e.bn_in = bnfwd(p, statptr(ws, p.o_st_t1[b][l], p.mid, 0, p.nrep_b[b]), params, run, lo.n2w, lo.n2b, lo.r2m, lo.r2v, cnt, training);
       e.w = fptr(ws, p.o_pk_c2f[b][l]); e.w_ld = c.growth;
+      if (p.o_pk_c2f3[b][l]) { e.w3 = ws + p.o_pk_c2f3[b][l]; e.x3 = ws + p.o_x3; e.x3_bytes = p.x3_bytes; }
       e.out = fptr(ws, p.o_x[b]); e.out_ns = xns; e.out_coff = lo.cin;
       e.drop_out = dropcfg(p, seed, layer_id, training);
       e.st_out = statptr(ws, p.o_st_x[b], p.ctot_b[b], lo.cin, p.nrep_b[b]);
@@ -693,6 +712,7 @@
       a.gr_in = concat_grad(b, lo.cin);
       a.drop_in = drop;
       a.w = fptr(ws, p.o_pk_c2b[b][l]); a.w_ld = p.mid;
+      if (p.o_pk_c2b3[b][l]) { a.w3 = ws + p.o_pk_c2b3[b][l]; a.x3 = ws + p.o_x3; a.x3_bytes = p.x3_bytes; }
       float* dz2 = fptr(ws, p.o_dz2[b]) + (long)l * N * tns;
       a.out = dz2; a.out_ns = tns; a.out_coff = 0;
       a.ex = fptr(ws, p.o_t1[b][l]); a.ex_ns = tns; a.ex_coff = 0;
@@ -725,7 +745,8 @@
       d.ebn = bn1;
       d.dbeta = dg1.sum; d.dgamma = dg1.sq;
       d.s_acc = sptr(b, 0);
-      if (l > 0) { d.pf_ptr = fptr(ws, p.o_pk_c2b[b][l - 1]); d.pf_bytes = (unsigned)(sizeof(float) * c.growth * p.mid * 27); }
+      if (l > 0 && p.o_pk_c2b3[b][l - 1]) { d.pf_ptr = fptr(ws, p.o_pk_c2b3[b][l - 1]); d.pf_bytes = (unsigned)(3 * sizeof(uint16_t) * c.growth * p.mid * 27); }
+      else if (l > 0) { d.pf_ptr = fptr(ws, p.o_pk_c2b[b][l - 1]); d.pf_bytes = (unsigned)(sizeof(float) * c.growth * p.mid * 27); }
       { ScopedTimer t(p, T_CONV1_DGRAD, b, stream); rc = launch_fprop(d, 1, PRO_GRAD, EPI_MASK_ACCUM, stream); }
       if (rc) return rc;
       PendingW pw;
@@ -870,6 +891,10 @@
   if (s == "pk_c1" && okl(i, j)) return (long)p.o_pk_c1[i][j];
   if (s == "pk_c2f" && okl(i, j)) return (long)p.o_pk_c2f[i][j];
   if (s == "pk_c2b" && okl(i, j)) return (long)p.o_pk_c2b[i][j];
+  if (s == "pk_c2f3" && okl(i, j)) return p.o_pk_c2f3[i][j] ? (long)p.o_pk_c2f3[i][j] : -1;
+  if (s == "pk_c2b3" && okl(i, j)) return p.o_pk_c2b3[i][j] ? (long)p.o_pk_c2b3[i][j] : -1;
+  if (s == "x3") return p.x3_bytes ? (long)p.o_x3 : -1;
+  if (s == "#x3_bytes") return (long)p.x3_bytes;
   if (s == "pk_conv0") return (long)p.o_pk_conv0;
   if (s == "#pack_launches") return p.pack_launches;
   return -1;
diff --git a/mmnn_sts_amd/csrc/densenet.hpp b/mmnn_sts_amd/csrc/densenet.hpp
--- a/mmnn_sts_amd/csrc/densenet.hpp
+++ b/mmnn_sts_amd/csrc/densenet.hpp
@@ -47,6 +47,8 @@
   std::vector<size_t> o_dg_tr;
   size_t o_pk_conv0;
   std::vector<std::vector<size_t>> o_pk_c1, o_pk_c2f, o_pk_c2b;
+  std::vector<std::vector<size_t>> o_pk_c2f3, o_pk_c2b3;
+  size_t o_x3 = 0, x3_bytes = 0;
   std::vector<size_t> o_pk_tr;
   size_t o_sl_conv0; int ns_conv0;
   std::vector<std::vector<size_t>> o_sl_c1, o_sl_c2;
diff --git a/mmnn_sts_amd/csrc/elementwise.hip b/mmnn_sts_amd/csrc/elementwise.hip
--- a/mmnn_sts_amd/csrc/elementwise.hip
+++ b/mmnn_sts_amd/csrc/elementwise.hip
@@ -1,4 +1,5 @@
 #include "elementwise.hpp"
+#include "bf16x3.hpp"
 
 #include <algorithm>
 
@@ -205,6 +206,29 @@
     }
     return;
   }
+  if (j.kind >= 5) {
+    uint4* dst = reinterpret_cast<uint4*>(j.dst);
+    for (long i = (long)blockIdx.x * 256 + threadIdx.x; i < j.count; i += (long)gridDim.x * 256) {
+      float v[8];
+      if (j.kind == 5) {
+        const int m = (int)(i % j.M);
+        const long k = i / j.M;
+        const int c8 = (int)(k % (j.C / 8)), t = (int)(k / (j.C / 8));
+#pragma unroll
+        for (int e = 0; e < 8; ++e) v[e] = j.src[((long)m * j.C + 8 * c8 + e) * 27 + t];
+      } else {
+        const int c = (int)(i % j.C);
+        const long k = i / j.C;
+        const int m8 = (int)(k % (j.M / 8)), t = (int)(k / (j.M / 8));
+#pragma unroll
+        for (int e = 0; e < 8; ++e) v[e] = j.src[((long)(8 * m8 + e) * j.C + c) * 27 + 26 - t];
+      }
+      uint4 hi, mid, lo;
+      split3x8(v, hi, mid, lo);
+      dst[i] = hi; dst[j.count + i] = mid; dst[2 * j.count + i] = lo;
+    }
+    return;
+  }
   for (long i = (long)blockIdx.x * 256 + threadIdx.x; i < j.count; i += (long)gridDim.x * 256) {
     float v = 0.f;
     if (j.kind == 0) {
diff --git a/mmnn_sts_amd/csrc/fprop.hpp b/mmnn_sts_amd/csrc/fprop.hpp
--- a/mmnn_sts_amd/csrc/fprop.hpp
+++ b/mmnn_sts_amd/csrc/fprop.hpp
@@ -34,11 +34,15 @@
   float* kz_part; unsigned* kz_cnt;
   size_t kz_part_bytes; unsigned kz_cnt_entries;
   const float* pf_ptr; unsigned pf_bytes;
+  const void* w3; void* x3; size_t x3_bytes;
   unsigned mg_w, mg_h, mg_d;
   unsigned long long* trace;
 };
 
 int launch_fprop(const FpropArgs& a, int taps, int pro, int epi, hipStream_t stream);
+bool conv3_fwd_bf16x3_eligible(const FpropArgs& a);
+bool conv3_dgrad_bf16x3_eligible(const FpropArgs& a);
+size_t conv3_bf16x3_plane_bytes(const FpropArgs& a);
 int current_device_slot();
 constexpr int MAX_DEVICES = 32;
 
```

After: 260.4 volumes/s (whole job; 1 volume = 1 patient = stacked T1+T2 2x128^3 + 32 tabular), median of 6. 1.02x the previous value.
